# HKU-BAL/MegaPath-Nano

Hardware: AMD Instinct MI355X
Metric: Gbp/min ONT reads aligned+species-assigned vs RefSeq, 1/2/4/8 MI355X (higher is better)
Workload: dtype int32

## Files before the change

### include/mpn_map.h

```cpp
#ifndef MPN_MAP_H
#define MPN_MAP_H
#include <stdint.h>

#ifdef __cplusplus
extern "C" {
#endif

typedef struct mpn_index mpn_index;

typedef struct {
    int32_t k, w;
    float mid_occ_frac;
    int32_t mid_occ;
    int32_t max_gap, bw, max_chain_skip, max_chain_iter, min_cnt, min_chain_score;
    float mask_level, pri_ratio;
    int32_t best_n;
    int32_t max_join_long, max_join_short, min_join_flank_sc;
    float min_join_flank_ratio;
    int32_t a, b, q, e, q2, e2, sc_ambi, zdrop, zdrop_inv, end_bonus, min_dp_max, min_ksw_len;
    float max_clip_ratio;
    int64_t max_sw_mat;
    int32_t with_cigar;
    uint32_t seed;
    int32_t host_threads;
    int32_t out_sam;
    int32_t out_tags;
} mpn_map_opt;

enum {
    MPN_TAG_CS = 1,
    MPN_TAG_CS_LONG = 2,
    MPN_TAG_MD = 4,
    MPN_TAG_EQX = 8
};

void mpn_map_opt_init(mpn_map_opt *opt);

mpn_index *mpn_index_build(int32_t n_seq, const char *const *names, const char *const *seqs, const int32_t *lens,
                           int32_t k, int32_t w);
mpn_index *mpn_index_build_device(int32_t n_seq, const char *const *names, const void *d_seqs, const int64_t *seq_off,
                                  const int32_t *lens, int32_t k, int32_t w);
void mpn_index_destroy(mpn_index *idx);
int mpn_index_save(const mpn_index *idx, const char *path);
int64_t mpn_sam_header(const mpn_index *idx, const char *cmdline, char *buf, int64_t cap);
mpn_index *mpn_index_load(const char *path);
int mpn_index_save_append(const mpn_index *idx, const char *path);
mpn_index *mpn_index_load_at(const char *path, int64_t offset, int64_t *next_offset);
int32_t mpn_index_part_info(const char *path, int64_t offset, int64_t *bases, int64_t *next_offset);
int32_t mpn_index_n_seq(const mpn_index *idx);
int32_t mpn_index_seq_len(const mpn_index *idx, int32_t i);
int32_t mpn_index_seq_name(const mpn_index *idx, int32_t i, char *buf, int32_t cap);
int32_t mpn_index_k(const mpn_index *idx);
int32_t mpn_index_w(const mpn_index *idx);
int64_t mpn_index_n_minimizers(const mpn_index *idx);
int64_t mpn_index_n_keys(const mpn_index *idx);
int32_t mpn_index_mid_occ(const mpn_index *idx, float frac);
int64_t mpn_index_fetch_seq(const mpn_index *idx, int32_t i, int64_t start, int64_t len, char *out);
int mpn_index_export(const mpn_index *idx, uint64_t *keys, int64_t *key_off, uint64_t *pos);

int64_t mpn_sketch_batch(int32_t n, const char *seqs, const int64_t *seq_off, const int32_t *seq_len, int32_t k,
                         int32_t w, int64_t *mz_off, uint64_t *mz, int64_t cap);

int mpn_seed_chain_batch(const mpn_index *idx, const mpn_map_opt *opt, int32_t n, const char *seqs,
                         const int64_t *seq_off, const int32_t *seq_len, int64_t *n_anchor, int32_t *rep_len,
                         int64_t *chain_off, uint64_t *u, int64_t u_cap, int64_t *anchor_off, uint64_t *b,
                         int64_t b_cap);

int mpn_chain_batch(const mpn_map_opt *opt, int32_t n, const int64_t *anchor_off, const uint64_t *anchors, int32_t chain_item,
                    int32_t bt_par_min, int32_t grid_cap, int32_t *n_chain, int64_t *n_chained, uint64_t *u, int64_t *recs,
                    int64_t u_cap, uint64_t *b, int64_t b_cap);

int mpn_ext_dp_batch(const mpn_map_opt *opt, int32_t n, const uint8_t *qcodes, const int64_t *q_off, const int32_t *q_len,
                     const uint8_t *tcodes, const int64_t *t_off, const int32_t *t_len, const int32_t *w, const int32_t *zdrop,
                     const int32_t *end_bonus, const int32_t *flag, int32_t force_kernel, int32_t *out9, uint32_t *cigar_pool,
                     int64_t cigar_cap, int64_t *cig_off);

int mpn_aln_tags_batch(int32_t n, const uint8_t *qcodes, const int64_t *q_off, const int32_t *q_len,
                       const int32_t *qs, const int32_t *qe, const int32_t *rev,
                       const uint8_t *tcodes, const int64_t *t_off, const int32_t *t_len, const int32_t *ts,
                       const uint32_t *cigar, const int64_t *cig_off, const int32_t *n_cigar, int32_t out_tags,
                       char *cs, int64_t cs_cap, int64_t *cs_off, char *md, int64_t md_cap, int64_t *md_off,
                       uint32_t *eqx, int64_t eqx_cap, int64_t *eqx_off);

int mpn_aln_finish_batch(const mpn_map_opt *opt, int32_t n, const uint8_t *qcodes, const int64_t *q_off, const int32_t *q_len,
                         const int32_t *qs, const int32_t *qe, const int32_t *rev,
                         const uint8_t *tcodes, const int64_t *t_off, const int32_t *t_len, const int32_t *ts,
                         const uint32_t *cigar, const int64_t *cig_off, const int32_t *n_cigar, int32_t force_class,
                         int32_t *out8, uint32_t *cigar_out);

int mpn_hit_select_batch(const mpn_map_opt *opt, int32_t k, int32_t n, const int32_t *q_len, const char *const *names,
                         const int64_t *chain_off, const uint64_t *u, const uint64_t *fx, const uint64_t *fy, const uint64_t *lx,
                         const uint64_t *ly, const int32_t *mlen, const int32_t *blen, const int64_t *anchor_off, const uint64_t *anchors,
                         int32_t path, int32_t max_chains, int32_t grid_cap, int32_t *n_regs, int32_t *n_a, int64_t *hits,
                         uint64_t *sq_anchors);

int mpn_ext_plan_batch(const mpn_map_opt *opt, int32_t k, int32_t n_targets, const int32_t *t_len, int32_t n, const int32_t *q_len,
                       const int64_t *anchor_off, const uint64_t *anchors, const int64_t *hit_off, const int32_t *h_as,
                       const int32_t *h_cnt, const int32_t *h_mlen, const int32_t *h_split_inv, int32_t grid_cap,
                       int32_t *hits_out, int64_t win_cap, int64_t *n_win, int32_t *win_out, uint64_t *anchors_out);

int mpn_stitch_batch(int32_t n, const int64_t *anchor_off, const uint64_t *anchors, int32_t n_hits, const int32_t *hits, int64_t n_win,
                     const int32_t *wins, const int64_t *cig_pos, int64_t n_compact, const uint32_t *compact, int32_t min_cnt,
                     int32_t grid_cap, int64_t *out, int64_t pool_cap, uint32_t *pool_out, int64_t *pool_used, int64_t *splits_out,
                     int64_t *n_splits);

int64_t mpn_map_batch(const mpn_index *idx, const mpn_map_opt *opt, int32_t n, const char *const *names,
                      const char *seqs, const int64_t *seq_off, const int32_t *seq_len, char *paf, int64_t paf_cap);

typedef struct {
    int64_t cap, n_rows;
    int32_t *read_idx, *qs, *qe, *rev, *rid, *rs, *re, *mlen, *blen, *mapq, *nm, *as, *primary;
} mpn_aln_cols;

int64_t mpn_map_batch_ex(const mpn_index *idx, const mpn_map_opt *opt, int32_t n, const char *const *names,
                         const char *seqs, const int64_t *seq_off, const int32_t *seq_len, const void *d_seqs,
                         const int64_t *d_off, const int32_t *d_len, char *paf, int64_t paf_cap, mpn_aln_cols *cols);

int64_t mpn_map_batch_q(const mpn_index *idx, const mpn_map_opt *opt, int32_t n, const char *const *names, const char *seqs,
                        const char *quals, const int64_t *seq_off, const int32_t *seq_len, const void *d_seqs, const int64_t *d_off,
                        const int32_t *d_len, char *paf, int64_t paf_cap, mpn_aln_cols *cols);
int64_t mpn_map_fetch_sam(char *buf, int64_t cap);

typedef struct mpn_hits mpn_hits;
mpn_hits *mpn_hits_create(int32_t n_reads);
void mpn_hits_destroy(mpn_hits *h);
void mpn_hits_set_text(mpn_hits *h, int32_t want_text);
int mpn_map_batch_part(const mpn_index *part, const mpn_map_opt *opt, int32_t n, const char *const *names, const char *seqs,
                       const int64_t *seq_off, const int32_t *seq_len, const void *d_seqs, const int64_t *d_off,
                       const int32_t *d_len, mpn_hits *acc);
int mpn_map_batch_parts(const mpn_index *const *parts, int32_t n_parts, const mpn_map_opt *opt, int32_t n, const char *const *names,
                        const char *seqs, const int64_t *seq_off, const int32_t *seq_len, const void *r_seqs, const int64_t *r_off,
                        const int32_t *r_len, mpn_hits *acc);
int64_t mpn_hits_finish(mpn_hits *acc, const mpn_map_opt *opt, int32_t n, const char *const *names, const char *seqs,
                        const char *quals, const int64_t *seq_off, const int32_t *seq_len, char *paf, int64_t paf_cap,
                        mpn_aln_cols *cols);
int32_t mpn_hits_n_parts(const mpn_hits *h);
int32_t mpn_hits_n_seq(const mpn_hits *h);
int32_t mpn_hits_seq_len(const mpn_hits *h, int32_t i);
int32_t mpn_hits_seq_name(const mpn_hits *h, int32_t i, char *buf, int32_t cap);
int64_t mpn_hits_sam_header(const mpn_hits *h, const char *cmdline, char *buf, int64_t cap);

int64_t mpn_hits_export(const mpn_hits *h, int32_t lo, int32_t hi, void *buf, int64_t cap);
int mpn_hits_import(mpn_hits *h, const void *buf, int64_t len, int32_t n_parts, int32_t n_seq, const char *const *names,
                    const int32_t *lens);

int64_t mpn_map_fetch_cols(mpn_aln_cols *cols);
int64_t mpn_map_fetch_text(char *buf, int64_t cap);

void mpn_map_last_stats(int64_t stats[32]);
int32_t mpn_map_last_stats_ex(int64_t *stats, int32_t n);

#ifdef __cplusplus
}
#endif
#endif
```

### megapath_nano_amd/csrc/align.hip

```cpp
#include "map_types.h"
#include "ext_kernels.h"
#include "fin_kernels.h"
#include "tag_kernels.h"
#include "stitch_kernels.h"
#include "plan_kernels.h"
#include "hit_kernels.h"
#include "mapper_internal.h"
#include "../../include/mpn_map.h"
#include "../../include/mpn_ssw.h"

#include <algorithm>
#include <condition_variable>
#include <deque>
#include <math.h>
#include <stdio.h>
#include <string.h>
#include <thread>
#include <pthread.h>
#include <time.h>
#include <atomic>
#include <functional>
#include <mutex>
#include <stdlib.h>
#include <string>
// ... 1818 lines not shown
        std::vector<uint32_t> nh((size_t)n, 0u);
        if (names) for (int i = 0; i < n; ++i) nh[(size_t)i] = names[i] ? x31_hash(names[i]) : 0u;
        if (d_name_hash.upload(nh.data(), (size_t)n, st0)) return -1;
        MPN_HIP_CHECK(hipStreamSynchronize(st0));
    }
    MPN_HIP_CHECK(hipStreamSynchronize(st0));
    wt.stop_into(g_stats[16]);
    int n_threads = default_host_threads(opt);
    *n_threads_out = n_threads;
    g_pool.ensure(n_threads);
    int n_workers = 12;
    if (const char *e = getenv("MPN_PIPE_WORKERS")) n_workers = std::max(1, std::min(16, atoi(e)));
    static double obs_bytes_per_bp = 0.0;
    static int64_t obs_sub_bp = 0;
    const bool env_target = getenv("MPN_SUB_BATCH_BP") != nullptr;
    const int W_all = n_workers;
    std::vector<int> cut;
    auto make_cuts = [&](int64_t target) {
        cut.assign(1, 0);
        std::vector<int64_t> sizes;
        int64_t n_cut = std::max<int64_t>(1, (bases + target - 1) / target);
        if (n_cut > W_all) n_cut = (n_cut + W_all - 1) / W_all * W_all;
        for (int64_t i = 0; i < n_cut; ++i) sizes.push_back(std::max<int64_t>(1, (bases + n_cut - 1) / n_cut));
        size_t si = 0;
        int64_t acc = 0;
        for (int i = 0; i < n; ++i) {
            acc += seq_len[i];
            if (si + 1 < sizes.size() && acc >= sizes[si] && i + 1 < n) { cut.push_back(i + 1); acc = 0; ++si; }
        }
        cut.push_back(n);
    };
    int64_t target = 32000000;
    if (env_target) target = std::max<int64_t>(1000, atoll(getenv("MPN_SUB_BATCH_BP")));
    make_cuts(target);
    int n_sub = (int)cut.size() - 1;
    int64_t largest = n_sub > 0 ? (bases + n_sub - 1) / n_sub : bases;
    {
        size_t free_b = 0, total_b = 0, held = 0;
        if (hipMemGetInfo(&free_b, &total_b) == hipSuccess) {
            for (const Slot &S : g_slots) held += S.device_bytes();
            const double avail = 0.9 * (double)(free_b + held);
            const double bytes_per_bp = obs_bytes_per_bp > 0 ? std::max(400.0, 1.15 * obs_bytes_per_bp) : 900.0;
            auto per_worker = [&](int64_t sub_bp) { return bytes_per_bp * (double)std::max<int64_t>(sub_bp, 1) + 2e9; };
            int fit = (int)std::max(1.0, avail / per_worker(largest));
            if (fit < std::min(W_all, n_sub) && !env_target && largest > 11000000) {
                const double room = avail / W_all - 2e9;
                const int64_t t2 = std::max<int64_t>(11000000, (int64_t)(room / bytes_per_bp));
                if (t2 < largest) {
                    make_cuts(t2);
                    n_sub = (int)cut.size() - 1;
                    largest = n_sub > 0 ? (bases + n_sub - 1) / n_sub : bases;
                    fit = (int)std::max(1.0, avail / per_worker(largest));
                }
            }
            if (obs_sub_bp > 0 && largest < obs_sub_bp * 3 / 4) {
                MPN_HIP_CHECK(hipDeviceSynchronize());
                for (Slot &S : g_slots) S.release_device();
            }
            n_workers = std::min(n_workers, fit);
        }
    }
    const int n_items = n_sub;
    n_workers = std::max(1, std::min(n_workers, n_items));
    for (int wdx = n_workers; wdx < 16; ++wdx)
        if (g_slots[wdx].device_bytes()) { MPN_HIP_CHECK(hipDeviceSynchronize()); g_slots[wdx].release_device(); }
    int dev = 0;
    MPN_HIP_CHECK(hipGetDevice(&dev));
    QueueStreams *qs = queue_streams(dev);
    if (!qs) { set_error("creating the submission streams failed"); return -1; }
    rs.assign((size_t)n_parts, std::vector<ReadState>());
    rep_len.assign((size_t)n_parts, std::vector<int32_t>());
    for (int p = 0; p < n_parts; ++p) { rs[(size_t)p].assign((size_t)n, ReadState()); rep_len[(size_t)p].assign((size_t)n, 0); }
    std::atomic<int> next(0), failed(0);
    std::mutex mu;
    std::deque<int> retry;
    int live_workers = n_workers, live_workers_busy = 0, n_shed = 0;
    int64_t tot_stats[MPN_NSTATS] = {0};
    std::string err;
    const bool dbg_workers = getenv("MPN_DEBUG_WORKERS") != nullptr;
    g_phase_log.on = getenv("MPN_DEBUG_PHASES") != nullptr;
    g_cpu_on = getenv("MPN_DEBUG_CPU") != nullptr;
    if (g_cpu_on) { for (auto &c : g_cpu_ns) c = 0; for (auto &c : g_worker_cpu_ns) c = 0; }
    g_worker_cpu_on = g_cpu_on;
    if (g_phase_log.on) { g_phase_log.recs.clear(); g_phase_log.origin = std::chrono::steady_clock::now(); }
    const auto t_call = std::chrono::steady_clock::now();
    auto since = [&]() { return std::chrono::duration<double, std::milli>(std::chrono::steady_clock::now() - t_call).count(); };
    auto worker = [&](int wid) {
        pthread_setname_np(pthread_self(), "mpn-work");
        if (hipSetDevice(dev) != hipSuccess) { failed = 1; return; }
        Slot &S = g_slots[wid];
        StreamLease lease(qs);
        tl_slot = &S;
        tl_arena = &S.arena;
        tl_worker_id = wid;
        memset(g_stats, 0, sizeof(g_stats));
        for (;;) {
            int sb = -1;
            { std::lock_guard<std::mutex> g(mu); if (!retry.empty()) { sb = retry.front(); retry.pop_front(); } }
            if (sb < 0) sb = next.fetch_add(1);
            if (sb >= n_items || failed) {
                std::unique_lock<std::mutex> lk(mu);
                if (failed || (retry.empty() && live_workers_busy == 0)) break;
                lk.unlock();
                timespec ts{0, 200000};
                nanosleep(&ts, nullptr);
                continue;
            }
            { std::lock_guard<std::mutex> g(mu); ++live_workers_busy; }
            struct Busy { std::mutex &m; int &c; ~Busy() { std::lock_guard<std::mutex> g(m); --c; } } busy_{mu, live_workers_busy};
            S.arena.reset();
            tl_oom = false;
            int64_t stats_before[MPN_NSTATS];
            memcpy(stats_before, g_stats, sizeof(stats_before));
            const double t_in = since();
            struct Out { bool on; int wid, sb; double t_in; decltype(since) &f; ~Out() { if (on) fprintf(stderr, "[worker %d] sub-batch %d: %.1f -> %.1f ms\n", wid, sb, t_in, f()); } } out_{dbg_workers, wid, sb, t_in, since};
            int rc_item = 0;
            {
                ReadSketch sk;
                const int sbi = sb, nr = cut[sbi + 1] - cut[sbi];
                if (n_parts > 1 && nr > 0) {
                    WallTimer wts;
                    rc_item = sketch_reads(parts[0]->k, parts[0]->w, nr, dv.p, dv.po + cut[sbi], dv.pl + cut[sbi], seq_len + cut[sbi], sk, lease);
                    wts.stop_into(g_stats[17]);
                }
                const Arena::Mark after_sketch = S.arena.mark();
                for (int prt = 0; prt < n_parts && !rc_item; ++prt) {
                    S.arena.rewind(after_sketch);
                    rc_item = map_range(parts[prt], opt, names, seqs, seq_off, seq_len, dv.p, dv.po, dv.pl, d_name_hash.p, cut[sbi], cut[sbi + 1], n_threads, lease,
                                        rs[(size_t)prt], rep_len[(size_t)prt], sk.valid ? &sk : nullptr);
                }
                if (!rc_item && stream_sync(lease) != hipSuccess) { set_error("stream wait failed"); rc_item = -1; }
            }
            if (rc_item) {
                std::lock_guard<std::mutex> g(mu);
                if (tl_oom && live_workers > 1) {
                    --live_workers;
                    ++n_shed;
                    memcpy(g_stats, stats_before, sizeof(stats_before));
                    (void)hipGetLastError();
                    (void)stream_sync(lease);
                    S.release_device();
                    retry.push_back(sb);
                    if (dbg_workers) fprintf(stderr, "[worker %d] out of device memory at sub-batch %d: leaving, %d workers go on\n", wid, sb, live_workers);
                    break;
                }
                err = get_error();
                failed = 1;
                (void)stream_sync(lease);
                break;
            }
        }
        tl_arena = nullptr;
        std::lock_guard<std::mutex> g(mu);
        for (int k = 0; k < MPN_NSTATS; ++k) tot_stats[k] += g_stats[k];
    };
    {
        std::vector<std::thread> th;
        for (int wdx = 0; wdx < n_workers; ++wdx) th.emplace_back(worker, wdx);
        for (auto &t : th) t.join();
    }
    if (dbg_workers) {
        fprintf(stderr, "[call] workers joined at %.1f ms\n", since());
        for (int wdx = 0; wdx < n_workers; ++wdx) {
            const Slot &S = g_slots[wdx];
            size_t arena = 0;
            for (const auto &c : S.arena.chunks) arena += c.cap;
            const size_t pools = S.pool_jobs.cap + S.pool_P.cap + S.pool_P2.cap + S.pool_OFF.cap + S.pool_order.cap + S.pool_state.cap + S.pool_CIG.cap +
                                 S.pool_res.cap + S.pool_redo.cap + S.pool_compact.cap + S.pool_used.cap;
            const size_t pinned = S.pin_order.cap + S.pin_res.cap + S.pin_chain_u.cap + S.pin_chain_b.cap + S.pin_segs.cap + S.pin_pregs.cap + S.pin_fin_cig.cap + S.pin_fin_out.cap + S.pin_tags.cap + S.pin_tag_bytes.cap;
            fprintf(stderr, "[slot %d] arena %.2f GB, pools %.2f GB (P %.2f, CIG %.2f, compact %.2f), pinned host %.2f GB\n", wdx, arena / 1e9,
                    pools / 1e9, S.pool_P.cap / 1e9, S.pool_CIG.cap / 1e9, S.pool_compact.cap / 1e9, pinned / 1e9);
        }
    }
    if (g_phase_log.on) {
        for (const auto &r : g_phase_log.recs) fprintf(stderr, "[phase] %d %d %lld %lld\n", r.worker, r.slot, (long long)r.t0, (long long)r.t1);
        fprintf(stderr, "[phase-end]\n");
    }
    if (g_cpu_on) {
        static const char *const nm[] = {"other", "hits", "plan", "plan-copy", "stitch", "final", "dp-group-A", "strip-sort", "job-copy", "finish-copy", "accumulate", "merge"};
        fprintf(stderr, "[cpu] thread CPU ms in parallel regions:");
        for (int k = 0; k < 12; ++k) fprintf(stderr, " %s %.0f", nm[k], g_cpu_ns[k].load() / 1e6);
        fprintf(stderr, "\n[cpu] sections: stitch-append %.0f", g_cpu_ns[16].load() / 1e6);
        for (int k = 3; k < 16; ++k) if (g_cpu_ns[16 + k].load() > 500000) fprintf(stderr, " s%d %.0f", k, g_cpu_ns[16 + k].load() / 1e6);
        fprintf(stderr, "\n[cpu] worker-thread CPU ms by phase slot:");
        for (int k = 0; k < 64; ++k) if (g_worker_cpu_ns[k].load() > 500000) fprintf(stderr, " [%d] %.0f", k, g_worker_cpu_ns[k].load() / 1e6);
        fprintf(stderr, "\n");
    }
    if (failed) { set_error("%s", err.empty() ? "worker failed" : err.c_str()); return -1; }
    {
        const int64_t h2d = g_stats[16];
        memcpy(g_stats, tot_stats, sizeof(tot_stats));
        g_stats[16] = h2d;
        g_stats[0] = bases;
        g_stats[60] = n_shed; g_stats[61] = n_workers;
        {
            size_t held_max = 0;
            for (const Slot &S : g_slots) held_max = std::max(held_max, S.device_bytes());
            if (largest > 0 && held_max > 0) {
                const double r = (double)held_max / (double)largest;
                obs_bytes_per_bp = obs_sub_bp == largest ? std::max(obs_bytes_per_bp, r) : r;
                obs_sub_bp = largest;
            }
        }
    }
    return 0;
}

static struct Kept { std::vector<int32_t> cols; int64_t n_rows = -1; std::string text, sam; bool has_text = false, has_sam = false; } g_kept;

static int64_t emit_batch(const Targets tg, const mpn_map_opt *opt, int32_t n, const char *const *names, const char *seqs, const char *quals,
                          const int64_t *seq_off, const int32_t *seq_len, std::vector<std::vector<Reg>*> &regs, const std::vector<int32_t> &rep_len,
                          int n_threads, char *text, int64_t text_cap, mpn_aln_cols *cols) {
    const bool want_paf = text && opt->out_sam != 1, want_sam = opt->out_sam == 2 || (text && opt->out_sam == 1);
    std::vector<std::string> paf_lines(want_paf ? n : 0), sam_lines(want_sam ? n : 0);
    int64_t n_aln = 0;
    for (int i = 0; i < n; ++i) n_aln += (int64_t)regs[i]->size();
    if (want_paf || want_sam)
        parallel_for(n, n_threads, [&](int i, int) {
            const char *nm = names && names[i] ? names[i] : "*";
            if (want_paf && !regs[i]->empty()) write_paf(tg, opt, nm, seq_len[i], *regs[i], rep_len[i], paf_lines[i]);
            if (want_sam) write_sam(tg, opt, nm, seq_len[i], seqs + seq_off[i], quals ? quals + seq_off[i] : nullptr, *regs[i], rep_len[i], sam_lines[i]);
        }, 0, 16);
    bool short_cols = false, short_text = false;
    g_kept.cols.clear(); g_kept.text.clear(); g_kept.sam.clear(); g_kept.n_rows = -1; g_kept.has_text = g_kept.has_sam = false;
    if (cols) {
        cols->n_rows = n_aln;
        short_cols = n_aln > cols->cap;
        int32_t *dst[13] = {cols->read_idx, cols->qs, cols->qe, cols->rev, cols->rid, cols->rs, cols->re, cols->mlen, cols->blen, cols->mapq,
                            cols->nm, cols->as, cols->primary};
        if (short_cols) {
            g_kept.cols.resize((size_t)n_aln * 13);
            g_kept.n_rows = n_aln;
            for (int c = 0; c < 13; ++c) dst[c] = g_kept.cols.data() + (size_t)c * (size_t)n_aln;
        }
        int64_t k = 0;
        for (int i = 0; i < n; ++i)
            for (const Reg &r : *regs[i]) {
                dst[0][k] = i; dst[1][k] = r.qs; dst[2][k] = r.qe; dst[3][k] = (int32_t)r.rev; dst[4][k] = r.rid;
                dst[5][k] = r.rs; dst[6][k] = r.re; dst[7][k] = r.mlen; dst[8][k] = r.blen; dst[9][k] = (int32_t)r.mapq;
                dst[10][k] = r.has_p ? r.blen - r.mlen + r.n_ambi : -1;
                dst[11][k] = r.has_p ? r.dp_score : -1;
                dst[12][k] = r.id == r.parent;
                ++k;
            }
    }
    int64_t w = 0;
    if (text) {
        std::vector<std::string> &lines = opt->out_sam == 1 ? sam_lines : paf_lines;
        int64_t tot = 0;
        for (auto &l : lines) tot += (int64_t)l.size();
        short_text = tot + 1 > text_cap;
        if (short_text) {
            g_kept.text.reserve((size_t)tot);
            for (auto &l : lines) g_kept.text += l;
            g_kept.has_text = true;
        } else {
            for (auto &l : lines) { memcpy(text + w, l.data(), l.size()); w += (int64_t)l.size(); }
            text[w] = 0;
        }
    }
    if (opt->out_sam == 2) {
        size_t tot = 0;
        for (auto &l : sam_lines) tot += l.size();
        g_kept.sam.reserve(tot);
        for (auto &l : sam_lines) g_kept.sam += l;
        g_kept.has_sam = true;
    }
    parallel_chunks(n, n_threads, [&](int64_t lo, int64_t hi, int) {
        for (int64_t i = lo; i < hi; ++i) { if (want_paf) std::string().swap(paf_lines[i]); if (want_sam) std::string().swap(sam_lines[i]); }
    });
    g_stats[6] = n_aln;
    return (short_cols || short_text) ? -3 : w;
}

static std::mutex g_call_mu;

extern "C" int64_t mpn_map_batch_q(const mpn_index *idx, const mpn_map_opt *opt, int32_t n, const char *const *names,
                                   const char *seqs, const char *quals, const int64_t *seq_off, const int32_t *seq_len, const void *r_seqs,
                                   const int64_t *r_off, const int32_t *r_len, char *paf, int64_t paf_cap, mpn_aln_cols *cols) {
    std::lock_guard<std::mutex> call_guard(g_call_mu);
    memset(g_stats, 0, sizeof(g_stats));
    if (cols) cols->n_rows = 0;
    if (n <= 0) { if (paf && paf_cap > 0) paf[0] = 0; g_kept = Kept(); if (opt->out_sam == 2) g_kept.has_sam = true; return 0; }
    WallTimer whole;
    std::vector<std::vector<ReadState>> rs_p;
    std::vector<std::vector<int32_t>> rep_p;
    int n_threads = 1;
    g_need_cigar = paf != nullptr || opt->out_sam != 0;
    if (map_batch_core(&idx, 1, opt, n, names, seqs, seq_off, seq_len, r_seqs, r_off, r_len, rs_p, rep_p, &n_threads)) return -1;
    std::vector<ReadState> &rs = rs_p[0];
    std::vector<int32_t> &rep_len = rep_p[0];
    std::vector<std::vector<Reg>*> regs((size_t)n);
    for (int i = 0; i < n; ++i) regs[(size_t)i] = &rs[(size_t)i].regs;
    const int64_t w = emit_batch(Targets{&idx->names, &idx->lens}, opt, n, names, seqs, quals, seq_off, seq_len, regs, rep_len, n_threads, paf, paf_cap, cols);
    parallel_chunks(n, n_threads, [&](int64_t lo, int64_t hi, int) { for (int64_t i = lo; i < hi; ++i) rs[(size_t)i] = ReadState(); });
    whole.stop_into(g_stats[24]);
    return w;
}

extern "C" int64_t mpn_map_batch_ex(const mpn_index *idx, const mpn_map_opt *opt, int32_t n, const char *const *names,
                                    const char *seqs, const int64_t *seq_off, const int32_t *seq_len, const void *r_seqs,
                                    const int64_t *r_off, const int32_t *r_len, char *paf, int64_t paf_cap, mpn_aln_cols *cols) {
    return mpn_map_batch_q(idx, opt, n, names, seqs, nullptr, seq_off, seq_len, r_seqs, r_off, r_len, paf, paf_cap, cols);
}

extern "C" mpn_hits *mpn_hits_create(int32_t n_reads) {
    if (n_reads < 0) { set_error("mpn_hits_create: negative read count"); return nullptr; }
// ... 885 lines not shown
```

### megapath_nano_amd/csrc/map_kernels.h

```cpp
#pragma once
#include "mpn_common.h"
#include "map_types.h"

#include <type_traits>

namespace mpn {

__device__ __forceinline__ uint64_t hash64m(uint64_t key, uint64_t mask) {
    key = (~key + (key << 21)) & mask;
    key = key ^ key >> 24;
    key = ((key + (key << 3)) + (key << 8)) & mask;
    key = key ^ key >> 14;
    key = ((key + (key << 2)) + (key << 4)) & mask;
    key = key ^ key >> 28;
    key = (key + (key << 31)) & mask;
    return key;
}

constexpr int SKETCH_FAST_MAX_W = 32;

template <bool HASH64>
__device__ __forceinline__ uint64_t sketch_hash(uint64_t key, uint64_t mask) {
    if (HASH64) return hash64m(key, mask);
    uint32_t h = (uint32_t)key;
// ... 1272 lines not shown
                const unsigned long long over = __ballot(skipev && skips > cp.max_skip);
                const int brk = over ? __builtin_ctzll(over) : 64;
                if (!over) n_skip = __builtin_amdgcn_readlane(skips, 63);
                const bool elig = !cont && lane < brk;
                const int best = brk > 0 ? __builtin_amdgcn_readlane(incl, brk - 1) : NEG_INF;
                if (best > max_f) {
                    const unsigned long long who = __ballot(elig && sc == best);
                    const int wl = __builtin_ctzll(who);
                    max_f = best;
                    max_j = j0 - wl;
                }
                if (!tile_in_ring && elig && pj >= 0) {
                    if (pj >= win_lo) wt[pj & M] = i;
                    else { t[pj] = i; gmark = true; }
                }
                if (brk < 64) done = true;
                if (__ballot(gmark)) __builtin_amdgcn_fence(__ATOMIC_RELEASE, "workgroup");
                MPN_LDS_FENCE();
            }
            int32_t vprev = 0;
            if (max_j >= 0) vprev = max_j >= win_lo ? wv[max_j & M] : v[max_j];
            const int32_t vi = (max_j >= 0 && vprev > max_f) ? vprev : max_f;
            if (lane == li) { rf = max_f; rp = max_j >= 0 ? max_j + rel : -1; rv = vi; }
            if (lane == 0) {
                const int sl = i & M;
                *reinterpret_cast<uint4 *>(&ring[sl]) = make_uint4(ri, (uint32_t)qi, (uint32_t)max_f, (uint32_t)max_j);
                wv[sl] = vi; wt[sl] = 0;
            }
            MPN_LDS_FENCE();
            if (li == 63 || i == n - 1) {
                const int32_t k = (i & ~63) + lane;
                if (k <= i) { f[k] = rf; p[k] = rp; v[k] = rv; }
                const uint32_t carry = (uint32_t)__builtin_amdgcn_readlane((int)cx, 63);
                cx = (uint32_t)wave_scan_add((int)nstep) + carry; cx64 = nx64; cyl = nyl; cyh = nyh;
            }
        }
        __builtin_amdgcn_fence(__ATOMIC_RELEASE, "workgroup");
        __syncthreads();
    }
}

__global__ __launch_bounds__(64) void chain_ends_kernel(const int64_t *__restrict__ anchor_off, int n_reads, ChainParams cp,
                                                        const int32_t *__restrict__ F, const int32_t *__restrict__ P,
                                                        int32_t *__restrict__ T, const int32_t *__restrict__ V,
                                                        uint64_t *__restrict__ U, int32_t *__restrict__ n_ends) {
    const int lane = threadIdx.x;
    for (int read = blockIdx.x; read < n_reads; read += gridDim.x) {
        const int64_t base = anchor_off[read];
        const int64_t n = anchor_off[read + 1] - base;
        const int32_t *f = F + base, *p = P + base, *v = V + base;
        int32_t *t = T + base;
        uint64_t *u = U + base;
        for (int64_t i = lane; i < n; i += 64) t[i] = 0;
        __builtin_amdgcn_fence(__ATOMIC_RELEASE, "workgroup");
        __syncthreads();
        for (int64_t i = lane; i < n; i += 64) if (p[i] >= 0) t[p[i]] = 1;
        __builtin_amdgcn_fence(__ATOMIC_RELEASE, "workgroup");
        __syncthreads();
        int cnt = 0;
        for (int64_t i0 = 0; i0 < n; i0 += 64) {
            const int64_t i = i0 + lane;
            bool is_end = i < n && t[i] == 0 && v[i] >= cp.min_sc;
            uint64_t val = 0;
            if (is_end) {
                int64_t j = i;
                while (j >= 0 && f[j] < v[j]) j = p[j];
                if (j < 0) j = i;
                val = (uint64_t)(uint32_t)f[j] << 32 | (uint64_t)j;
            }
            const unsigned long long m = __ballot(is_end);
            if (is_end) u[cnt + __popcll(m & ((1ULL << lane) - 1))] = val;
            cnt += __popcll(m);
        }
        if (lane == 0) n_ends[read] = cnt;
        __syncthreads();
    }
}

__global__ __launch_bounds__(256) void chain_sort_ends_kernel(uint64_t *__restrict__ U, uint64_t *__restrict__ Utmp,
                                                              const int64_t *__restrict__ anchor_off,
                                                              const int32_t *__restrict__ n_ends, int n_reads) {
    __shared__ uint32_t hist[256];
    __shared__ uint32_t bins[256];
    __shared__ uint32_t wcnt[4][256];
    __shared__ int s_skip;
    const int tid = threadIdx.x, lane = tid & 63, wv = tid >> 6;
    for (int read = blockIdx.x; read < n_reads; read += gridDim.x) {
        const int64_t base = anchor_off[read];
        const int n = n_ends[read];
        if (n < 2) continue;
        uint64_t *src = U + base, *dst = Utmp + base;
        for (int pass = 0; pass < 8; ++pass) {
            hist[tid] = 0;
            __syncthreads();
            for (int i = tid; i < n; i += 256) atomicAdd(&hist[(uint32_t)(~src[i] >> (8 * pass)) & 0xff], 1u);
            __syncthreads();
            if (tid == 0) s_skip = 0;
            __syncthreads();
            if (hist[tid] == (uint32_t)n) s_skip = 1;
            __syncthreads();
            if (s_skip) { __syncthreads(); continue; }
            {
                uint32_t v = hist[tid];
                bins[tid] = v;
                __syncthreads();
                for (int d = 1; d < 256; d <<= 1) {
                    uint32_t a = tid >= d ? bins[tid - d] : 0;
                    __syncthreads();
                    bins[tid] += a;
                    __syncthreads();
                }
                uint32_t excl = bins[tid] - v;
                __syncthreads();
                bins[tid] = excl;
                __syncthreads();
            }
            for (int t0 = 0; t0 < n; t0 += 256) {
                const int i = t0 + tid;
                const bool act = i < n;
                uint64_t r = 0;
                uint32_t dg = 0;
                if (act) { r = src[i]; dg = (uint32_t)(~r >> (8 * pass)) & 0xff; }
                wcnt[0][tid] = 0; wcnt[1][tid] = 0; wcnt[2][tid] = 0; wcnt[3][tid] = 0;
                __syncthreads();
                unsigned long long same = __ballot(act);
#pragma unroll
                for (int b = 0; b < 8; ++b) {
                    unsigned long long m = __ballot((dg >> b) & 1);
                    same &= ((dg >> b) & 1) ? m : ~m;
                }
                const uint32_t rank = __popcll(same & ((1ULL << lane) - 1));
                if (act && rank == 0) wcnt[wv][dg] = __popcll(same);
                __syncthreads();
                if (act) {
                    uint32_t o = bins[dg] + rank;
                    for (int w2 = 0; w2 < wv; ++w2) o += wcnt[w2][dg];
                    dst[o] = r;
                }
                __syncthreads();
                bins[tid] += wcnt[0][tid] + wcnt[1][tid] + wcnt[2][tid] + wcnt[3][tid];
                __syncthreads();
            }
            uint64_t *sw = src; src = dst; dst = sw;
            __threadfence_block();
            __syncthreads();
        }
        if (src != U + base) for (int i = tid; i < n; i += 256) U[base + i] = src[i];
        __syncthreads();
    }
}

constexpr int BT_PAR_MIN = 16;

__global__ __launch_bounds__(64) void chain_backtrack_kernel(const u128 *__restrict__ anchors, const int64_t *__restrict__ anchor_off,
                                                             int n_reads, ChainParams cp, const int32_t *__restrict__ F,
                                                             const int32_t *__restrict__ P, int32_t *__restrict__ T,
                                                             int32_t *__restrict__ V, uint64_t *__restrict__ U,
                                                             const int32_t *__restrict__ n_ends, u128 *__restrict__ B,
                                                             uint64_t *__restrict__ Uc, unsigned long long *__restrict__ used,
                                                             int64_t *__restrict__ u_pos, int64_t *__restrict__ b_pos,
                                                             int32_t *__restrict__ n_chain, int64_t *__restrict__ n_chained,
                                                             ChainRec *__restrict__ Rc, int par_min) {
    __shared__ int s_k;
    __shared__ unsigned long long s_up, s_bp;
    const int lane = threadIdx.x;
    for (int read = blockIdx.x; read < n_reads; read += gridDim.x) {
        const int64_t base = anchor_off[read];
        const int64_t n = anchor_off[read + 1] - base;
        const u128 *a = anchors + base;
        const int32_t *f = F + base, *p = P + base;
        int32_t *t = T + base, *v = V + base;
        uint64_t *u = U + base;
        const int n_u = n_ends[read];
        if (n_u >= par_min) {
            for (int64_t i = lane; i < n; i += 64) t[i] = 0x7fffffff;
            __builtin_amdgcn_fence(__ATOMIC_RELEASE, "agent");
            __syncthreads();
            for (int e0 = 0; e0 < n_u; e0 += 64) {
                const int e = e0 + lane;
                if (e < n_u) {
                    int32_t j = (int32_t)u[e];
                    while (j >= 0) { const int32_t nj = p[j]; if (atomicMin(&t[j], e) < e) break; j = nj; }
                }
            }
            __builtin_amdgcn_fence(__ATOMIC_ACQ_REL, "agent");
            __syncthreads();
            int k_run = 0, nv_run = 0;
            for (int e0 = 0; e0 < n_u; e0 += 64) {
                const int e = e0 + lane;
                int cnt = 0;
                if (e < n_u) {
                    const uint64_t ui = u[e];
                    int32_t j = p[(int32_t)ui];
                    cnt = 1;
                    while (j >= 0) { const int32_t tj = t[j], nj = p[j]; if (tj != e) break; ++cnt; j = nj; }
                    const bool keep = cnt >= cp.min_cnt && (j < 0 || (int32_t)(ui >> 32) - f[j] >= cp.min_sc);
                    if (!keep) cnt = 0;
                    v[e] = cnt;
                }
                k_run += __builtin_amdgcn_readlane(wave_scan_add(cnt > 0 ? 1 : 0), 63);
                nv_run += __builtin_amdgcn_readlane(wave_scan_add(cnt), 63);
            }
            if (lane == 0) {
                s_k = k_run;
                n_chain[read] = k_run;
                n_chained[read] = nv_run;
                s_up = k_run ? atomicAdd(&used[0], (unsigned long long)k_run) : 0ULL;
                s_bp = nv_run ? atomicAdd(&used[1], (unsigned long long)nv_run) : 0ULL;
                u_pos[read] = (int64_t)s_up;
                b_pos[read] = (int64_t)s_bp;
            }
            __builtin_amdgcn_fence(__ATOMIC_ACQ_REL, "agent");
            __syncthreads();
            u128 *b = B + s_bp;
            uint64_t *uc = Uc + s_up;
            ChainRec *rc = Rc + s_up;
            k_run = 0; nv_run = 0;
            for (int e0 = 0; e0 < n_u; e0 += 64) {
                const int e = e0 + lane;
                const int cnt = e < n_u ? v[e] : 0;
                const int incl = wave_scan_add(cnt), kin = wave_scan_add(cnt > 0 ? 1 : 0);
                if (cnt > 0) {
                    const int kidx = k_run + kin - 1, off = nv_run + incl - cnt;
                    const uint64_t ui = u[e];
                    int32_t j = (int32_t)ui;
                    u128 nxt = a[j];
                    const u128 last = nxt;
                    int ml = 0, bl = 0;
                    b[off + cnt - 1] = nxt;
                    for (int q = cnt - 2; q >= 0; --q) {
                        j = p[j];
                        const u128 cur = a[j];
                        b[off + q] = cur;
                        const int span = (int)(nxt.y >> 32 & 0xff);
                        const int tl = (int32_t)nxt.x - (int32_t)cur.x, ql = (int32_t)nxt.y - (int32_t)cur.y;
                        bl += tl > ql ? tl : ql;
                        ml += tl > span && ql > span ? span : tl < ql ? tl : ql;
                        nxt = cur;
                    }
                    const int span0 = (int)(nxt.y >> 32 & 0xff);
                    ml += span0; bl += span0;
                    j = p[j];
                    const uint64_t sc = j < 0 ? ui >> 32 : (ui >> 32) - (uint64_t)f[j];
                    uc[kidx] = sc << 32 | (uint32_t)cnt;
                    rc[kidx] = ChainRec{nxt.x, nxt.y, last.x, last.y, ml, bl};
                }
                k_run += __builtin_amdgcn_readlane(kin, 63);
                nv_run += __builtin_amdgcn_readlane(incl, 63);
            }
            __syncthreads();
            continue;
        }
        for (int64_t i = lane; i < n; i += 64) t[i] = 0;
        __builtin_amdgcn_fence(__ATOMIC_RELEASE, "workgroup");
        __syncthreads();
        if (lane == 0) {
            int n_v = 0, k = 0;
            for (int i = 0; i < n_u; ++i) {
                const int n_v0 = n_v, k0 = k;
                const uint64_t ui = u[i];
                int64_t j = (int32_t)ui;
                do { v[n_v++] = (int32_t)j; t[j] = 1; j = p[j]; } while (j >= 0 && t[j] == 0);
                if (j < 0) {
                    if (n_v - n_v0 >= cp.min_cnt) u[k++] = ui >> 32 << 32 | (uint32_t)(n_v - n_v0);
                } else if ((int32_t)(ui >> 32) - f[j] >= cp.min_sc) {
                    if (n_v - n_v0 >= cp.min_cnt) u[k++] = ((ui >> 32) - (uint64_t)f[j]) << 32 | (uint32_t)(n_v - n_v0);
                }
                if (k0 == k) n_v = n_v0;
            }
            s_k = k;
            n_chain[read] = k;
            n_chained[read] = n_v;
            s_up = k ? atomicAdd(&used[0], (unsigned long long)k) : 0ULL;
            s_bp = n_v ? atomicAdd(&used[1], (unsigned long long)n_v) : 0ULL;
            u_pos[read] = (int64_t)s_up;
            b_pos[read] = (int64_t)s_bp;
        }
        __builtin_amdgcn_fence(__ATOMIC_RELEASE, "workgroup");
        __syncthreads();
        const int k = s_k;
        u128 *b = B + s_bp;
        uint64_t *uc = Uc + s_up;
        ChainRec *rc = Rc + s_up;
        int off = 0;
        for (int c = 0; c < k; ++c) {
            const int ni = (int32_t)u[c];
            int ml = 0, bl = 0;
            for (int j = lane; j < ni; j += 64) {
                const u128 cur = a[v[off + (ni - j - 1)]];
                b[off + j] = cur;
                const int span = (int)(cur.y >> 32 & 0xff);
                if (j == 0) { ml += span; bl += span; }
                else {
                    const u128 prev = a[v[off + (ni - j)]];
                    const int tl = (int32_t)cur.x - (int32_t)prev.x, ql = (int32_t)cur.y - (int32_t)prev.y;
                    bl += tl > ql ? tl : ql;
                    ml += tl > span && ql > span ? span : tl < ql ? tl : ql;
                }
            }
            ml = __builtin_amdgcn_readlane(wave_scan_add(ml), 63);
            bl = __builtin_amdgcn_readlane(wave_scan_add(bl), 63);
            if (lane == 0) {
                const u128 first = a[v[off + ni - 1]], last = a[v[off]];
                rc[c] = ChainRec{first.x, first.y, last.x, last.y, ml, bl};
            }
            off += ni;
        }
        for (int c = lane; c < k; c += 64) uc[c] = u[c];
        __syncthreads();
    }
}

__global__ __launch_bounds__(256) void idx_bucket_hist_kernel(const u128 *__restrict__ mz, int64_t n, int shift, unsigned long long *__restrict__ hist) {
    for (int64_t i = (int64_t)blockIdx.x * blockDim.x + threadIdx.x; i < n; i += (int64_t)gridDim.x * blockDim.x)
        atomicAdd(&hist[(mz[i].x >> 8) >> shift], 1ULL);
}

__global__ __launch_bounds__(256) void idx_bucket_scatter_kernel(const u128 *__restrict__ mz, int64_t n, int shift,
                                                                 unsigned long long *__restrict__ cursor, u128 *__restrict__ out) {
    for (int64_t i = (int64_t)blockIdx.x * blockDim.x + threadIdx.x; i < n; i += (int64_t)gridDim.x * blockDim.x) {
        u128 r = mz[i];
        r.x >>= 8;
        const unsigned long long p = atomicAdd(&cursor[r.x >> shift], 1ULL);
        out[p] = r;
    }
}

__global__ __launch_bounds__(256) void idx_flag_count_kernel(const u128 *__restrict__ rec, int64_t n, int64_t *__restrict__ block_cnt) {
    __shared__ int s[256];
    const int64_t base = (int64_t)blockIdx.x * 2048;
    int c = 0;
    for (int k = 0; k < 8; ++k) {
        const int64_t i = base + k * 256 + threadIdx.x;
        if (i < n && (i == 0 || rec[i].x != rec[i - 1].x)) ++c;
    }
    s[threadIdx.x] = c;
    __syncthreads();
    for (int d = 128; d; d >>= 1) { if (threadIdx.x < d) s[threadIdx.x] += s[threadIdx.x + d]; __syncthreads(); }
    if (threadIdx.x == 0) block_cnt[blockIdx.x] = s[0];
}

__global__ __launch_bounds__(256) void idx_emit_kernel(const u128 *__restrict__ rec, int64_t n, const int64_t *__restrict__ block_off,
                                                       uint64_t *__restrict__ keys, int64_t *__restrict__ key_off,
                                                       uint64_t *__restrict__ pos) {
    __shared__ int s[256];
    const int64_t base = (int64_t)blockIdx.x * 2048;
    int flags = 0, c = 0;
    for (int k = 0; k < 8; ++k) {
        const int64_t i = base + (int64_t)threadIdx.x * 8 + k;
        if (i < n) {
            pos[i] = rec[i].y;
            if (i == 0 || rec[i].x != rec[i - 1].x) { flags |= 1 << k; ++c; }
        }
    }
    s[threadIdx.x] = c;
    __syncthreads();
    for (int d = 1; d < 256; d <<= 1) {
        const int v = threadIdx.x >= d ? s[threadIdx.x - d] : 0;
        __syncthreads();
        s[threadIdx.x] += v;
        __syncthreads();
    }
    int64_t o = block_off[blockIdx.x] + s[threadIdx.x] - c;
    for (int k = 0; k < 8; ++k)
        if (flags >> k & 1) {
            const int64_t i = base + (int64_t)threadIdx.x * 8 + k;
            keys[o] = rec[i].x;
            key_off[o] = i;
            ++o;
        }
}

__global__ __launch_bounds__(256) void idx_pack2_kernel(const uint8_t *__restrict__ seqs, int64_t total, uint32_t *__restrict__ words,
                                                        int64_t n_words, unsigned long long *__restrict__ counters,
                                                        int64_t *__restrict__ starts, int64_t *__restrict__ ends, int64_t cap) {
    const bool aligned = (reinterpret_cast<uintptr_t>(seqs) & 15) == 0;
    for (int64_t wi = (int64_t)blockIdx.x * blockDim.x + threadIdx.x; wi < n_words; wi += (int64_t)gridDim.x * blockDim.x) {
        const int64_t g0 = wi * 16;
        uint8_t b[16];
        if (aligned && g0 + 16 <= total) {
            const uint4 v = *reinterpret_cast<const uint4 *>(seqs + g0);
            const uint32_t q[4] = {v.x, v.y, v.z, v.w};
#pragma unroll
            for (int k = 0; k < 16; ++k) b[k] = (uint8_t)(q[k >> 2] >> (8 * (k & 3)));
        } else {
#pragma unroll
            for (int k = 0; k < 16; ++k) b[k] = g0 + k < total ? seqs[g0 + k] : (uint8_t)'A';
        }
        bool prev_n = g0 > 0 && g0 - 1 < total && nt4_code(seqs[g0 - 1]) > 3;
        uint32_t word = 0;
#pragma unroll
        for (int k = 0; k < 16; ++k) {
            const int64_t g = g0 + k;
            const int c = nt4_code(b[k]);
            const bool isn = g < total && c > 3;
            if (g < total && !isn) word |= (uint32_t)c << (2 * k);
            if (isn != prev_n && g <= total) {
                const unsigned long long p = atomicAdd(&counters[isn ? 0 : 1], 1ULL);
                if ((int64_t)p < cap) (isn ? starts : ends)[p] = g;
            }
            prev_n = isn;
        }
        words[wi] = word;
    }
}

__global__ __launch_bounds__(256) void idx_occ_hist_kernel(const u128 *__restrict__ kv, int64_t n_keys, int nbins,
                                                           unsigned long long *__restrict__ hist) {
    __shared__ unsigned int local[1024];
    for (int k = threadIdx.x; k < 1024; k += blockDim.x) local[k] = 0;
    __syncthreads();
    for (int64_t i = (int64_t)blockIdx.x * blockDim.x + threadIdx.x; i < n_keys; i += (int64_t)gridDim.x * blockDim.x) {
        const int64_t occ = (int64_t)(kv[i + 1].y - kv[i].y);
        if (occ < 1024) atomicAdd(&local[(int)occ], 1u);
        else atomicAdd(&hist[occ < nbins - 1 ? occ : nbins - 1], 1ULL);
    }
    __syncthreads();
    for (int k = threadIdx.x; k < 1024; k += blockDim.x) if (local[k]) atomicAdd(&hist[k], (unsigned long long)local[k]);
}

}
```

### megapath_nano_amd/csrc/mapper.hip

```cpp
#include "map_kernels.h"
#include "mapper_internal.h"
#include "../../include/mpn_map.h"

#include <algorithm>
#include <mutex>
#include <string.h>
#include <time.h>
#include <sys/stat.h>
#include <string>
#include <vector>

namespace mpn {

hipError_t stream_sync(hipStream_t st) {
    struct Ev {
        hipEvent_t e = nullptr;
        ~Ev() { if (e) (void)hipEventDestroy(e); }
    };
    static thread_local Ev ev;
    hipError_t rc;
    if (!ev.e && (rc = hipEventCreateWithFlags(&ev.e, hipEventDisableTiming)) != hipSuccess) return rc;
    if ((rc = hipEventRecord(ev.e, st)) != hipSuccess) return rc;
    unsigned int us = 20;
    for (;;) {
// ... 57 lines not shown
    *out = *s;
    return 0;
}

thread_local int64_t g_stats[MPN_NSTATS] = {0};
PhaseLog g_phase_log;
bool g_worker_cpu_on = false;
std::atomic<long long> g_worker_cpu_ns[64];
thread_local int tl_worker_id = -1;

void pack_2bit(const uint8_t *codes, int64_t n, std::vector<uint32_t> &words, std::vector<int64_t> &ns, std::vector<int64_t> &ne) {
    words.assign((size_t)(n + 15) / 16 + 1, 0u);
    ns.clear(); ne.clear();
    for (int64_t i = 0; i < n; ++i) {
        const uint8_t c = codes[i];
        if (c > 3) {
            if (!ne.empty() && ne.back() == i) ne.back() = i + 1;
            else { ns.push_back(i); ne.push_back(i + 1); }
        } else words[(size_t)(i >> 4)] |= (uint32_t)c << (2 * (int)(i & 15));
    }
}

static int grid_1d(int64_t n, int block, int cap = 256 * 16) {
    int64_t g = (n + block - 1) / block;
    return (int)std::max<int64_t>(1, std::min<int64_t>(g, cap));
}

int sketch_device(const uint8_t *d_seqs, const int64_t *d_off, const int32_t *d_len, const int32_t *h_len, int n, int k, int w,
                  uint32_t rid_base, DevBuf<int64_t> &mz_off, DevBuf<u128> &mz, int64_t *n_mz, hipStream_t st, EvTimer *ev = nullptr) {
    const int C = 256;
    std::vector<int64_t> chunk_off((size_t)n + 1, 0);
    for (int i = 0; i < n; ++i) chunk_off[i + 1] = chunk_off[i] + (h_len[i] + C - 1) / C;
    const int64_t n_chunks = chunk_off[n];
    DevBuf<int64_t> cnt, d_chunk_off, slow_list;
    DevBuf<int32_t> chunk_cnt, chunk_rel;
    DevBuf<unsigned long long> n_slow, emask;
    DevBuf<uint8_t> cfast;
    DevBuf<int32_t> chunk_read;
    DevBuf<u128> stage;
    int64_t stage_chunks = 0;
    if (cnt.alloc((size_t)n + 1) || mz_off.alloc((size_t)n + 1) || d_chunk_off.upload(chunk_off.data(), (size_t)n + 1, st) ||
        chunk_cnt.alloc((size_t)n_chunks) || chunk_rel.alloc((size_t)n_chunks) || slow_list.alloc((size_t)n_chunks) || n_slow.alloc(1) ||
        emask.alloc((size_t)n_chunks * 4 + 4) || cfast.alloc((size_t)n_chunks + 1) || chunk_read.alloc((size_t)n_chunks + 1))
        return -1;
    hipLaunchKernelGGL(sketch_chunk_read_kernel, dim3(std::max(1, std::min((n + 3) / 4, 4096))), dim3(256), 0, st, (const int64_t *)d_chunk_off.p, n, chunk_read.p);
    {
        std::vector<int64_t> slow;
        const bool none_fast = !(k & 1) || w > SKETCH_FAST_MAX_W;
        for (int i = 0; i < n; ++i) {
            const int64_t nc = chunk_off[i + 1] - chunk_off[i];
            for (int64_t c = 0; c < nc; ++c) {
                const int64_t p0 = c * C, p1 = std::min<int64_t>(h_len[i], p0 + C);
                if (none_fast || p0 - 2 * w - k < 0 || p1 + w + 1 > h_len[i]) slow.push_back(chunk_off[i] + c);
                else if (p1 + C + w + 1 <= h_len[i]) c = std::max<int64_t>(c, (h_len[i] - w - 1) / C - 2);
            }
        }
        const unsigned long long ns = slow.size();
        stage_chunks = (int64_t)std::min<unsigned long long>((unsigned long long)n_chunks, ns + 2048);
        if (stage_chunks * SKETCH_STAGE_CAP * sizeof(u128) > ((size_t)1 << 30)) stage_chunks = ((size_t)1 << 30) / (SKETCH_STAGE_CAP * sizeof(u128));
        if (stage.alloc((size_t)stage_chunks * SKETCH_STAGE_CAP + 1)) return -1;
        if (ns) MPN_HIP_CHECK(hipMemcpyAsync(slow_list.p, slow.data(), ns * 8, hipMemcpyHostToDevice, st));
        MPN_HIP_CHECK(hipMemcpyAsync(n_slow.p, &ns, 8, hipMemcpyHostToDevice, st));
        MPN_HIP_CHECK(stream_sync(st));
    }
    const size_t lds = (size_t)2 * w * 64 * sizeof(uint64_t);
    const unsigned fast_grid = (unsigned)std::max<int64_t>(1, std::min<int64_t>((n_chunks + 3) / 4, 256 * 64));
    const unsigned slow_grid = (unsigned)std::max<int64_t>(1, std::min<int64_t>((n_chunks + 63) / 64, 256 * 16));
    const bool hash64 = 2 * k > 32;
    auto pass = [&](bool fill, u128 *out) {
        if (n_chunks <= 0) return;
        const int64_t *moff = fill ? (const int64_t *)mz_off.p : nullptr;
        const int32_t *crel = fill ? (const int32_t *)chunk_rel.p : nullptr;
        int32_t *ccnt = fill ? nullptr : chunk_cnt.p;
        if (fill) {
            if (hash64) hipLaunchKernelGGL(sketch_fill_kernel<true>, dim3(fast_grid), dim3(256), 0, st, d_seqs, d_off, d_len, n, (const int64_t *)d_chunk_off.p, (const int32_t *)chunk_read.p, n_chunks, C,
                                           w, k, moff, crel, out, rid_base, (const unsigned long long *)emask.p, (const uint8_t *)cfast.p);
            else hipLaunchKernelGGL(sketch_fill_kernel<false>, dim3(fast_grid), dim3(256), 0, st, d_seqs, d_off, d_len, n, (const int64_t *)d_chunk_off.p, (const int32_t *)chunk_read.p, n_chunks, C,
                                    w, k, moff, crel, out, rid_base, (const unsigned long long *)emask.p, (const uint8_t *)cfast.p);
        } else {
#define MPN_SKETCH_FAST(H, WCT) hipLaunchKernelGGL((sketch_fast_kernel<H, WCT>), dim3(fast_grid), dim3(256), 0, st, d_seqs, d_off, d_len, n, \
                                                  (const int64_t *)d_chunk_off.p, (const int32_t *)chunk_read.p, n_chunks, C, w, k, ccnt, slow_list.p, n_slow.p, emask.p, cfast.p)
            if (hash64) MPN_SKETCH_FAST(true, 0); else if (w == 10) MPN_SKETCH_FAST(false, 10); else MPN_SKETCH_FAST(false, 0);
#undef MPN_SKETCH_FAST
        }
        if (fill) {
            hipLaunchKernelGGL(sketch_stage_copy_kernel, dim3(slow_grid), dim3(256), 0, st, (const int32_t *)chunk_read.p, (const int64_t *)slow_list.p,
                               (const unsigned long long *)n_slow.p, stage_chunks, moff, crel, (const int32_t *)chunk_cnt.p, (const u128 *)stage.p, out);
            if (stage_chunks < n_chunks)
                hipLaunchKernelGGL(sketch_chunk_kernel<true>, dim3(slow_grid), dim3(64), lds, st, d_seqs, d_off, d_len, n, (const int64_t *)d_chunk_off.p, (const int32_t *)chunk_read.p,
                                   (const int64_t *)slow_list.p, (const unsigned long long *)n_slow.p, C, w, k, moff, crel, ccnt, out, rid_base,
                                   (u128 *)nullptr, (int64_t)0, stage_chunks);
        } else hipLaunchKernelGGL(sketch_chunk_kernel<false>, dim3(slow_grid), dim3(64), lds, st, d_seqs, d_off, d_len, n, (const int64_t *)d_chunk_off.p, (const int32_t *)chunk_read.p,
                                  (const int64_t *)slow_list.p, (const unsigned long long *)n_slow.p, C, w, k, moff, crel, ccnt, out, rid_base,
                                  stage.p, stage_chunks, (int64_t)0);
    };
    if (ev) ev->skip();
    pass(false, nullptr);
    MPN_HIP_CHECK(hipGetLastError());
    if (ev) ev->mark(10, 33);
    hipLaunchKernelGGL(sketch_chunk_prefix_kernel, dim3((n + 255) / 256), dim3(256), 0, st, (const int64_t *)d_chunk_off.p, n,
                       (const int32_t *)chunk_cnt.p, chunk_rel.p, cnt.p);
    MPN_HIP_CHECK(hipGetLastError());
    hipLaunchKernelGGL(scan_i64_kernel, dim3(1), dim3(1024), 0, st, cnt.p, mz_off.p, n);
    MPN_HIP_CHECK(hipGetLastError());
    int64_t total = 0;
    if (read_i64(mz_off.p + n, &total, st)) return -1;
    if (mz.alloc((size_t)total)) return -1;
    if (ev) ev->mark(10);
    if (total > 0) {
        pass(true, mz.p);
        MPN_HIP_CHECK(hipGetLastError());
        if (ev) ev->mark(10, 34);
    }
    *n_mz = total;
    return 0;
}

int upload_seqs(int32_t n, const char *seqs, const int64_t *seq_off, const int32_t *seq_len, DevBuf<uint8_t> &d_seqs,
                DevBuf<int64_t> &d_off, DevBuf<int32_t> &d_len, int64_t *total_bases, hipStream_t st) {
    int64_t extent = 0, bases = 0;
    for (int i = 0; i < n; ++i) {
        if (seq_len[i] < 0 || seq_off[i] < 0) { set_error("negative sequence length/offset at %d", i); return -2; }
        extent = std::max<int64_t>(extent, seq_off[i] + seq_len[i]);
        bases += seq_len[i];
    }
    if (d_seqs.alloc((size_t)extent + 16)) return -1;
    if (extent) MPN_HIP_CHECK(hipMemcpyAsync(d_seqs.p, seqs, (size_t)extent, hipMemcpyHostToDevice, st));
    if (d_off.upload(seq_off, n, st) || d_len.upload(seq_len, n, st)) return -1;
    *total_bases = bases;
    return 0;
}

int sketch_reads(int k, int w, int n, const uint8_t *d_seqs, const int64_t *d_off, const int32_t *d_len, const int32_t *h_len, ReadSketch &sk,
                 StreamLease &st) {
    EvTimer ev(st);
    sk.valid = false;
    if (sketch_device(d_seqs, d_off, d_len, h_len, n, k, w, 0, sk.mz_off, sk.mz, &sk.n_mz, st, &ev)) return -1;
    MPN_HIP_CHECK(stream_sync(st));
    ev.resolve();
    sk.k = k; sk.w = w; sk.valid = true;
    return 0;
}

static int chain_gap_check(const mpn_map_opt *opt, const char *who) {
    if (opt->max_gap > CHAIN_MAX_GAP) {
        set_error("%s: max_gap %d is beyond %d, the largest the chain DP's 32-bit ring coordinate holds", who, opt->max_gap, CHAIN_MAX_GAP);
        return -1;
    }
    return 0;
}

static int alloc_chain_tables(SeedChainOut &o, int n) {
    const size_t N = (size_t)n, o1 = (N + 1) * 8, o2 = o1 + N * 8, o3 = o2 + N * 8, o4 = o3 + N * 8, o5 = o4 + N * 4, o6 = (o5 + N * 4 + 7) & ~(size_t)7;
    o.tables_bytes = o6 + (size_t)(2 + WORK_SLOTS) * 8;
    if (o.tables.alloc(o.tables_bytes)) return -1;
    auto view = [&](auto &buf, size_t off, size_t count) { buf.release(); buf.p = reinterpret_cast<decltype(buf.p)>(o.tables.p + off); buf.n = count; buf.owned = false; };
    view(o.n_anchor, 0, N + 1); view(o.n_chained, o1, N); view(o.u_pos, o2, N); view(o.b_pos, o3, N);
    view(o.n_chain, o4, N); view(o.rep_len, o5, N); view(o.used, o6, 2 + WORK_SLOTS);
    return 0;
}

struct ChainKnobs {
    int chain_item = 0;
    int bt_par_min = 0;
    int grid_cap = 0;
};
struct ChainScratch {
    DevBuf<int64_t> kept, piece_kept, piece_off;
    DevBuf<float> avg_qspan;
    DevBuf<int32_t> F, P, T, V;
    DevBuf<uint64_t> Utmp;
    DevBuf<ChainSeg> seg_big, seg_small;
};
static int chain_enqueue(const mpn_map_opt *opt, int n, int64_t n_a, SeedChainOut &o, u128 *tmp, unsigned long long *read_kept,
                         const unsigned long long *span_sum, unsigned int *seg_counters, const ChainKnobs &kn, ChainScratch &cs, StreamLease &st,
                         EvTimer &ev) {
    auto &[kept, piece_kept, piece_off, avg_qspan, F, P, T, V, Utmp, seg_big, seg_small] = cs;
    ChainParams cp;
    cp.max_dist_x = opt->max_gap; cp.max_dist_y = opt->max_gap; cp.bw = opt->bw; cp.max_skip = opt->max_chain_skip;
    cp.max_iter = opt->max_chain_iter; cp.min_cnt = opt->min_cnt; cp.min_sc = opt->min_chain_score;
    const auto capped = [&](int64_t grid) { return (int)(kn.grid_cap > 0 ? std::min<int64_t>(grid, kn.grid_cap) : grid); };
    const int g = capped(std::max(1, std::min(n, 256 * 32)));
    const int64_t n_pieces = (n_a + COMPACT_PIECE - 1) / COMPACT_PIECE;
    if (kept.alloc((size_t)n + 1) || o.c_off.alloc((size_t)n + 1) || avg_qspan.alloc(n) || piece_kept.alloc((size_t)n_pieces + 1) ||
        piece_off.alloc((size_t)n_pieces + 1))
        return -1;
    const int gp = capped(std::max<int64_t>(1, std::min<int64_t>(n_pieces, 256 * 64)));
    if (n_a > 0) {
        hipLaunchKernelGGL(anchor_compact_kernel<false>, dim3(gp), dim3(64), 0, st, (const u128 *)o.anchors.p, (const int64_t *)o.anchor_off.p, n, n_a,
                           cp.max_dist_x, cp.min_cnt, piece_kept.p, read_kept, (const int64_t *)nullptr, (u128 *)nullptr);
        MPN_HIP_CHECK(hipGetLastError());
    }
    hipLaunchKernelGGL(anchor_compact_finish_kernel, dim3((n + 255) / 256), dim3(256), 0, st, (const int64_t *)o.n_anchor.p, n,
                       (const unsigned long long *)read_kept, span_sum, kept.p, avg_qspan.p);
    hipLaunchKernelGGL(scan_i64x2_kernel, dim3(2), dim3(1024), 0, st, (const int64_t *)kept.p, o.c_off.p, n, (const int64_t *)piece_kept.p, piece_off.p, (int)n_pieces);
    MPN_HIP_CHECK(hipGetLastError());
    int64_t n_c = 0;
    if (read_i64(o.c_off.p + n, &n_c, st)) return -1;
    g_stats[45] += n_c;
    if (F.alloc(n_c) || P.alloc(n_c) || T.alloc(n_c) || V.alloc(n_c) || o.u.alloc(n_c) || Utmp.alloc(n_c) || o.chained.alloc(n_c) ||
        o.recs.alloc((size_t)(n_c / std::max(1, opt->min_cnt)) + 1))
        return -1;
    u128 *ca = tmp;
    if (n_a > 0) {
        hipLaunchKernelGGL(anchor_compact_kernel<true>, dim3(gp), dim3(64), 0, st, (const u128 *)o.anchors.p, (const int64_t *)o.anchor_off.p, n, n_a,
                           cp.max_dist_x, cp.min_cnt, (int64_t *)nullptr, (unsigned long long *)nullptr, (const int64_t *)piece_off.p, ca);
        MPN_HIP_CHECK(hipGetLastError());
    }
    ev.mark(46);
    static const int chain_item_env = []() { const char *e = getenv("MPN_CHAIN_ITEM"); return e ? std::min(CHAIN_BIG, std::max(16, atoi(e))) : CHAIN_ITEM; }();
    const int chain_item = kn.chain_item > 0 ? std::min(CHAIN_BIG, std::max(16, kn.chain_item)) : chain_item_env;
    if (seg_big.alloc((size_t)n_c / CHAIN_BIG + (size_t)n + 1) || seg_small.alloc((size_t)n_c / chain_item + (size_t)n + 1)) return -1;
    hipLaunchKernelGGL(chain_segments_kernel, dim3(g), dim3(64), 0, st, (const u128 *)ca, (const int64_t *)o.c_off.p, n, cp, avg_qspan.p, 1, seg_big.p,
                       seg_small.p, seg_counters, chain_item);
    MPN_HIP_CHECK(hipGetLastError());
    ev.mark(13);
    hipLaunchKernelGGL(chain_dp_kernel, dim3(capped(256 * 32)), dim3(64), 0, st, (const u128 *)ca, (const int64_t *)o.c_off.p, (const float *)avg_qspan.p,
                       (const ChainSeg *)seg_big.p, (const ChainSeg *)seg_small.p, seg_counters, cp, F.p, P.p, T.p, V.p);
    MPN_HIP_CHECK(hipGetLastError());
    ev.mark(13, 37);
    hipLaunchKernelGGL(chain_ends_kernel, dim3(g), dim3(64), 0, st, (const int64_t *)o.c_off.p, n, cp, F.p, P.p, T.p, V.p, o.u.p, o.n_ends.p);
    MPN_HIP_CHECK(hipGetLastError());
    hipLaunchKernelGGL(chain_sort_ends_kernel, dim3(capped(std::max(1, std::min(n, 256 * 8)))), dim3(256), 0, st, o.u.p, Utmp.p,
                       (const int64_t *)o.c_off.p, o.n_ends.p, n);
    MPN_HIP_CHECK(hipGetLastError());
    o.u_compact.p = Utmp.p; o.u_compact.n = Utmp.n; o.u_compact.owned = Utmp.owned; Utmp.p = nullptr; Utmp.n = 0;
    static const int bt_par_min_env = []() { const char *e = getenv("MPN_BT_PAR_MIN"); return e ? std::max(1, atoi(e)) : BT_PAR_MIN; }();
    const int bt_par_min = kn.bt_par_min > 0 ? kn.bt_par_min : bt_par_min_env;
    hipLaunchKernelGGL(chain_backtrack_kernel, dim3(g), dim3(64), 0, st, (const u128 *)ca, (const int64_t *)o.c_off.p, n, cp, F.p, P.p, T.p, V.p,
                       o.u.p, o.n_ends.p, o.chained.p, o.u_compact.p, o.used.p, o.u_pos.p, o.b_pos.p, o.n_chain.p, o.n_chained.p, o.recs.p, bt_par_min);
    MPN_HIP_CHECK(hipGetLastError());
    return 0;
}

int seed_chain_device(const mpn_index *idx, const mpn_map_opt *opt, int n, const uint8_t *d_seqs, const int64_t *d_off,
                      const int32_t *d_len, const int32_t *h_len, SeedChainOut &o, StreamLease &st, const ReadSketch *pre) {
    if (chain_gap_check(opt, "seed + chain stage")) return -1;
    int64_t n_mz = 0;
    DevBuf<int64_t> mz_off;
    DevBuf<u128> mz;
    EvTimer ev(st);
    if (pre && pre->valid && pre->k == idx->k && pre->w == idx->w) {
        mz_off.p = pre->mz_off.p; mz_off.n = pre->mz_off.n; mz_off.owned = false;
        mz.p = pre->mz.p; mz.n = pre->mz.n; mz.owned = false;
        n_mz = pre->n_mz;
    } else if (sketch_device(d_seqs, d_off, d_len, h_len, n, idx->k, idx->w, 0, mz_off, mz, &n_mz, st, &ev)) return -1;
    g_stats[1] += n_mz;
    int32_t mid_occ = opt->mid_occ > 0 ? opt->mid_occ : mpn_index_mid_occ(idx, opt->mid_occ_frac);
    if (mid_occ > (1 << 25)) {
        const int32_t top = mpn_index_mid_occ(idx, 1e-30f);
        if (top > 0) mid_occ = std::min(mid_occ, top);
    }
    DevBuf<int32_t> occ;
    DevBuf<int64_t> pos_start, rel_off, full_off, n_blk, blk_base;
    DevBuf<unsigned long long> span_sum;
    if (alloc_chain_tables(o, n)) return -1;
    if (occ.alloc(n_mz) || pos_start.alloc(n_mz) || rel_off.alloc(n_mz) || full_off.alloc((size_t)n + 1) ||
        n_blk.alloc((size_t)n + 1) || blk_base.alloc((size_t)n + 1) || span_sum.alloc(n) || o.anchor_off.alloc((size_t)n + 1))
        return -1;
    if (n_mz > 0) {
        hipLaunchKernelGGL(seed_lookup_kernel, dim3(grid_1d(n_mz, 256)), dim3(256), 0, st, (const u128 *)idx->kv.p,
                           idx->n_keys, (const int64_t *)idx->bucket_start.p, idx->bucket_shift, mz.p, n_mz, mid_occ, occ.p, pos_start.p);
        MPN_HIP_CHECK(hipGetLastError());
        ev.mark(11, 35);
    }
    hipLaunchKernelGGL(seed_prefix_kernel, dim3(std::max(1, std::min(n, 256 * 32))), dim3(64), 0, st, mz.p, mz_off.p, n, occ.p, rel_off.p,
                       o.n_anchor.p, o.rep_len.p, span_sum.p, n_blk.p);
    MPN_HIP_CHECK(hipGetLastError());
    hipLaunchKernelGGL(scan_i64x2_kernel, dim3(2), dim3(1024), 0, st, (const int64_t *)o.n_anchor.p, full_off.p, n, (const int64_t *)n_blk.p, blk_base.p, n);
    MPN_HIP_CHECK(hipGetLastError());
    int64_t n_full = 0;
    if (read_i64(full_off.p + n, &n_full, st)) return -1;
    g_stats[2] += n_full;
    const int64_t nb_cap = n_mz / 64 + n + 1;
    DevBuf<unsigned long long> keep;
    DevBuf<int64_t> blk_kept, blk_off;
    DevBuf<int32_t> blk_read, order;
    DevBuf<unsigned int> next_read;
    DevBuf<unsigned int> n_list, seg_counters;
    DevBuf<unsigned long long> read_kept;
    if (next_read.alloc(4) || order.alloc(n) || keep.alloc((size_t)(n_full / 64 + nb_cap + 8)) || blk_kept.alloc((size_t)nb_cap + 1) || blk_off.alloc((size_t)nb_cap + 2) ||
        blk_read.alloc((size_t)nb_cap + 1) || n_list.alloc(4) || seg_counters.alloc(4) || read_kept.alloc(n))
        return -1;
    {
        ZeroList z{};
        zero_list_push(z, next_read.p, 4 * sizeof(unsigned int));
        zero_list_push(z, blk_kept.p, ((size_t)nb_cap + 1) * 8);
        zero_list_push(z, o.used.p, o.used.n * sizeof(unsigned long long));
        zero_list_push(z, n_list.p, 4 * sizeof(unsigned int));
        zero_list_push(z, seg_counters.p, 4 * sizeof(unsigned int));
        zero_list_push(z, read_kept.p, (size_t)n * 8);
        MPN_HIP_CHECK(zero_regions(z, st));
    }
    if (nb_cap > 0x7fffffff) { set_error("sub-batch too large for the seed filter"); return -1; }
    if (mid_occ > (1 << 25)) { set_error("occurrence cut-off %d too large (a block of 64 minimizers must hold fewer than 2^32 hits)", mid_occ); return -1; }
    if (n_full > 0) {
        FilterParams fp;
        {
            const int T = std::max(1, std::min(opt->min_cnt, 3));
            const int64_t need = 2 * (int64_t)(T - 1) * std::max(opt->max_gap, 1);
            int sh = 1;
            while (sh < 32 && ((int64_t)1 << sh) < need) ++sh;
            fp.shift = sh; fp.half = (uint32_t)((uint64_t)1 << (sh - 1)); fp.level = T - 1;
            static const int64_t round2 = []() { const char *e = getenv("MPN_FLT_ROUND2"); return e ? atoll(e) : INT64_MAX; }();
            fp.second_round = round2;
        }
        MPN_HIP_CHECK(hipFuncSetAttribute((const void *)seed_filter_kernel, hipFuncAttributeMaxDynamicSharedMemorySize, (int)FLT_LDS_BYTES));
        hipLaunchKernelGGL(seed_order_kernel, dim3(1), dim3(1024), 0, st, (const int64_t *)o.n_anchor.p, n, order.p);
        static const int flt_wgs = []() { const char *e = getenv("MPN_FLT_WGS"); return e ? std::max(1, atoi(e)) : 256; }();
        hipLaunchKernelGGL(seed_filter_kernel, dim3(std::max(1, std::min(n, flt_wgs))), dim3(FLT_THREADS), FLT_LDS_BYTES, st, mz.p, mz_off.p, n, occ.p,
                           pos_start.p, rel_off.p, idx->pos.p, (const int64_t *)full_off.p, (const int64_t *)blk_base.p, (const int32_t *)order.p,
                           fp, keep.p, blk_kept.p, blk_read.p, next_read.p);
        MPN_HIP_CHECK(hipGetLastError());
        ev.mark(11, 50);
    }
    hipLaunchKernelGGL(scan_i64_kernel, dim3(1), dim3(1024), 0, st, blk_kept.p, blk_off.p, (int)nb_cap);
    hipLaunchKernelGGL(seed_read_off_kernel, dim3((n + 256) / 256), dim3(256), 0, st, (const int64_t *)blk_off.p, (const int64_t *)blk_base.p, n,
                       o.anchor_off.p);
    MPN_HIP_CHECK(hipGetLastError());
    int64_t n_a = 0;
    if (read_i64(o.anchor_off.p + n, &n_a, st)) return -1;
    o.n_anchors = n_a;
    g_stats[51] += n_a;
    DevBuf<u128> tmp;
    if (o.anchors.alloc(n_a) || tmp.alloc(n_a) || o.n_ends.alloc(n)) return -1;
    ev.mark(11);
    if (n_a > 0) {
        hipLaunchKernelGGL(seed_emit_kernel, dim3(grid_1d(nb_cap, 4, 256 * 64)), dim3(256), 0, st, mz.p, mz_off.p, occ.p, pos_start.p, rel_off.p,
                           idx->pos.p, (const int64_t *)full_off.p, (const int64_t *)blk_base.p, n, (const unsigned long long *)keep.p,
                           (const int64_t *)blk_kept.p, (const int64_t *)blk_off.p, (const int32_t *)blk_read.p, d_len, tmp.p);
        MPN_HIP_CHECK(hipGetLastError());
        ev.mark(11, 36);
        BinParams bp;
        {
            int32_t max_len = 1;
            for (int32_t l : idx->lens) max_len = std::max(max_len, l);
            int rid_bits = 0, pos_bits = 1;
            while (((int64_t)1 << rid_bits) < (int64_t)idx->n_seq) ++rid_bits;
            while (((int64_t)1 << pos_bits) < (int64_t)max_len) ++pos_bits;
            bp.pos_bits = pos_bits;
            bp.shift = std::max(0, rid_bits + pos_bits - (MSD_BITS - 1));
        }
        SortLists lists;
        DevBuf<SortSeg> list_mem;
        {
            const int64_t c0 = n_a / (SMALL_BUCKET + 1) + (int64_t)n + 16, c1 = n_a / (BITONIC_SMALL + 1) + 16, c2 = n_a / (BITONIC_MID + 1) + 16;
            if (c0 > 0x7fffffff) { set_error("sub-batch too large for the anchor sort"); return -1; }
            if (list_mem.alloc((size_t)(c0 + c1 + c2))) return -1;
            lists.seg[0] = list_mem.p; lists.seg[1] = list_mem.p + c0; lists.seg[2] = list_mem.p + c0 + c1;
            lists.cap[0] = (unsigned int)c0; lists.cap[1] = (unsigned int)c1; lists.cap[2] = (unsigned int)c2;
            lists.count = n_list.p;
        }
        const size_t msd_lds = (size_t)(MSD_NB + 32) * sizeof(uint32_t);
        MPN_HIP_CHECK(hipFuncSetAttribute((const void *)anchor_msd_kernel, hipFuncAttributeMaxDynamicSharedMemorySize, (int)msd_lds));
        const int gr = std::max(1, std::min(n, 256 * 4));
        hipLaunchKernelGGL(anchor_msd_kernel, dim3(gr), dim3(MSD_THREADS), msd_lds, st, (const u128 *)tmp.p, o.anchors.p, (const int64_t *)o.anchor_off.p, n, bp,
                           lists, o.used.p + 2);
        MPN_HIP_CHECK(hipGetLastError());
        ev.mark(12, 47);
        const int64_t n_win = (n_a + SORT_WIN - 1) / SORT_WIN;
        hipLaunchKernelGGL(anchor_window_sort_kernel, dim3((unsigned)std::min<int64_t>(n_win, 256 * 64)), dim3(256), 0, st, o.anchors.p,
                           (const int64_t *)o.anchor_off.p, n, n_a, bp, o.used.p + 2);
        MPN_HIP_CHECK(hipGetLastError());
        ev.mark(12, 48);
        hipLaunchKernelGGL(anchor_bitonic_list_kernel<BITONIC_SMALL>, dim3(256 * 16), dim3(256), 0, st, o.anchors.p, (const SortSeg *)lists.seg[0],
                           (const unsigned int *)n_list.p, lists.cap[0], o.used.p + 2);
        hipLaunchKernelGGL(anchor_bitonic_list_kernel<BITONIC_MID>, dim3(256 * 4), dim3(256), 0, st, o.anchors.p, (const SortSeg *)lists.seg[1],
                           (const unsigned int *)n_list.p + 1, lists.cap[1], o.used.p + 2);
        hipLaunchKernelGGL(seg_sort_list_kernel<4>, dim3(256 * 4), dim3(256), 0, st, o.anchors.p, tmp.p, (const SortSeg *)lists.seg[2],
                           (const unsigned int *)n_list.p + 2, lists.cap[2], o.used.p + 2);
        MPN_HIP_CHECK(hipGetLastError());
        ev.mark(12, 49);
    }
    ChainScratch cs;
    if (chain_enqueue(opt, n, n_a, o, tmp.p, read_kept.p, span_sum.p, seg_counters.p, ChainKnobs{}, cs, st, ev)) return -1;
    ev.mark(14);
    MPN_HIP_CHECK(stream_sync(st));
    ev.resolve();
    return 0;
}

int download_chains(int n, SeedChainOut &o, HostChains &h, PoolBuf &pin_u, PoolBuf &pin_b, StreamLease &st, int mode) {
    const bool with_anchors = mode == 2;
    h.n_anchor.resize((size_t)n);
    h.n_chain.resize(n); h.n_chained.resize(n); h.rep_len.resize(n); h.u_pos.resize(n); h.b_pos.resize(n);
    unsigned long long used[2 + WORK_SLOTS] = {0};
    {
        const size_t N = (size_t)n;
        const size_t o1 = (N + 1) * 8, o2 = o1 + N * 8, o3 = o2 + N * 8, o4 = o3 + N * 8, o5 = o4 + N * 4, o6 = (o5 + N * 4 + 7) & ~(size_t)7;
        char *pn = (char *)tl_pin.get(o.tables_bytes + 64);
        if (!pn) { set_error("pinned scratch allocation failed"); return -1; }
        MPN_HIP_CHECK(hipMemcpyAsync(pn, o.tables.p, o.tables_bytes, hipMemcpyDeviceToHost, st));
        MPN_HIP_CHECK(stream_sync(st));
        memcpy(h.n_anchor.data(), pn, N * 8); memcpy(h.n_chained.data(), pn + o1, N * 8);
        memcpy(h.u_pos.data(), pn + o2, N * 8); memcpy(h.b_pos.data(), pn + o3, N * 8);
        memcpy(h.n_chain.data(), pn + o4, N * 4); memcpy(h.rep_len.data(), pn + o5, N * 4);
        memcpy(used, pn + o6, sizeof(used));
    }
    for (int k = 0; k < WORK_SLOTS; ++k) g_stats[44] += (int64_t)used[2 + k];
    ++g_stats[32];
    h.n_pool_chains = (int64_t)used[0];
    if (mode == 0) { h.u_all = nullptr; h.rec_all = nullptr; h.b_all = nullptr; }
    else if (with_anchors) {
        if (pin_u.ensure((size_t)used[0] * 8 + 16) || pin_b.ensure((size_t)used[1] * 16 + 16)) return -1;
        if (o.u_compact.download(pin_u.as<uint64_t>(), (size_t)used[0], st) || o.chained.download(pin_b.as<u128>(), (size_t)used[1], st)) return -1;
        h.u_all = pin_u.as<uint64_t>(); h.b_all = pin_b.as<u128>();
    } else {
        const size_t rec_bytes = ((size_t)used[0] * sizeof(ChainRec) + 15) & ~(size_t)15;
        if (pin_u.ensure(rec_bytes + (size_t)used[0] * 8 + 16)) return -1;
        h.rec_all = pin_u.as<ChainRec>();
        h.u_all = reinterpret_cast<const uint64_t *>(reinterpret_cast<const char *>(pin_u.p) + rec_bytes);
        h.b_all = nullptr;
        if (o.recs.download(const_cast<ChainRec *>(h.rec_all), (size_t)used[0], st) || o.u_compact.download(const_cast<uint64_t *>(h.u_all), (size_t)used[0], st)) return -1;
    }
    h.chain_off.assign((size_t)n + 1, 0);
    h.b_off.assign((size_t)n + 1, 0);
    for (int i = 0; i < n; ++i) { h.chain_off[i + 1] = h.chain_off[i] + h.n_chain[i]; h.b_off[i + 1] = h.b_off[i] + h.n_chained[i]; }
    MPN_HIP_CHECK(stream_sync(st));
    return 0;
}

void HostChains::read_chains(int i, uint64_t *uo, u128 *bo) const {
    const int nc = n_chain[i];
    if (nc == 0) return;
    const uint64_t *u = u_all + u_pos[i];
    const u128 *b = b_all + b_pos[i];
    std::vector<std::pair<std::pair<uint64_t, uint64_t>, int>> w(nc);
    int64_t k = 0;
    for (int c = 0; c < nc; ++c) { w[c] = {{b[k].x, (uint64_t)k << 32 | (uint32_t)c}, c}; k += (int32_t)u[c]; }
    std::sort(w.begin(), w.end());
    int64_t kk = 0;
    for (int c = 0; c < nc; ++c) {
        const int j = w[c].second;
        const int64_t start = (int64_t)(w[c].first.second >> 32);
        const int32_t cnt = (int32_t)u[j];
        uo[c] = u[j];
        memcpy(bo + kk, b + start, (size_t)cnt * sizeof(u128));
        kk += cnt;
    }
}

int download_chain_records(SeedChainOut &o, HostChains &h, PoolBuf &pin_u, StreamLease &st) {
    const size_t nc = (size_t)h.n_pool_chains;
    const size_t rec_bytes = (nc * sizeof(ChainRec) + 15) & ~(size_t)15;
    if (pin_u.ensure(rec_bytes + nc * 8 + 16)) return -1;
    h.rec_all = pin_u.as<ChainRec>();
    h.u_all = reinterpret_cast<const uint64_t *>(reinterpret_cast<const char *>(pin_u.p) + rec_bytes);
    if (o.recs.download(const_cast<ChainRec *>(h.rec_all), nc, st) || o.u_compact.download(const_cast<uint64_t *>(h.u_all), nc, st)) return -1;
    MPN_HIP_CHECK(stream_sync(st));
    return 0;
}

void HostChains::chain_order(int i, int32_t *order, int64_t *src) const {
    const int nc = n_chain[i];
    if (nc == 0) return;
    const uint64_t *u = u_all + u_pos[i];
    const ChainRec *r = rec_all + u_pos[i];
    static thread_local std::vector<std::pair<std::pair<uint64_t, uint64_t>, int>> w;
    w.resize((size_t)nc);
    int64_t k = 0;
    for (int c = 0; c < nc; ++c) { w[c] = {{r[c].fx, (uint64_t)k << 32 | (uint32_t)c}, c}; k += (int32_t)u[c]; }
    std::sort(w.begin(), w.end());
    for (int c = 0; c < nc; ++c) { order[c] = w[c].second; src[c] = (int64_t)(w[c].first.second >> 32); }
}

}

using namespace mpn;

extern "C" {

void mpn_map_opt_init(mpn_map_opt *o) {
    memset(o, 0, sizeof(*o));
    o->k = 15; o->w = 10;
    o->mid_occ_frac = 2e-4f;
    o->min_cnt = 3; o->min_chain_score = 40; o->bw = 500; o->max_gap = 5000;
    o->max_chain_skip = 25; o->max_chain_iter = 5000;
    o->mask_level = 0.5f; o->pri_ratio = 0.8f; o->best_n = 5;
    o->max_join_long = 20000; o->max_join_short = 2000; o->min_join_flank_sc = 1000; o->min_join_flank_ratio = 0.5f;
    o->a = 2; o->b = 4; o->q = 4; o->e = 2; o->q2 = 24; o->e2 = 1;
    o->sc_ambi = 1; o->zdrop = 400; o->zdrop_inv = 200; o->end_bonus = -1;
    o->min_dp_max = o->min_chain_score * o->a;
    o->min_ksw_len = 200;
    o->max_clip_ratio = 1.0f;
    o->max_sw_mat = 100000000;
    o->with_cigar = 1;
    o->seed = 11;
    o->host_threads = 0;
}

static int build_bucket_table(mpn_index *idx, hipStream_t st);

static int pack_targets_device(mpn_index *idx, const uint8_t *d_seqs, int64_t total, hipStream_t st) {
    const int64_t n_words = (total + 15) / 16 + 1;
    DevBuf<unsigned long long> cnt;
    DevBuf<int64_t> starts, ends;
    if (idx->d_seq2.alloc((size_t)n_words) || cnt.alloc(2)) return -1;
    std::vector<int64_t> ns, ne;
    for (int64_t cap = 1 << 16;;) {
        if (cnt.zero(st) || starts.alloc((size_t)cap) || ends.alloc((size_t)cap)) return -1;
        hipLaunchKernelGGL(idx_pack2_kernel, dim3(grid_1d(n_words, 256, 256 * 64)), dim3(256), 0, st, d_seqs, total, idx->d_seq2.p, n_words,
                           cnt.p, starts.p, ends.p, cap);
        MPN_HIP_CHECK(hipGetLastError());
        unsigned long long h_cnt[2] = {0, 0};
        if (cnt.download(h_cnt, 2, st)) return -1;
        MPN_HIP_CHECK(stream_sync(st));
        if (h_cnt[0] != h_cnt[1]) { set_error("index build: unbalanced ambiguous-base runs"); return -1; }
        if ((int64_t)h_cnt[0] > cap) { cap = (int64_t)h_cnt[0] + 16; continue; }
        ns.resize((size_t)h_cnt[0]); ne.resize((size_t)h_cnt[0]);
        if (starts.download(ns.data(), ns.size(), st) || ends.download(ne.data(), ne.size(), st)) return -1;
        MPN_HIP_CHECK(stream_sync(st));
        break;
    }
    std::sort(ns.begin(), ns.end());
    std::sort(ne.begin(), ne.end());
    idx->n_nruns = (int32_t)ns.size();
    if (idx->d_nrun_s.upload(ns.data(), ns.size(), st) || idx->d_nrun_e.upload(ne.data(), ne.size(), st)) return -1;
    MPN_HIP_CHECK(stream_sync(st));
    idx->h_nrun_s.swap(ns); idx->h_nrun_e.swap(ne);
    return 0;
}

static int build_index_device(mpn_index *idx, const uint8_t *d_seqs, const std::vector<int64_t> &off, const int32_t *lens, hipStream_t st) {
    const int n_seq = idx->n_seq, k = idx->k, w = idx->w;
    const int64_t total = off[(size_t)n_seq];
    if (pack_targets_device(idx, d_seqs, total, st)) return -1;
    DevBuf<int64_t> d_off;
    DevBuf<int32_t> d_len;
    if (d_off.upload(off.data(), (size_t)n_seq, st) || d_len.upload(lens, (size_t)n_seq, st)) return -1;
    DevBuf<u128> rec;
    int64_t n_mz = 0;
    const int hbits = 2 * k;
    int bbits = 8, shift = 0, nb = 0;
    DevBuf<int64_t> bucket_off;
    std::vector<int64_t> h_bucket_off;
    {
        DevBuf<int64_t> mz_off;
        DevBuf<u128> mz;
        if (sketch_device(d_seqs, d_off.p, d_len.p, lens, n_seq, k, w, 0, mz_off, mz, &n_mz, st)) return -1;
        idx->n_mz = n_mz;
        while (bbits < 16 && ((int64_t)1 << (bbits + 16)) < n_mz) ++bbits;
        bbits = std::min(bbits, hbits);
        shift = hbits - bbits; nb = 1 << bbits;
        DevBuf<unsigned long long> hist, cursor;
        if (hist.alloc((size_t)nb) || hist.zero(st) || cursor.alloc((size_t)nb + 1) || bucket_off.alloc((size_t)nb + 1) || rec.alloc((size_t)n_mz))
            return -1;
        const int g = grid_1d(n_mz, 256);
        if (n_mz > 0) hipLaunchKernelGGL(idx_bucket_hist_kernel, dim3(g), dim3(256), 0, st, mz.p, n_mz, shift, hist.p);
        hipLaunchKernelGGL(scan_i64_kernel, dim3(1), dim3(1024), 0, st, (const int64_t *)hist.p, bucket_off.p, nb);
        MPN_HIP_CHECK(hipMemcpyAsync(cursor.p, bucket_off.p, ((size_t)nb + 1) * 8, hipMemcpyDeviceToDevice, st));
        if (n_mz > 0) hipLaunchKernelGGL(idx_bucket_scatter_kernel, dim3(g), dim3(256), 0, st, mz.p, n_mz, shift, cursor.p, rec.p);
        MPN_HIP_CHECK(hipGetLastError());
        h_bucket_off.resize((size_t)nb + 1);
// ... 246 lines not shown
    for (int64_t i = 0; i < idx->n_keys; ++i) {
        if (h_key_off[(size_t)i + 1] <= h_key_off[(size_t)i]) return fail("corrupt key offsets");
        if (keys[(size_t)i] > hmask || (i > 0 && keys[(size_t)i] <= keys[(size_t)i - 1])) return fail("keys are not sorted");
    }
    for (int64_t i = 0; i < idx->n_mz; ++i) {
        const uint64_t rid = pos[(size_t)i] >> 32, p = (uint32_t)pos[(size_t)i] >> 1;
        if (rid >= (uint64_t)idx->n_seq || p >= (uint64_t)idx->lens[(size_t)rid]) return fail("position outside its target");
    }
    {
        const int64_t end = (int64_t)ftello(f);
        if (next_offset && end >= 0 && end < file_size) *next_offset = end;
    }
    fclose(f);
    f = nullptr;
    hipStream_t st = 0;
    if (idx->keys.upload(keys.data(), keys.size(), st) || idx->key_off.upload(h_key_off.data(), h_key_off.size(), st) ||
        idx->pos.upload(pos.data(), pos.size(), st) || idx->d_seq_off.upload(idx->seq_off.data(), idx->seq_off.size(), st) ||
        idx->d_lens.upload(idx->lens.data(), idx->lens.size(), st) ||
        idx->d_seq2.upload(idx->h_seq2.data(), idx->h_seq2.size(), st) || idx->d_nrun_s.upload(ns.data(), ns.size(), st) ||
        idx->d_nrun_e.upload(ne.data(), ne.size(), st) || build_bucket_table(idx, st) || stream_sync(st) != hipSuccess) {
        delete idx;
        return nullptr;
    }
    idx->h_nrun_s.swap(ns); idx->h_nrun_e.swap(ne);
    std::vector<uint32_t>().swap(idx->h_seq2);
    return idx;
}

void mpn_index_destroy(mpn_index *idx) { delete idx; }
int64_t mpn_index_n_minimizers(const mpn_index *idx) { return idx->n_mz; }
int64_t mpn_index_n_keys(const mpn_index *idx) { return idx->n_keys; }
int32_t mpn_index_n_seq(const mpn_index *idx) { return idx->n_seq; }
int32_t mpn_index_k(const mpn_index *idx) { return idx->k; }
int32_t mpn_index_w(const mpn_index *idx) { return idx->w; }
int32_t mpn_index_seq_len(const mpn_index *idx, int32_t i) { return i >= 0 && i < idx->n_seq ? idx->lens[(size_t)i] : -1; }
int32_t mpn_index_seq_name(const mpn_index *idx, int32_t i, char *buf, int32_t cap) {
    if (i < 0 || i >= idx->n_seq || !buf || cap <= 0) return -1;
    const std::string &nm = idx->names[(size_t)i];
    const int32_t l = (int32_t)std::min<size_t>(nm.size(), (size_t)cap - 1);
    memcpy(buf, nm.data(), (size_t)l);
    buf[l] = 0;
    return (int32_t)nm.size();
}

int32_t mpn_index_mid_occ(const mpn_index *idx, float f) {
    if (f <= 0.f) return INT32_MAX;
    const int64_t n = idx->n_keys;
    if (n == 0) return 1;
    std::lock_guard<std::mutex> g(idx->mu);
    for (auto &kv : idx->mid_occ_cache) if (kv.first == f) return kv.second;
    int64_t kk = (int64_t)(uint32_t)((1. - (double)f) * (double)n);
    if (kk >= n) kk = n - 1;
    hipStream_t st = 0;
    const int nbins = 1 << 16;
    if (idx->occ_hist.empty()) {
        DevBuf<unsigned long long> hist;
        idx->occ_hist.assign((size_t)nbins, 0);
        if (hist.alloc((size_t)nbins) || hist.zero(st)) return -1;
        hipLaunchKernelGGL(idx_occ_hist_kernel, dim3(grid_1d(n, 256)), dim3(256), 0, st, (const u128 *)idx->kv.p, n, nbins, hist.p);
        if (hist.download((unsigned long long *)idx->occ_hist.data(), (size_t)nbins, st) || stream_sync(st) != hipSuccess) {
            idx->occ_hist.clear();
            set_error("mpn_index_mid_occ: histogram failed");
            return -1;
        }
    }
    int64_t cum = 0, v = -1;
    for (int b = 0; b < nbins; ++b) { cum += (int64_t)idx->occ_hist[(size_t)b]; if (cum > kk) { v = b; break; } }
    if (v < 0 || v == nbins - 1) {
        std::vector<int64_t> h_key_off((size_t)n + 1);
        if (fetch_keys(idx, nullptr, h_key_off.data(), st)) return -1;
        std::vector<uint32_t> a((size_t)n);
        for (int64_t i = 0; i < n; ++i) a[(size_t)i] = (uint32_t)(h_key_off[(size_t)i + 1] - h_key_off[(size_t)i]);
        std::nth_element(a.begin(), a.begin() + kk, a.end());
        v = a[(size_t)kk];
    }
    idx->mid_occ_cache.push_back({f, (int32_t)(v + 1)});
    return (int32_t)(v + 1);
}

__global__ void idx_decode_kernel(RefView rv, int64_t g0, int64_t len, char *out) {
    const int64_t i = (int64_t)blockIdx.x * blockDim.x + threadIdx.x;
    if (i < len) out[i] = "ACGTN"[ref_code(rv, g0 + i)];
}

int64_t mpn_index_fetch_seq(const mpn_index *idx, int32_t i, int64_t start, int64_t len, char *out) {
    if (!idx || !out || i < 0 || i >= idx->n_seq || start < 0 || len < 0 || start + len > idx->lens[(size_t)i]) {
        set_error("mpn_index_fetch_seq: range outside the target");
        return -2;
    }
    if (len == 0) return 0;
    hipStream_t st = 0;
    DevBuf<char> d;
    if (d.alloc((size_t)len)) return -1;
    const RefView rv{idx->d_seq2.p, idx->d_seq_off.p, idx->d_nrun_s.p, idx->d_nrun_e.p, idx->n_nruns};
    hipLaunchKernelGGL(idx_decode_kernel, dim3((unsigned)((len + 255) / 256)), dim3(256), 0, st, rv, idx->seq_off[(size_t)i] + start, len, d.p);
    MPN_HIP_CHECK(hipGetLastError());
    if (d.download(out, (size_t)len, st)) return -1;
    MPN_HIP_CHECK(stream_sync(st));
    return len;
}

int mpn_index_export(const mpn_index *idx, uint64_t *keys, int64_t *key_off, uint64_t *pos) {
    hipStream_t st = 0;
    if (fetch_keys(idx, keys, key_off, st) || idx->pos.download(pos, (size_t)idx->n_mz, st)) return -1;
    MPN_HIP_CHECK(stream_sync(st));
    return 0;
}

int64_t mpn_sketch_batch(int32_t n, const char *seqs, const int64_t *seq_off, const int32_t *seq_len, int32_t k, int32_t w,
                         int64_t *mz_off, uint64_t *mz, int64_t cap) {
    hipStream_t st = 0;
    DevBuf<uint8_t> d_seqs;
    DevBuf<int64_t> d_off, d_mz_off;
    DevBuf<int32_t> d_len;
    DevBuf<u128> d_mz;
    int64_t bases = 0, n_mz = 0;
    if (upload_seqs(n, seqs, seq_off, seq_len, d_seqs, d_off, d_len, &bases, st)) return -1;
    if (sketch_device(d_seqs.p, d_off.p, d_len.p, seq_len, n, k, w, 0, d_mz_off, d_mz, &n_mz, st)) return -1;
    if (d_mz_off.download(mz_off, (size_t)n + 1, st)) return -1;
    if (n_mz <= cap && d_mz.download((u128 *)mz, (size_t)n_mz, st)) return -1;
    MPN_HIP_CHECK(stream_sync(st));
    return n_mz <= cap ? n_mz : -3;
}

int mpn_seed_chain_batch(const mpn_index *idx, const mpn_map_opt *opt, int32_t n, const char *seqs, const int64_t *seq_off,
                         const int32_t *seq_len, int64_t *n_anchor, int32_t *rep_len, int64_t *chain_off, uint64_t *u,
                         int64_t u_cap, int64_t *anchor_off, uint64_t *b, int64_t b_cap) {
    hipStream_t st = 0;
    memset(g_stats, 0, sizeof(g_stats));
    DevBuf<uint8_t> d_seqs;
    DevBuf<int64_t> d_off;
    DevBuf<int32_t> d_len;
    int64_t bases = 0;
    if (upload_seqs(n, seqs, seq_off, seq_len, d_seqs, d_off, d_len, &bases, st)) return -1;
    g_stats[0] = bases;
    SeedChainOut o;
    StreamLease sl(st);
    if (seed_chain_device(idx, opt, n, d_seqs.p, d_off.p, d_len.p, seq_len, o, sl, nullptr)) return -1;
    HostChains h;
    PoolBuf pin_u{nullptr, 0, true}, pin_b{nullptr, 0, true};
    struct Free { PoolBuf &a, &b; ~Free() { a.release(); b.release(); } } free_pins{pin_u, pin_b};
    if (download_chains(n, o, h, pin_u, pin_b, sl, 2)) return -1;
    for (int i = 0; i < n; ++i) { n_anchor[i] = h.n_anchor[i]; rep_len[i] = h.rep_len[i]; }
    memcpy(chain_off, h.chain_off.data(), ((size_t)n + 1) * 8);
    memcpy(anchor_off, h.b_off.data(), ((size_t)n + 1) * 8);
    if (h.chain_off[n] > u_cap || h.b_off[n] > b_cap) return -3;
    for (int i = 0; i < n; ++i) h.read_chains(i, u + h.chain_off[i], (u128 *)b + h.b_off[i]);
    return 0;
}

int mpn_chain_batch(const mpn_map_opt *opt, int32_t n, const int64_t *anchor_off, const uint64_t *anchors, int32_t chain_item,
                    int32_t bt_par_min, int32_t grid_cap, int32_t *n_chain, int64_t *n_chained, uint64_t *u, int64_t *recs, int64_t u_cap,
                    uint64_t *b, int64_t b_cap) {
    if (!opt || n < 0) { set_error("mpn_chain_batch: options missing or a negative count"); return -1; }
    if (opt->max_gap < 0 || opt->bw < 0 || opt->max_chain_skip < 0 || opt->max_chain_iter < 0 || opt->min_cnt < 0 || opt->min_chain_score < 0) {
        set_error("mpn_chain_batch: a negative option"); return -1;
    }
    if (opt->max_chain_iter < 1) { set_error("mpn_chain_batch: max_chain_iter below 1"); return -1; }
    if (chain_gap_check(opt, "mpn_chain_batch")) return -1;
    if (chain_item < 0 || bt_par_min < 0 || grid_cap < 0 || u_cap < 0 || b_cap < 0) { set_error("mpn_chain_batch: chain_item, bt_par_min, grid_cap or a capacity negative"); return -1; }
    if (n == 0) return 0;
    if (!anchor_off || !n_chain || !n_chained) { set_error("mpn_chain_batch: an array missing"); return -1; }
    if (anchor_off[0] != 0) { set_error("mpn_chain_batch: offsets do not start at 0"); return -1; }
    for (int i = 0; i < n; ++i)
        if (anchor_off[i + 1] < anchor_off[i] || anchor_off[i + 1] - anchor_off[i] > 0x3fffffff) { set_error("mpn_chain_batch: read %d: offsets out of order", i); return -1; }
    const int64_t n_a = anchor_off[n];
    if (n_a > 0 && !anchors) { set_error("mpn_chain_batch: an array missing"); return -1; }
    std::vector<int64_t> cnt((size_t)n + 1, 0);
    std::vector<unsigned long long> sums((size_t)n, 0);
    for (int i = 0; i < n; ++i) {
        unsigned long long s = 0;
        for (int64_t k = anchor_off[i]; k < anchor_off[i + 1]; ++k) {
            const uint64_t x = anchors[2 * k], y = anchors[2 * k + 1];
            if (k > anchor_off[i] && x < anchors[2 * (k - 1)]) { set_error("mpn_chain_batch: read %d: anchor %lld: x decreases", i, (long long)(k - anchor_off[i])); return -1; }
            if (y & 0x80000000ull) { set_error("mpn_chain_batch: read %d: anchor %lld: query position outside 0 .. 2^31 - 1", i, (long long)(k - anchor_off[i])); return -1; }
            s += y >> 32 & 0xff;
        }
        cnt[(size_t)i] = anchor_off[i + 1] - anchor_off[i];
        sums[(size_t)i] = s;
    }
    hipStream_t st = 0;
    memset(g_stats, 0, sizeof(g_stats));
    SeedChainOut o;
    StreamLease sl(st);
    EvTimer ev(sl);
    DevBuf<u128> tmp;
    DevBuf<unsigned long long> span_sum, read_kept;
    DevBuf<unsigned int> seg_counters;
    if (alloc_chain_tables(o, n) || o.anchor_off.upload(anchor_off, (size_t)n + 1, st) || o.anchors.upload(reinterpret_cast<const u128 *>(anchors), (size_t)n_a, st) ||
        tmp.alloc((size_t)n_a) || o.n_ends.alloc((size_t)n) || span_sum.upload(sums.data(), (size_t)n, st) || read_kept.alloc((size_t)n) || seg_counters.alloc(4))
        return -1;
    MPN_HIP_CHECK(hipMemcpyAsync(o.n_anchor.p, cnt.data(), ((size_t)n + 1) * 8, hipMemcpyHostToDevice, st));
    {
        ZeroList z{};
        zero_list_push(z, o.used.p, o.used.n * sizeof(unsigned long long));
        zero_list_push(z, seg_counters.p, 4 * sizeof(unsigned int));
        zero_list_push(z, read_kept.p, (size_t)n * 8);
        zero_list_push(z, o.rep_len.p, (size_t)n * 4);
        MPN_HIP_CHECK(zero_regions(z, st));
    }
    o.n_anchors = n_a;
    ChainKnobs kn;
    kn.chain_item = chain_item; kn.bt_par_min = bt_par_min; kn.grid_cap = grid_cap;
    ChainScratch cs;
    if (chain_enqueue(opt, n, n_a, o, tmp.p, read_kept.p, span_sum.p, seg_counters.p, kn, cs, sl, ev)) return -1;
    ev.mark(14);
    MPN_HIP_CHECK(stream_sync(sl));
    ev.resolve();
    HostChains h;
    PoolBuf pin_u{nullptr, 0, true}, pin_b{nullptr, 0, true};
    struct Free { PoolBuf &a, &b; ~Free() { a.release(); b.release(); } } free_pins{pin_u, pin_b};
    if (download_chains(n, o, h, pin_u, pin_b, sl, 2)) return -1;
    if (h.n_pool_chains < 0 || (size_t)h.n_pool_chains > o.recs.n || (size_t)h.b_off[(size_t)n] > o.chained.n || h.chain_off[(size_t)n] != h.n_pool_chains) {
        set_error("mpn_chain_batch: the kernels counted %lld chains and %lld chained anchors, %zu and %zu at most expected", (long long)h.n_pool_chains,
                  (long long)h.b_off[(size_t)n], o.recs.n, o.chained.n);
        return -1;
    }
    std::vector<ChainRec> rv((size_t)h.n_pool_chains + 1);
    if (o.recs.download(rv.data(), (size_t)h.n_pool_chains, st)) return -1;
    MPN_HIP_CHECK(stream_sync(st));
    h.rec_all = rv.data();
    for (int i = 0; i < n; ++i) { n_chain[i] = h.n_chain[(size_t)i]; n_chained[i] = h.n_chained[(size_t)i]; }
    if (h.chain_off[(size_t)n] > u_cap || h.b_off[(size_t)n] > b_cap) return -3;
    if ((h.chain_off[(size_t)n] > 0 && (!u || !recs)) || (h.b_off[(size_t)n] > 0 && !b)) { set_error("mpn_chain_batch: an array missing"); return -1; }
    std::vector<int32_t> order;
    std::vector<int64_t> src;
    for (int i = 0; i < n; ++i) {
        const int nc = h.n_chain[(size_t)i];
        h.read_chains(i, u + h.chain_off[(size_t)i], (u128 *)b + h.b_off[(size_t)i]);
        order.resize((size_t)nc + 1); src.resize((size_t)nc + 1);
        h.chain_order(i, order.data(), src.data());
        for (int c = 0; c < nc; ++c) {
            const ChainRec &r = h.rec_all[h.u_pos[(size_t)i] + order[(size_t)c]];
            int64_t *q = recs + (size_t)(h.chain_off[(size_t)i] + c) * 6;
            q[0] = (int64_t)r.fx; q[1] = (int64_t)r.fy; q[2] = (int64_t)r.lx; q[3] = (int64_t)r.ly; q[4] = r.mlen; q[5] = r.blen;
        }
    }
    return 0;
}

void mpn_map_last_stats(int64_t stats[32]) { memcpy(stats, g_stats, 32 * sizeof(int64_t)); }
int32_t mpn_map_last_stats_ex(int64_t *stats, int32_t n) {
    const int32_t m = n < MPN_NSTATS ? n : MPN_NSTATS;
    if (stats && m > 0) memcpy(stats, g_stats, (size_t)m * sizeof(int64_t));
    return MPN_NSTATS;
}

}
```

### megapath_nano_amd/csrc/mapper_internal.h

```cpp
#pragma once
#include "mpn_common.h"
#include "map_types.h"
#include "queue_lease.h"

#include <atomic>
#include <chrono>
#include <time.h>
#include <mutex>
#include <stdint.h>
#include <stdlib.h>
#include <string.h>
#include <string>
#include <vector>

struct mpn_map_opt_s;


struct mpn_index {
    int k = 15, w = 10;
    int32_t n_seq = 0;
    std::vector<std::string> names;
    std::vector<int32_t> lens;
    std::vector<int64_t> seq_off;
    std::vector<uint32_t> h_seq2;
    std::vector<int64_t> h_nrun_s, h_nrun_e;
    int64_t n_keys = 0, n_mz = 0;
    mpn::DevBuf<uint64_t> keys, pos;
    mpn::DevBuf<int64_t> key_off;
    mpn::DevBuf<int64_t> bucket_start;
    mpn::DevBuf<mpn::u128> kv;
    int bucket_shift = 0;
    mpn::DevBuf<uint32_t> d_seq2;
    mpn::DevBuf<int64_t> d_seq_off, d_nrun_s, d_nrun_e;
    mpn::DevBuf<int32_t> d_lens;
    int32_t n_nruns = 0;
    mutable std::mutex mu;
    mutable std::vector<std::pair<float, int32_t>> mid_occ_cache;
    mutable std::vector<uint64_t> occ_hist;
};

namespace mpn {

struct SeedChainOut {
    int64_t n_anchors = 0;
    DevBuf<unsigned char> tables;
    size_t tables_bytes = 0;
    DevBuf<int64_t> n_anchor;
    DevBuf<int64_t> anchor_off, c_off, n_chained, u_pos, b_pos;
    DevBuf<int32_t> rep_len, n_ends, n_chain;
    DevBuf<u128> anchors, chained;
    DevBuf<uint64_t> u, u_compact;
    DevBuf<ChainRec> recs;
    DevBuf<unsigned long long> used;
};

struct ReadSketch {
    DevBuf<int64_t> mz_off;
    DevBuf<u128> mz;
    int64_t n_mz = 0;
    int k = 0, w = 0;
    bool valid = false;
};

struct HostChains {
    std::vector<int64_t> n_anchor, chain_off, b_off;
    std::vector<int64_t> n_chained, u_pos, b_pos;
    std::vector<int32_t> n_chain, rep_len;
    const uint64_t *u_all = nullptr;
    const u128 *b_all = nullptr;
    const ChainRec *rec_all = nullptr;
    int64_t n_pool_chains = 0;
    void read_chains(int i, uint64_t *u_out, u128 *b_out) const;
    void chain_order(int i, int32_t *order, int64_t *src) const;
};

constexpr int MPN_NSTATS = 77;
constexpr int STAT_LEASE_WAIT = 65;
constexpr int STAT_SIDE_LEASED = 66, STAT_SIDE_OWN = 67;
constexpr int STAT_TILE_CLASS = 68, STAT_TILE_GIVEUPS = 72;
constexpr int STAT_WALK_WAVE = 73, STAT_EV_WALK_LONG = 74, STAT_WALK_WAVE_FAILED = 75;
constexpr int STAT_K_TAGS = 76;
extern thread_local int64_t g_stats[MPN_NSTATS];

void pack_2bit(const uint8_t *codes, int64_t n, std::vector<uint32_t> &words, std::vector<int64_t> &ns, std::vector<int64_t> &ne);

hipError_t stream_sync(hipStream_t st);

struct QueueStreams {
    LeasePool pool;
    std::vector<hipStream_t> st;
    explicit QueueStreams(int q) : pool(q), st((size_t)q, nullptr) {}
};
QueueStreams *queue_streams(int dev);

class StreamLease {
  public:
    explicit StreamLease(QueueStreams *qs) : qs_(qs) {}
    explicit StreamLease(hipStream_t fixed) : fixed_(fixed) {}
    StreamLease(const StreamLease &) = delete;
    StreamLease &operator=(const StreamLease &) = delete;
    ~StreamLease() { release(); }
    hipStream_t get() {
        if (!qs_) return fixed_;
        if (n_ == 0) n_ = qs_->pool.acquire(1, id_, &g_stats[STAT_LEASE_WAIT]);
        return qs_->st[(size_t)id_[0]];
    }
    operator hipStream_t() { return get(); }
    int try_extra(int k, hipStream_t *out) {
        if (!qs_ || n_ == 0) return 0;
        const int got = qs_->pool.try_acquire(std::min(k, 3 - n_), id_ + n_);
        for (int i = 0; i < got; ++i) out[i] = qs_->st[(size_t)id_[n_ + i]];
        n_ += got;
        return got;
    }
    hipError_t sync_release() {
        hipError_t rc = hipSuccess;
        if (!qs_) return stream_sync(fixed_);
        for (int i = 0; i < n_; ++i) { const hipError_t r = stream_sync(qs_->st[(size_t)id_[i]]); if (rc == hipSuccess) rc = r; }
        release();
        return rc;
    }

  private:
    void release() { if (qs_ && n_) { qs_->pool.release(id_, n_); n_ = 0; } }
    QueueStreams *qs_ = nullptr;
    hipStream_t fixed_ = nullptr;
    int id_[3] = {0, 0, 0};
    int n_ = 0;
};
static inline hipError_t stream_sync(StreamLease &st) { return st.sync_release(); }

struct EvTimer {
    hipStream_t st = nullptr;
    StreamLease *lease = nullptr;
    std::vector<hipEvent_t> ev;
    std::vector<int> slot, slot2;
    static bool enabled() { static const bool on = []() { const char *e = getenv("MPN_KERNEL_EVENTS"); return !e || atoi(e) != 0; }(); return on; }
    explicit EvTimer(hipStream_t s) : st(s) { push(); }
    explicit EvTimer(StreamLease &l) : lease(&l) { push(); }
    void push() {
        if (!enabled()) return;
        hipEvent_t e = nullptr;
        (void)hipEventCreate(&e);
        (void)hipEventRecord(e, lease ? lease->get() : st);
        ev.push_back(e);
        slot.push_back(-1); slot2.push_back(-1);
    }
    void mark(int stat_index, int single = -1) { if (!enabled()) return; slot.back() = stat_index; slot2.back() = single; push(); }
    void skip() { push(); }
    void resolve() {
        if (!enabled()) return;
        for (size_t i = 0; i + 1 < ev.size(); ++i) {
            if (slot[i] < 0 && slot2[i] < 0) continue;
            float ms = 0;
            if (hipEventElapsedTime(&ms, ev[i], ev[i + 1]) != hipSuccess) continue;
            if (slot[i] >= 0) g_stats[slot[i]] += (int64_t)(ms * 1e6);
            if (slot2[i] >= 0) g_stats[slot2[i]] += (int64_t)(ms * 1e6);
        }
        for (size_t i = 0; i + 1 < ev.size(); ++i) (void)hipEventDestroy(ev[i]);
        hipEvent_t last = ev.back();
        ev.assign(1, last); slot.assign(1, -1); slot2.assign(1, -1);
    }
    ~EvTimer() { for (hipEvent_t e : ev) (void)hipEventDestroy(e); }
};

struct PoolBuf {
    void *p = nullptr;
    size_t cap = 0;
    bool pinned_host = false;
    int ensure(size_t bytes) {
        if (bytes <= cap) return 0;
        if (p) { if (pinned_host) (void)hipHostFree(p); else (void)hipFree(p); p = nullptr; cap = 0; }
        size_t want = bytes + bytes / 8 + 4096;
        const hipError_t e_ = pinned_host ? hipHostMalloc(&p, want, hipHostMallocDefault) : guarded_malloc(&p, want);
        if (e_ != hipSuccess) {
            if (e_ == hipErrorOutOfMemory && !pinned_host) tl_oom = true;
            p = nullptr;
            set_error("%s of %zu bytes failed: %s", pinned_host ? "hipHostMalloc" : "hipMalloc", want, hipGetErrorString(e_));
            (void)hipGetLastError();
            return -1;
        }
        cap = want;
        return 0;
    }
    void release() { if (p) { if (pinned_host) (void)hipHostFree(p); else (void)hipFree(p); } p = nullptr; cap = 0; }
    template <typename T> T *as() const { return (T *)p; }
};

struct PhaseLog {
    struct Rec { int worker, slot; int64_t t0, t1; };
    std::mutex mu;
    std::vector<Rec> recs;
    bool on = false;
    std::chrono::steady_clock::time_point origin;
    void add(int worker, int slot, std::chrono::steady_clock::time_point a, std::chrono::steady_clock::time_point b) {
        std::lock_guard<std::mutex> g(mu);
        recs.push_back({worker, slot, std::chrono::duration_cast<std::chrono::nanoseconds>(a - origin).count(),
                        std::chrono::duration_cast<std::chrono::nanoseconds>(b - origin).count()});
    }
};
extern PhaseLog g_phase_log;
extern thread_local int tl_worker_id;

extern bool g_worker_cpu_on;
extern std::atomic<long long> g_worker_cpu_ns[64];
static inline long long thread_cpu_ns() {
    timespec t;
    clock_gettime(CLOCK_THREAD_CPUTIME_ID, &t);
    return t.tv_sec * 1000000000LL + t.tv_nsec;
}

struct WallTimer {
    std::chrono::steady_clock::time_point t0 = std::chrono::steady_clock::now();
    long long c0 = g_worker_cpu_on ? thread_cpu_ns() : 0;
    void stop_into(int64_t &acc) {
        auto t1 = std::chrono::steady_clock::now();
        acc += std::chrono::duration_cast<std::chrono::nanoseconds>(t1 - t0).count();
        if (g_phase_log.on) g_phase_log.add(tl_worker_id, (int)(&acc - g_stats), t0, t1);
        if (g_worker_cpu_on) { const long long c1 = thread_cpu_ns(); g_worker_cpu_ns[(&acc - g_stats) & 63] += c1 - c0; c0 = c1; }
        t0 = t1;
    }
};

}
```

### megapath_nano_amd/mapper.py

```python
import ctypes as ct
import os

import numpy as np

from . import _ffi


class MapOpt(ct.Structure):
    _fields_ = [('k', ct.c_int32), ('w', ct.c_int32), ('mid_occ_frac', ct.c_float), ('mid_occ', ct.c_int32),
                ('max_gap', ct.c_int32), ('bw', ct.c_int32), ('max_chain_skip', ct.c_int32), ('max_chain_iter', ct.c_int32),
                ('min_cnt', ct.c_int32), ('min_chain_score', ct.c_int32), ('mask_level', ct.c_float),
                ('pri_ratio', ct.c_float), ('best_n', ct.c_int32), ('max_join_long', ct.c_int32),
                ('max_join_short', ct.c_int32), ('min_join_flank_sc', ct.c_int32), ('min_join_flank_ratio', ct.c_float),
                ('a', ct.c_int32), ('b', ct.c_int32), ('q', ct.c_int32), ('e', ct.c_int32), ('q2', ct.c_int32),
                ('e2', ct.c_int32), ('sc_ambi', ct.c_int32), ('zdrop', ct.c_int32), ('zdrop_inv', ct.c_int32),
                ('end_bonus', ct.c_int32), ('min_dp_max', ct.c_int32), ('min_ksw_len', ct.c_int32),
                ('max_clip_ratio', ct.c_float), ('max_sw_mat', ct.c_int64), ('with_cigar', ct.c_int32),
                ('seed', ct.c_uint32), ('host_threads', ct.c_int32), ('out_sam', ct.c_int32), ('out_tags', ct.c_int32)]


TAG_CS, TAG_CS_LONG, TAG_MD, TAG_EQX = 1, 2, 4, 8


COL_NAMES = ('read_idx', 'qs', 'qe', 'rev', 'rid', 'rs', 're', 'mlen', 'blen', 'mapq', 'nm', 'as_', 'primary')


class AlnCols(ct.Structure):
    _fields_ = [('cap', ct.c_int64), ('n_rows', ct.c_int64)] + [(n, ct.c_void_p) for n in COL_NAMES]


_bound = False


def _bind():
    global _bound
    lib = _ffi.lib()
    if not _bound:
        P = ct.c_void_p
        lib.mpn_map_opt_init.argtypes = [ct.POINTER(MapOpt)]
        lib.mpn_map_opt_init.restype = None
        lib.mpn_index_build.argtypes = [ct.c_int32, ct.POINTER(ct.c_char_p), ct.POINTER(ct.c_char_p), P, ct.c_int32, ct.c_int32]
        lib.mpn_index_build.restype = P
        lib.mpn_index_build_device.argtypes = [ct.c_int32, ct.POINTER(ct.c_char_p), P, P, P, ct.c_int32, ct.c_int32]
        lib.mpn_index_build_device.restype = P
        lib.mpn_index_destroy.argtypes = [P]
        lib.mpn_index_destroy.restype = None
        lib.mpn_index_n_minimizers.argtypes = [P]
        lib.mpn_index_n_minimizers.restype = ct.c_int64
        lib.mpn_index_n_keys.argtypes = [P]
        lib.mpn_index_n_keys.restype = ct.c_int64
        lib.mpn_index_mid_occ.argtypes = [P, ct.c_float]
        lib.mpn_index_mid_occ.restype = ct.c_int32
        lib.mpn_index_fetch_seq.argtypes = [P, ct.c_int32, ct.c_int64, ct.c_int64, ct.c_char_p]
        lib.mpn_index_fetch_seq.restype = ct.c_int64
        lib.mpn_index_export.argtypes = [P, P, P, P]
        lib.mpn_index_export.restype = ct.c_int
        lib.mpn_sam_header.argtypes = [P, ct.c_char_p, ct.c_char_p, ct.c_int64]
        lib.mpn_sam_header.restype = ct.c_int64
        lib.mpn_index_save.argtypes = [P, ct.c_char_p]
        lib.mpn_index_save.restype = ct.c_int
        lib.mpn_index_load.argtypes = [ct.c_char_p]
        lib.mpn_index_load.restype = P
        lib.mpn_index_save_append.argtypes = [P, ct.c_char_p]
        lib.mpn_index_save_append.restype = ct.c_int
        lib.mpn_index_load_at.argtypes = [ct.c_char_p, ct.c_int64, ct.POINTER(ct.c_int64)]
        lib.mpn_index_load_at.restype = P
        for fn in ('mpn_index_n_seq', 'mpn_index_k', 'mpn_index_w'):
            getattr(lib, fn).argtypes = [P]
            getattr(lib, fn).restype = ct.c_int32
        lib.mpn_index_seq_len.argtypes = [P, ct.c_int32]
        lib.mpn_index_seq_len.restype = ct.c_int32
        lib.mpn_index_seq_name.argtypes = [P, ct.c_int32, ct.c_char_p, ct.c_int32]
        lib.mpn_index_seq_name.restype = ct.c_int32
        lib.mpn_sketch_batch.argtypes = [ct.c_int32, P, P, P, ct.c_int32, ct.c_int32, P, P, ct.c_int64]
        lib.mpn_sketch_batch.restype = ct.c_int64
        lib.mpn_seed_chain_batch.argtypes = [P, ct.POINTER(MapOpt), ct.c_int32, P, P, P, P, P, P, P, ct.c_int64, P, P, ct.c_int64]
        lib.mpn_seed_chain_batch.restype = ct.c_int
        if True:
            lib.mpn_map_batch.argtypes = [P, ct.POINTER(MapOpt), ct.c_int32, ct.POINTER(ct.c_char_p), P, P, P, P, ct.c_int64]
            lib.mpn_map_batch.restype = ct.c_int64
        lib.mpn_map_batch_ex.argtypes = [P, ct.POINTER(MapOpt), ct.c_int32, ct.POINTER(ct.c_char_p), P, P, P, P, P, P, P,
                                         ct.c_int64, ct.POINTER(AlnCols)]
        lib.mpn_map_batch_ex.restype = ct.c_int64
        lib.mpn_map_batch_q.argtypes = [P, ct.POINTER(MapOpt), ct.c_int32, ct.POINTER(ct.c_char_p), P, P, P, P, P, P, P, P,
                                        ct.c_int64, ct.POINTER(AlnCols)]
        lib.mpn_map_batch_q.restype = ct.c_int64
        lib.mpn_hits_create.argtypes = [ct.c_int32]
        lib.mpn_hits_create.restype = P
        lib.mpn_hits_destroy.argtypes = [P]
        lib.mpn_hits_destroy.restype = None
        for fn in ('mpn_hits_n_seq', 'mpn_hits_n_parts'):
            getattr(lib, fn).argtypes = [P]
            getattr(lib, fn).restype = ct.c_int32
        lib.mpn_hits_seq_len.argtypes = [P, ct.c_int32]
        lib.mpn_hits_seq_len.restype = ct.c_int32
        lib.mpn_hits_seq_name.argtypes = [P, ct.c_int32, ct.c_char_p, ct.c_int32]
        lib.mpn_hits_seq_name.restype = ct.c_int32
        lib.mpn_hits_sam_header.argtypes = [P, ct.c_char_p, ct.c_char_p, ct.c_int64]
        lib.mpn_hits_sam_header.restype = ct.c_int64
        lib.mpn_map_batch_part.argtypes = [P, ct.POINTER(MapOpt), ct.c_int32, ct.POINTER(ct.c_char_p), P, P, P, P, P, P, P]
        lib.mpn_map_batch_part.restype = ct.c_int
        lib.mpn_map_batch_parts.argtypes = [ct.POINTER(ct.c_void_p), ct.c_int32, ct.POINTER(MapOpt), ct.c_int32, ct.POINTER(ct.c_char_p), P, P, P, P, P, P, P]
        lib.mpn_map_batch_parts.restype = ct.c_int
        lib.mpn_hits_set_text.argtypes = [P, ct.c_int32]
        lib.mpn_hits_set_text.restype = None
        lib.mpn_hits_export.argtypes = [P, ct.c_int32, ct.c_int32, P, ct.c_int64]
        lib.mpn_hits_export.restype = ct.c_int64
        lib.mpn_hits_import.argtypes = [P, P, ct.c_int64, ct.c_int32, ct.c_int32, ct.POINTER(ct.c_char_p), P]
        lib.mpn_hits_import.restype = ct.c_int
        lib.mpn_index_part_info.argtypes = [ct.c_char_p, ct.c_int64, ct.POINTER(ct.c_int64), ct.POINTER(ct.c_int64)]
        lib.mpn_index_part_info.restype = ct.c_int32
        lib.mpn_hits_finish.argtypes = [P, ct.POINTER(MapOpt), ct.c_int32, ct.POINTER(ct.c_char_p), P, P, P, P, P, ct.c_int64,
                                        ct.POINTER(AlnCols)]
        lib.mpn_hits_finish.restype = ct.c_int64
        lib.mpn_map_fetch_sam.argtypes = [ct.c_char_p, ct.c_int64]
        lib.mpn_map_fetch_sam.restype = ct.c_int64
        lib.mpn_map_fetch_cols.argtypes = [ct.POINTER(AlnCols)]
        lib.mpn_map_fetch_cols.restype = ct.c_int64
        lib.mpn_map_fetch_text.argtypes = [ct.c_char_p, ct.c_int64]
        lib.mpn_map_fetch_text.restype = ct.c_int64
        lib.mpn_ext_dp_batch.argtypes = [ct.POINTER(MapOpt), ct.c_int32, P, P, P, P, P, P, P, P, P, P, ct.c_int32, P, P, ct.c_int64, P]
        lib.mpn_ext_dp_batch.restype = ct.c_int
        lib.mpn_aln_tags_batch.argtypes = [ct.c_int32, P, P, P, P, P, P, P, P, P, P, P, P, P, ct.c_int32, P, ct.c_int64, P, P, ct.c_int64, P,
                                           P, ct.c_int64, P]
        lib.mpn_aln_tags_batch.restype = ct.c_int
        lib.mpn_aln_finish_batch.argtypes = [ct.POINTER(MapOpt), ct.c_int32, P, P, P, P, P, P, P, P, P, P, P, P, P, ct.c_int32, P, P]
        lib.mpn_aln_finish_batch.restype = ct.c_int
        lib.mpn_hit_select_batch.argtypes = [ct.POINTER(MapOpt), ct.c_int32, ct.c_int32, P, ct.POINTER(ct.c_char_p), P, P, P, P, P, P, P, P, P, P,
                                             ct.c_int32, ct.c_int32, ct.c_int32, P, P, P, P]
        lib.mpn_hit_select_batch.restype = ct.c_int
        lib.mpn_ext_plan_batch.argtypes = [ct.POINTER(MapOpt), ct.c_int32, ct.c_int32, P, ct.c_int32, P, P, P, P, P, P, P, P, ct.c_int32, P, ct.c_int64,
                                           P, P, P]
        lib.mpn_ext_plan_batch.restype = ct.c_int
        lib.mpn_stitch_batch.argtypes = [ct.c_int32, P, P, ct.c_int32, P, ct.c_int64, P, P, ct.c_int64, P, ct.c_int32, ct.c_int32, P, ct.c_int64, P, P,
                                         P, P]
        lib.mpn_stitch_batch.restype = ct.c_int
        lib.mpn_chain_batch.argtypes = [ct.POINTER(MapOpt), ct.c_int32, P, P, ct.c_int32, ct.c_int32, ct.c_int32, P, P, P, P, ct.c_int64, P, ct.c_int64]
        lib.mpn_chain_batch.restype = ct.c_int
        lib.mpn_map_last_stats.argtypes = [P]
        lib.mpn_map_last_stats.restype = None
        lib.mpn_reads_split_plan.argtypes = [ct.c_int32, P, ct.c_int64, P, P, ct.c_int32, ct.c_int64, P, P, P, P, P, P]
        lib.mpn_reads_split_plan.restype = ct.c_int
        lib.mpn_reads_split_gather.argtypes = [ct.c_int32, P, P, ct.c_int64, P, P, ct.c_int32, ct.c_int64, P, P, ct.c_int64, P, P, ct.c_int64, P, P]
        lib.mpn_reads_split_gather.restype = ct.c_int
        lib.mpn_reads_split_last_ns.argtypes = [ct.c_int32]
        lib.mpn_reads_split_last_ns.restype = ct.c_int64
        lib.mpn_map_last_stats_ex.argtypes = [P, ct.c_int32]
        lib.mpn_map_last_stats_ex.restype = ct.c_int32
        _bound = True
    return lib


def default_opt(**kw):
    o = MapOpt()
    _bind().mpn_map_opt_init(ct.byref(o))
    for k, v in kw.items():
        setattr(o, k, v)
    return o


def pack_seqs(seqs):
    lens = np.array([len(s) for s in seqs], dtype=np.int32)
    off = np.zeros(len(seqs), dtype=np.int64)
    if len(seqs) > 1:
        off[1:] = np.cumsum(lens[:-1].astype(np.int64))
    total = int(lens.astype(np.int64).sum())
    buf = np.zeros(total + 16, dtype=np.uint8)
    for s, o in zip(seqs, off):
        a = np.frombuffer(s, dtype=np.uint8) if isinstance(s, (bytes, bytearray)) else np.asarray(s, dtype=np.uint8)
        buf[o:o + len(a)] = a
    return buf, off, lens


class Index:

    MAGIC = b'MPNIDX01'

    def __init__(self, genomes, k=15, w=10):
        lib = _bind()
        n = len(genomes)
        self.names = [g[0] for g in genomes]
        seqs_b = [bytes(g[1]) if not isinstance(g[1], bytes) else g[1] for g in genomes]
        self.lens = np.array([len(s) for s in seqs_b], dtype=np.int32)
        names = (ct.c_char_p * n)(*[x.encode() for x in self.names])
        seqs = (ct.c_char_p * n)(*seqs_b)
        self.k, self.w = k, w
        self.h = lib.mpn_index_build(n, names, seqs, self.lens.ctypes.data, k, w)
        if not self.h:
            raise _ffi.MpnError('mpn_index_build failed: ' + _ffi.hint(_ffi.last_error()))

    @classmethod
    def from_device(cls, names, d_seqs_ptr, lens, k=15, w=10):
        lib = _bind()
        self = cls.__new__(cls)
        n = len(names)
        self.names = list(names)
        self.lens = np.ascontiguousarray(lens, dtype=np.int32)
        off = np.zeros(n + 1, dtype=np.int64)
        off[1:] = np.cumsum(self.lens.astype(np.int64))
        cn = (ct.c_char_p * n)(*[x.encode() for x in self.names])
        self.k, self.w = k, w
        self.h = lib.mpn_index_build_device(n, cn, d_seqs_ptr, off.ctypes.data, self.lens.ctypes.data, k, w)
        if not self.h:
            raise _ffi.MpnError('mpn_index_build_device failed: ' + _ffi.hint(_ffi.last_error()))
        return self

    def sam_header(self, cmdline=None):
        cap = 64 * len(self.names) + sum(len(n) for n in self.names) + 4096 + (len(cmdline) if cmdline else 0)
        buf = ct.create_string_buffer(cap)
        r = _bind().mpn_sam_header(self.h, cmdline.encode() if cmdline else None, buf, cap)
        if r < 0:
            raise _ffi.MpnError(f'mpn_sam_header rc={r}')
        return buf.raw[:r].decode()

    def save(self, path, append=False):
        lib = _bind()
        _ffi.check((lib.mpn_index_save_append if append else lib.mpn_index_save)(self.h, os.fsencode(path)), 'mpn_index_save')

    @classmethod
    def load(cls, path):
        idx, _ = cls.load_at(path, 0)
        return idx

    @classmethod
    def iter_parts(cls, path):
        off = 0
        while off >= 0:
            idx, off = cls.load_at(path, off)
            yield idx

    @classmethod
    def load_at(cls, path, offset):
        lib = _bind()
        nxt = ct.c_int64(-1)
        h = lib.mpn_index_load_at(os.fsencode(path), int(offset), ct.byref(nxt))
        if not h:
            raise _ffi.MpnError('mpn_index_load failed: ' + _ffi.last_error())
        self = cls._from_handle(h)
        return self, int(nxt.value)

    @classmethod
    def part_info(cls, path):
        lib = _bind()
        out, off = [], 0
        while off >= 0:
            bases, nxt = ct.c_int64(0), ct.c_int64(-1)
            n = lib.mpn_index_part_info(os.fsencode(path), int(off), ct.byref(bases), ct.byref(nxt))
            if n < 0:
                raise _ffi.MpnError('mpn_index_part_info failed: ' + _ffi.last_error())
            out.append((off, int(n), int(bases.value)))
            off = int(nxt.value)
        return out

    @classmethod
    def _from_handle(cls, h):
        lib = _bind()
        self = cls.__new__(cls)
        self.h = h
        n = lib.mpn_index_n_seq(h)
        buf = ct.create_string_buffer(1 << 16)
        self.names, lens = [], []
        for i in range(n):
            lib.mpn_index_seq_name(h, i, buf, len(buf))
            self.names.append(buf.value.decode())
            lens.append(lib.mpn_index_seq_len(h, i))
        self.lens = np.array(lens, dtype=np.int32)
        self.k, self.w = lib.mpn_index_k(h), lib.mpn_index_w(h)
        return self

    @classmethod
    def is_index_file(cls, path):
        try:
            with open(path, 'rb') as f:
                return f.read(8) == cls.MAGIC
        except OSError:
            return False

    @property
    def n_minimizers(self):
        return _bind().mpn_index_n_minimizers(self.h)

    @property
    def n_keys(self):
        return _bind().mpn_index_n_keys(self.h)

    def mid_occ(self, f=2e-4):
        return _bind().mpn_index_mid_occ(self.h, f)

    def fetch_seq(self, i, start, length):
        buf = ct.create_string_buffer(int(length) + 1)
        r = _bind().mpn_index_fetch_seq(self.h, int(i), int(start), int(length), buf)
        if r < 0:
            raise _ffi.MpnError(f'mpn_index_fetch_seq rc={r}: {_ffi.last_error()}')
        return buf.raw[:r]

    def export(self):
        keys = np.zeros(self.n_keys, dtype=np.uint64)
        key_off = np.zeros(self.n_keys + 1, dtype=np.int64)
        pos = np.zeros(self.n_minimizers, dtype=np.uint64)
        _ffi.check(_bind().mpn_index_export(self.h, keys.ctypes.data, key_off.ctypes.data, pos.ctypes.data), 'mpn_index_export')
        return keys, key_off, pos

    def close(self):
        if self.h:
            _bind().mpn_index_destroy(self.h)
            self.h = None

    def __del__(self):
        try:
            self.close()
        except Exception:
            pass


def sketch_batch(seqs, k=15, w=10):
    lib = _bind()
    buf, off, lens = pack_seqs(seqs)
    n = len(seqs)
    mz_off = np.zeros(n + 1, dtype=np.int64)
    cap = int(lens.astype(np.int64).sum()) + 16
    mz = np.zeros((cap, 2), dtype=np.uint64)
    r = lib.mpn_sketch_batch(n, buf.ctypes.data, off.ctypes.data, lens.ctypes.data, k, w, mz_off.ctypes.data, mz.ctypes.data, cap)
    if r < 0:
        raise _ffi.MpnError(f'mpn_sketch_batch rc={r}: {_ffi.last_error()}')
    return [mz[mz_off[i]:mz_off[i + 1]].copy() for i in range(n)]


def seed_chain_batch(idx, opt, seqs):
    lib = _bind()
    buf, off, lens = pack_seqs(seqs)
    n = len(seqs)
    n_anchor = np.zeros(n, dtype=np.int64)
    rep_len = np.zeros(n, dtype=np.int32)
    chain_off = np.zeros(n + 1, dtype=np.int64)
    anchor_off = np.zeros(n + 1, dtype=np.int64)
    u_cap, b_cap = 1 << 16, 1 << 20
    while True:
        u = np.zeros(u_cap, dtype=np.uint64)
        b = np.zeros((b_cap, 2), dtype=np.uint64)
        rc = lib.mpn_seed_chain_batch(idx.h, ct.byref(opt), n, buf.ctypes.data, off.ctypes.data, lens.ctypes.data,
                                      n_anchor.ctypes.data, rep_len.ctypes.data, chain_off.ctypes.data, u.ctypes.data, u_cap,
                                      anchor_off.ctypes.data, b.ctypes.data, b_cap)
        if rc == -3:
            u_cap, b_cap = max(u_cap, int(chain_off[n]) + 1), max(b_cap, int(anchor_off[n]) + 1)
            continue
        _ffi.check(rc, 'mpn_seed_chain_batch')
        break
    return [dict(n_anchor=int(n_anchor[i]), rep_len=int(rep_len[i]), u=u[chain_off[i]:chain_off[i + 1]].copy(),
                 b=b[anchor_off[i]:anchor_off[i + 1]].copy()) for i in range(n)]


CHAIN_REC_KEYS = ('fx', 'fy', 'lx', 'ly', 'mlen', 'blen')


def chain_batch(opt, anchor_off, anchors, chain_item=0, bt_par_min=0, grid_cap=0):
    lib = _bind()
    anchor_off = np.ascontiguousarray(anchor_off, dtype=np.int64)
    anchors = np.ascontiguousarray(anchors, dtype=np.uint64).reshape(-1, 2)
    n = len(anchor_off) - 1
    assert n >= 0 and (n == 0 or len(anchors) >= int(anchor_off[-1]))
    n_chain = np.zeros(n + 1, dtype=np.int32)
    n_chained = np.zeros(n + 1, dtype=np.int64)
    u_cap, b_cap = len(anchors) // 4 + 16, len(anchors) + 16
    while True:
        u = np.zeros(u_cap, dtype=np.uint64)
        recs = np.zeros((u_cap, 6), dtype=np.int64)
        b = np.zeros((b_cap, 2), dtype=np.uint64)
        rc = lib.mpn_chain_batch(ct.byref(opt), n, anchor_off.ctypes.data, anchors.ctypes.data, int(chain_item), int(bt_par_min), int(grid_cap),
                                 n_chain.ctypes.data, n_chained.ctypes.data, u.ctypes.data, recs.ctypes.data, u_cap, b.ctypes.data, b_cap)
        if rc == -3:
            u_cap, b_cap = max(u_cap, int(n_chain.sum()) + 1), max(b_cap, int(n_chained.sum()) + 1)
            continue
        _ffi.check(rc, 'mpn_chain_batch')
        break
    c_off = np.concatenate([[0], np.cumsum(n_chain[:n].astype(np.int64))])
    b_off = np.concatenate([[0], np.cumsum(n_chained[:n])])
    return [dict(n_chain=int(n_chain[i]), n_chained=int(n_chained[i]), u=u[c_off[i]:c_off[i + 1]].copy(), b=b[b_off[i]:b_off[i + 1]].copy(),
                 recs=recs[c_off[i]:c_off[i + 1]].copy()) for i in range(n)]


def map_batch(idx, opt, names, seqs):
    packed = PackedReads(names, seqs)
    return map_batch_ex(idx, opt, packed, want_paf=True, want_cols=False)[0]


class PackedReads:

    def __init__(self, names, seqs, device=None, quals=None):
        self.n = len(seqs)
        self.names = list(names)
        self.buf, self.off, self.lens = pack_seqs(seqs)
        self.qbuf = None
        if quals is not None and any(q is not None for q in quals):
            self.qbuf = pack_seqs([q if q is not None else b'!' * int(l) for q, l in zip(quals, self.lens)])[0]
        self._finish(device)

    @classmethod
    def from_arrays(cls, names, buf, off, lens, dev=None, qbuf=None):
        self = cls.__new__(cls)
        self.n = len(lens)
        self.names = list(names)
        self.buf = np.ascontiguousarray(buf, dtype=np.uint8)
        self.off = np.ascontiguousarray(off, dtype=np.int64)
        self.lens = np.ascontiguousarray(lens, dtype=np.int32)
        self.qbuf = None if qbuf is None else np.ascontiguousarray(qbuf, dtype=np.uint8)
        self._finish(None)
        self.dev = dev
        return self

    def _finish(self, device):
        self.cnames = (ct.c_char_p * self.n)(*[x.encode() for x in self.names])
        self.bases = int(self.lens.astype(np.int64).sum())
        self.dev = None
        if device is not None:
            import torch
            self.dev = (torch.from_numpy(self.buf).to(device), torch.from_numpy(self.off).to(device),
                        torch.from_numpy(self.lens).to(device))
            torch.cuda.synchronize(device)

    def seq(self, i):
        return self.buf[self.off[i]:self.off[i] + self.lens[i]]

    def sub(self, lo, hi):
        lo, hi = int(lo), int(hi)
        assert 0 <= lo <= hi <= self.n, (lo, hi, self.n)
        a = int(self.off[lo]) if hi > lo else 0
        b = int(self.off[hi - 1] + self.lens[hi - 1]) if hi > lo else 0
        out = self.__class__.__new__(self.__class__)
        out.n = hi - lo
        out.names = self.names[lo:hi]
        out.buf = np.zeros(b - a + 16, dtype=np.uint8)
        out.buf[:b - a] = self.buf[a:b]
        out.off = (self.off[lo:hi] - a).astype(np.int64)
        out.lens = self.lens[lo:hi].copy()
        out.qbuf = None
        if getattr(self, 'qbuf', None) is not None:
            out.qbuf = np.zeros(b - a + 16, dtype=np.uint8)
            out.qbuf[:b - a] = self.qbuf[a:b]
        out._finish(self.dev[0].device if self.dev is not None else None)
        return out


SPLIT_ALIGN = 16
PLAN_KEYS = ('n_out', 'out_read', 'group_first', 'out_off', 'group_byte', 'out_bytes')


def _split_args(lens, mem_read, mem_group):
    c = lambda v, t: np.ascontiguousarray(v, dtype=t)
    lens, mem_read, mem_group = c(lens, np.int32), c(mem_read, np.int32), c(mem_group, np.int32)
    if mem_read.shape != mem_group.shape or mem_read.ndim != 1:
        raise ValueError('mem_read and mem_group: two 1-d arrays of one length')
    return lens, mem_read, mem_group


def host_split_plan(lens, mem_read, mem_group, n_groups):
    lens, mem_read, mem_group = _split_args(lens, mem_read, mem_group)
    n, n_groups = len(lens), int(n_groups)
    if (lens < 0).any() or ((mem_read < 0) | (mem_read >= n)).any() or ((mem_group < 0) | (mem_group >= n_groups)).any():
        raise ValueError('split: a negative length, or a pair outside [0, n) x [0, n_groups)')
    key = np.unique(mem_group.astype(np.int64) << 32 | mem_read.astype(np.int64))
    out_group, out_read = (key >> 32).astype(np.int64), (key & 0xffffffff).astype(np.int32)
    group_first = np.searchsorted(out_group, np.arange(n_groups + 1)).astype(np.int64)
    out_len = lens[out_read].astype(np.int64)
    g_bytes = np.bincount(out_group, weights=None if not len(key) else out_len, minlength=n_groups).astype(np.int64) if n_groups else np.zeros(0, np.int64)
    group_byte = np.zeros(n_groups + 1, dtype=np.int64)
    group_byte[1:] = np.cumsum((g_bytes + SPLIT_ALIGN - 1) // SPLIT_ALIGN * SPLIT_ALIGN)
    before = np.cumsum(out_len) - out_len
    out_off = group_byte[out_group] + before - (before[group_first[out_group]] if len(key) else 0)
    return dict(n_out=len(key), out_read=out_read, group_first=group_first, out_off=out_off.astype(np.int64), group_byte=group_byte,
                out_bytes=int(group_byte[n_groups]) + SPLIT_ALIGN)


def host_split_gather(plan, buf, off, lens, qbuf=None):
    outs = []
    for src in (buf, qbuf):
        if src is None:
            outs.append(None)
            continue
        o = np.zeros(plan['out_bytes'], dtype=np.uint8)
        for r, d in zip(plan['out_read'], plan['out_off']):
            o[d:d + lens[r]] = src[off[r]:off[r] + lens[r]]
        outs.append(o)
    return outs[0], outs[1]


def host_split_reads(buf, off, lens, mem_read, mem_group, n_groups, qbuf=None):
    plan = host_split_plan(lens, mem_read, mem_group, n_groups)
    plan['seqs'], plan['quals'] = host_split_gather(plan, buf, off, lens, qbuf)
    return plan


def device_split_plan(lens, mem_read, mem_group, n_groups, out_cap=None):
    lib = _bind()
    lens, mem_read, mem_group = _split_args(lens, mem_read, mem_group)
    n, m, n_groups = len(lens), len(mem_read), int(n_groups)
    cap = m if out_cap is None else int(out_cap)
    out_read, out_off = np.zeros(max(cap, 1), dtype=np.int32), np.zeros(max(cap, 1), dtype=np.int64)
    group_first, group_byte = np.zeros(max(n_groups, 0) + 1, dtype=np.int64), np.zeros(max(n_groups, 0) + 1, dtype=np.int64)
    n_out, out_bytes = ct.c_int64(0), ct.c_int64(0)
    _ffi.check(lib.mpn_reads_split_plan(n, lens.ctypes.data, m, mem_read.ctypes.data, mem_group.ctypes.data, n_groups, cap, ct.addressof(n_out),
                                        out_read.ctypes.data, group_first.ctypes.data, out_off.ctypes.data, group_byte.ctypes.data,
                                        ct.addressof(out_bytes)), 'mpn_reads_split_plan')
    k = int(n_out.value)
    return dict(n_out=k, out_read=out_read[:k], group_first=group_first, out_off=out_off[:k], group_byte=group_byte, out_bytes=int(out_bytes.value))


def device_split_gather(plan, buf, off, lens, d_out, qbuf=None, d_qout=None, dev_src=None, want_host=True):
    lib = _bind()
    off, lens = np.ascontiguousarray(off, dtype=np.int64), np.ascontiguousarray(lens, dtype=np.int32)
    src_bytes = int((off + lens).max()) if len(lens) else 0
    if dev_src is not None:
        if int(dev_src[0].numel()) < src_bytes or (qbuf is not None and int(dev_src[1].numel()) < src_bytes):
            raise ValueError(f'split: the reads end at byte {src_bytes}, beyond their device buffer')
        s_ptr, q_ptr = dev_src[0].data_ptr(), (dev_src[1].data_ptr() if qbuf is not None else None)
    else:
        buf = np.ascontiguousarray(buf, dtype=np.uint8)
        qbuf = None if qbuf is None else np.ascontiguousarray(qbuf, dtype=np.uint8)
        if len(buf) < src_bytes or (qbuf is not None and len(qbuf) < src_bytes):
            raise ValueError(f'split: the reads end at byte {src_bytes}, beyond their buffer')
        s_ptr, q_ptr = buf.ctypes.data, (qbuf.ctypes.data if qbuf is not None else None)
    with_q = qbuf is not None
    out_bytes = int(plan['out_bytes'])
# ... 263 lines not shown
    for c, o in zip(cigars, coff):
        cig[o:o + len(c)] = np.asarray(c, dtype=np.uint32)
    cols = sum(int(x) >> 4 for c in cigars for x in c)
    ops = int(ncig.astype(np.int64).sum())
    want_cs, want_md, want_eqx = bool(out_tags & (TAG_CS | TAG_CS_LONG)), bool(out_tags & TAG_MD), bool(out_tags & TAG_EQX)
    cs_cap, md_cap, eqx_cap = caps if caps is not None else (3 * cols + 2 * ops + 16, 2 * cols + 2 * ops + 16 * n + 16, cols + ops + 16)
    cs = np.zeros(cs_cap if want_cs else 1, dtype=np.uint8)
    md = np.zeros(md_cap if want_md else 1, dtype=np.uint8)
    eqx = np.zeros(eqx_cap if want_eqx else 1, dtype=np.uint32)
    cs_off, md_off, eqx_off = (np.zeros(n + 1, dtype=np.int64) for _ in range(3))
    rc = lib.mpn_aln_tags_batch(n, qbuf.ctypes.data, qoff.ctypes.data, qlen.ctypes.data, qs.ctypes.data, qe.ctypes.data, rev.ctypes.data,
                                tbuf.ctypes.data, toff.ctypes.data, tlen.ctypes.data, ts.ctypes.data, cig.ctypes.data, coff.ctypes.data,
                                ncig.ctypes.data, int(out_tags), cs.ctypes.data, cs_cap if want_cs else 0, cs_off.ctypes.data,
                                md.ctypes.data, md_cap if want_md else 0, md_off.ctypes.data, eqx.ctypes.data, eqx_cap if want_eqx else 0,
                                eqx_off.ctypes.data)
    _ffi.check(rc, 'mpn_aln_tags_batch')
    res = []
    for i in range(n):
        res.append(dict(cs=cs[cs_off[i]:cs_off[i + 1]].tobytes().decode() if want_cs else None,
                        md=md[md_off[i]:md_off[i + 1]].tobytes().decode() if want_md else None,
                        eqx=[int(x) for x in eqx[eqx_off[i]:eqx_off[i + 1]]] if want_eqx else None))
    return res



def aln_finish_batch(opt, queries, q_ivals, revs, targets, t_starts, cigars, force_class=0):
    lib = _bind()
    n = len(queries)
    qbuf, qoff, qlen = pack_seqs([np.asarray(q, dtype=np.uint8) for q in queries])
    tbuf, toff, tlen = pack_seqs([np.asarray(t, dtype=np.uint8) for t in targets])
    qs = np.ascontiguousarray([iv[0] for iv in q_ivals], dtype=np.int32)
    qe = np.ascontiguousarray([iv[1] for iv in q_ivals], dtype=np.int32)
    rev = np.ascontiguousarray(np.broadcast_to(np.asarray(revs, dtype=np.int32), (n,)))
    ts = np.ascontiguousarray(np.broadcast_to(np.asarray(t_starts, dtype=np.int32), (n,)))
    ncig = np.array([len(c) for c in cigars], dtype=np.int32)
    coff = np.zeros(n, dtype=np.int64)
    if n > 1:
        coff[1:] = np.cumsum(ncig[:-1].astype(np.int64))
    cig = np.zeros(int(ncig.astype(np.int64).sum()) + 1, dtype=np.uint32)
    for c, o in zip(cigars, coff):
        cig[o:o + len(c)] = np.asarray(c, dtype=np.uint32)
    out = np.zeros((n, 8), dtype=np.int32)
    fixed = np.zeros_like(cig)
    rc = lib.mpn_aln_finish_batch(ct.byref(opt), n, qbuf.ctypes.data, qoff.ctypes.data, qlen.ctypes.data, qs.ctypes.data, qe.ctypes.data,
                                  rev.ctypes.data, tbuf.ctypes.data, toff.ctypes.data, tlen.ctypes.data, ts.ctypes.data, cig.ctypes.data,
                                  coff.ctypes.data, ncig.ctypes.data, int(force_class), out.ctypes.data, fixed.ctypes.data)
    _ffi.check(rc, 'mpn_aln_finish_batch')
    keys = ('n_cigar', 'qshift', 'tshift', 'blen', 'mlen', 'n_ambi', 'dp_max')
    res = []
    for i in range(n):
        d = {k: int(out[i, j]) for j, k in enumerate(keys)}
        d['cigar'] = fixed[coff[i]:coff[i] + d['n_cigar']].tolist()
        res.append(d)
    return res


HIT_KEYS = ('fx', 'fy', 'lx', 'ly', 'score', 'score0', 'cnt', 'as', 'parent', 'subsc', 'n_sub', 'mlen', 'blen', 'hash', 'sam_pri')


def hit_select_batch(opt, k, q_len, names, chain_off, u, recs, anchor_off, anchors, path=0, max_chains=0, grid_cap=0):
    lib = _bind()
    n = len(q_len)
    c = lambda v, t: np.ascontiguousarray(v, dtype=t)
    q_len, chain_off, anchor_off, u = c(q_len, np.int32), c(chain_off, np.int64), c(anchor_off, np.int64), c(u, np.uint64)
    fx, fy, lx, ly = (c(r, np.uint64) for r in recs[:4])
    mlen, blen = c(recs[4], np.int32), c(recs[5], np.int32)
    anchors = c(anchors, np.uint64).reshape(-1, 2)
    assert len(chain_off) == n + 1 and len(anchor_off) == n + 1 and len(names) == n
    n_chains, n_anch = int(chain_off[-1]) if n else 0, int(anchor_off[-1]) if n else 0
    assert all(len(x) == n_chains for x in (u, fx, fy, lx, ly, mlen, blen)) and len(anchors) == n_anch
    cnames = (ct.c_char_p * max(1, n))(*[(nm.encode() if isinstance(nm, str) else nm) for nm in names])
    n_regs, n_a = np.zeros(n, dtype=np.int32), np.zeros(n, dtype=np.int32)
    hits = np.zeros((n_chains + 1, 15), dtype=np.int64)
    sq = np.zeros((n_anch + 1, 2), dtype=np.uint64)
    rc = lib.mpn_hit_select_batch(ct.byref(opt), int(k), n, q_len.ctypes.data, cnames, chain_off.ctypes.data, u.ctypes.data, fx.ctypes.data,
                                  fy.ctypes.data, lx.ctypes.data, ly.ctypes.data, mlen.ctypes.data, blen.ctypes.data, anchor_off.ctypes.data,
                                  anchors.ctypes.data, int(path), int(max_chains), int(grid_cap), n_regs.ctypes.data, n_a.ctypes.data,
                                  hits.ctypes.data, sq.ctypes.data)
    _ffi.check(rc, 'mpn_hit_select_batch')
    return n_regs, n_a, hits[:int(n_regs.sum())], (sq[:int(n_a.sum())] if opt.with_cigar else None)


PLAN_HIT_KEYS = ('n_jobs', 'as1', 'cnt1', 'qs', 'rs', 'qe', 're', 'qs0', 'qe0', 'rid', 'rev')
PLAN_WIN_KEYS = ('read', 'rid', 'rev', 'qs', 'qlen', 'ts', 'tlen', 'reversed', 'w', 'zdrop', 'end_bonus', 'flag', 'anchor')


def ext_plan_batch(opt, k, t_len, q_len, anchor_off, anchors, hit_off, h_as, h_cnt, h_mlen, h_split_inv, grid_cap=0):
    lib = _bind()
    n = len(q_len)
    c = lambda v, t: np.ascontiguousarray(v, dtype=t)
    t_len, q_len, anchor_off, hit_off = c(t_len, np.int32), c(q_len, np.int32), c(anchor_off, np.int64), c(hit_off, np.int64)
    h_as, h_cnt, h_mlen, h_split_inv = (c(v, np.int32) for v in (h_as, h_cnt, h_mlen, h_split_inv))
    anchors = c(anchors, np.uint64).reshape(-1, 2)
    assert len(anchor_off) == n + 1 and len(hit_off) == n + 1
    n_anch, n_hits = (int(anchor_off[-1]), int(hit_off[-1])) if n else (0, 0)
    assert len(anchors) == n_anch and all(len(v) == n_hits for v in (h_as, h_cnt, h_mlen, h_split_inv))
    win_cap = int(np.maximum(h_cnt.astype(np.int64), 0).sum()) + n_hits
    hits = np.zeros((n_hits + 1, 11), dtype=np.int32)
    wins = np.zeros((win_cap + 1, 13), dtype=np.int32)
    left = np.zeros((n_anch + 1, 2), dtype=np.uint64)
    n_win = ct.c_int64(0)
    rc = lib.mpn_ext_plan_batch(ct.byref(opt), int(k), len(t_len), t_len.ctypes.data, n, q_len.ctypes.data, anchor_off.ctypes.data,
                                anchors.ctypes.data, hit_off.ctypes.data, h_as.ctypes.data, h_cnt.ctypes.data, h_mlen.ctypes.data,
                                h_split_inv.ctypes.data, int(grid_cap), hits.ctypes.data, win_cap, ct.addressof(n_win), wins.ctypes.data,
                                left.ctypes.data)
    _ffi.check(rc, 'mpn_ext_plan_batch')
    return hits[:n_hits], wins[:n_win.value], left[:n_anch]


STITCH_HIT_KEYS = ('read', 'rid', 'rev', 'as', 'cnt', 'as1', 'cnt1', 'qs', 'rs', 'qe', 're', 'qs0', 'qe0', 'first_win', 'n_win')
STITCH_WIN_KEYS = ('flag', 'reversed', 'qs', 'ts', 'anchor', 'max', 'zdropped', 'max_q', 'max_t', 'mqe_t', 'score', 'reach_end', 'n_cigar')
STITCH_OUT_KEYS = ('cig_off', 'n_ops', 'dp_score', 'rs1', 're1', 'qs1', 'qe1', 'has_p', 'dropped', 'drop_fill', 'drop_max_t', 'drop_max_q',
                   'split_n', 'split_inv', 'split_rec')
STITCH_FIN_KEYS = ('cig_off', 'code_off', 'n_cigar', 'read', 'rid', 'rev', 'qs1', 'rs1', 'qspan', 'tspan')
STITCH_SPLIT_KEYS = ('fx', 'fy', 'lx_left', 'ly_left', 'mlen_l', 'blen_l', 'mlen_r', 'blen_r')


def stitch_batch(anchor_off, anchors, hits, wins, cig_pos, compact, min_cnt, grid_cap=0):
    lib = _bind()
    c = lambda v, t: np.ascontiguousarray(v, dtype=t)
    anchor_off, cig_pos, compact = c(anchor_off, np.int64), c(cig_pos, np.int64), c(compact, np.uint32)
    anchors, hits, wins = c(anchors, np.uint64).reshape(-1, 2), c(hits, np.int32).reshape(-1, 15), c(wins, np.int32).reshape(-1, 13)
    n = len(anchor_off) - 1
    assert n >= 0 and len(anchors) == (int(anchor_off[-1]) if n else 0) and len(cig_pos) == len(wins)
    n_hits = len(hits)
    pool_cap = int(np.maximum(wins[:, 12].astype(np.int64), 0).sum())
    out = np.zeros((n_hits + 1, 25), dtype=np.int64)
    pool = np.zeros(pool_cap + 1, dtype=np.uint32)
    splits = np.zeros((n_hits + 1, 8), dtype=np.int64)
    used, n_splits = ct.c_int64(0), ct.c_int64(0)
    rc = lib.mpn_stitch_batch(n, anchor_off.ctypes.data, anchors.ctypes.data, n_hits, hits.ctypes.data, len(wins), wins.ctypes.data,
                              cig_pos.ctypes.data, len(compact), compact.ctypes.data, int(min_cnt), int(grid_cap), out.ctypes.data, pool_cap,
                              pool.ctypes.data, ct.addressof(used), splits.ctypes.data, ct.addressof(n_splits))
    _ffi.check(rc, 'mpn_stitch_batch')
    return out[:n_hits], pool[:used.value], splits[:n_splits.value]


STAT_NAMES = {0: 'bases', 1: 'minimizers', 2: 'anchors', 3: 'chains', 4: 'dp_jobs', 5: 'dp_cells', 6: 'alignments',
              7: 'dp_rounds', 8: 'second_pass_jobs', 10: 'ev_sketch_ns', 11: 'ev_seed_ns', 12: 'ev_sort_ns',
              13: 'ev_chain_dp_ns', 14: 'ev_chain_bt_ns', 15: 'ev_ext_dp_ns', 25: 'ev_ext_bt_ns', 26: 'ev_ext_ztest_ns',
              16: 'wall_h2d_ns', 17: 'wall_seed_chain_ns', 18: 'wall_d2h_chains_ns', 19: 'wall_host_hits_ns',
              20: 'wall_host_plan_ns', 21: 'wall_ext_stage_ns', 22: 'wall_host_stitch_ns', 23: 'wall_host_final_ns',
              24: 'wall_total_ns', 27: 'wall_ext_host_prep_ns', 28: 'wall_ext_enqueue_ns', 29: 'wall_ext_gpu_wait_ns',
              30: 'wall_ext_finish_ns', 9: 'ev_ext_strip_ns', 31: 'strip_cells', 32: 'sub_batches',
              33: 'k_sketch_count_ns', 34: 'k_sketch_fill_ns', 35: 'k_seed_lookup_ns', 36: 'k_seed_fill_ns',
              37: 'k_chain_dp_ns', 38: 'k_strip16_ns', 39: 'k_strip32_ns', 40: 'k_strip64_ns', 41: 'strip16_cells',
              42: 'strip32_cells', 43: 'strip64_cells', 44: 'sort_records_moved', 45: 'anchors_kept', 46: 'k_compact_ns', 47: 'k_sort_msd_ns', 48: 'k_sort_chunk_ns', 49: 'k_sort_radix_ns',
              50: 'k_seed_filter_ns', 51: 'anchors_emitted', 52: 'k_finish_ns', 53: 'cigar_ops', 54: 'k_stitch_ns', 55: 'k_plan_ns', 56: 'k_layout_ns', 57: 'k_xstrip_ns', 58: 'xstrip_cells', 59: 'anchors_squeezed', 60: 'workers_shed', 61: 'workers', 62: 'k_hit_select_ns', 63: 'reads_hits_on_host',
              64: 'tile_windows', 65: 'wall_lease_wait_ns', 66: 'ext_groups_side_leased', 67: 'ext_groups_side_own',
              68: 'tile_windows_1w_s16', 69: 'tile_windows_s4_nw8', 70: 'tile_windows_s8_nw4', 71: 'tile_windows_s4_nw16',
              72: 'tile_wait_giveups',
              73: 'walk_wave_windows', 74: 'ev_ext_walk_long_ns',
              75: 'walk_wave_failed',
              76: 'k_tags_ns'}


def last_stats():
    n = max(STAT_NAMES) + 1
    s = np.zeros(n, dtype=np.int64)
    _bind().mpn_map_last_stats_ex(s.ctypes.data, n)
    return {name: int(s[i]) for i, name in STAT_NAMES.items()}
```

Baseline: 14.91.

## Stage chain backtrack predecessor steps in LDS with size-classed work queues

Adds an LDS-backed chain backtrack kernel that packs each read's predecessor steps and owner tags into 32-bit shared-memory words. The backtrack walk and ownership atomics then hit LDS instead of global memory. A classify kernel splits reads into small and big classes so the small class can run at higher per-CU occupancy, and blocks pull reads dynamically through atomic queues. Reads that are too large or have step overflows fall back to the old global path. This adds an extra kernel launch, dynamic-LDS limits and new stats counters.

Result: faster. 15.42 (median of 6 runs) (+3.5%).

```diff
diff --git a/include/mpn_map.h b/include/mpn_map.h
--- a/include/mpn_map.h
+++ b/include/mpn_map.h
@@ -69,6 +69,9 @@
 int mpn_chain_batch(const mpn_map_opt *opt, int32_t n, const int64_t *anchor_off, const uint64_t *anchors, int32_t chain_item,
                     int32_t bt_par_min, int32_t grid_cap, int32_t *n_chain, int64_t *n_chained, uint64_t *u, int64_t *recs,
                     int64_t u_cap, uint64_t *b, int64_t b_cap);
+int mpn_chain_batch_ex(const mpn_map_opt *opt, int32_t n, const int64_t *anchor_off, const uint64_t *anchors, int32_t chain_item,
+                       int32_t bt_par_min, int32_t grid_cap, int32_t *n_chain, int64_t *n_chained, uint64_t *u, int64_t *recs,
+                       int64_t u_cap, uint64_t *b, int64_t b_cap, int32_t bt_lds);
 
 int mpn_ext_dp_batch(const mpn_map_opt *opt, int32_t n, const uint8_t *qcodes, const int64_t *q_off, const int32_t *q_len,
                      const uint8_t *tcodes, const int64_t *t_off, const int32_t *t_len, const int32_t *w, const int32_t *zdrop,
diff --git a/megapath_nano_amd/csrc/align.hip b/megapath_nano_amd/csrc/align.hip
--- a/megapath_nano_amd/csrc/align.hip
+++ b/megapath_nano_amd/csrc/align.hip
@@ -1994,7 +1994,7 @@
         }
         tl_arena = nullptr;
         std::lock_guard<std::mutex> g(mu);
-        for (int k = 0; k < MPN_NSTATS; ++k) tot_stats[k] += g_stats[k];
+        for (int k = 0; k < MPN_NSTATS; ++k) tot_stats[k] = k == STAT_BT_MAX ? std::max(tot_stats[k], g_stats[k]) : tot_stats[k] + g_stats[k];
     };
     {
         std::vector<std::thread> th;
diff --git a/megapath_nano_amd/csrc/map_kernels.h b/megapath_nano_amd/csrc/map_kernels.h
--- a/megapath_nano_amd/csrc/map_kernels.h
+++ b/megapath_nano_amd/csrc/map_kernels.h
@@ -1448,19 +1448,44 @@
 
 constexpr int BT_PAR_MIN = 16;
 
-__global__ __launch_bounds__(64) void chain_backtrack_kernel(const u128 *__restrict__ anchors, const int64_t *__restrict__ anchor_off,
-                                                             int n_reads, ChainParams cp, const int32_t *__restrict__ F,
-                                                             const int32_t *__restrict__ P, int32_t *__restrict__ T,
-                                                             int32_t *__restrict__ V, uint64_t *__restrict__ U,
-                                                             const int32_t *__restrict__ n_ends, u128 *__restrict__ B,
-                                                             uint64_t *__restrict__ Uc, unsigned long long *__restrict__ used,
-                                                             int64_t *__restrict__ u_pos, int64_t *__restrict__ b_pos,
-                                                             int32_t *__restrict__ n_chain, int64_t *__restrict__ n_chained,
-                                                             ChainRec *__restrict__ Rc, int par_min) {
-    __shared__ int s_k;
-    __shared__ unsigned long long s_up, s_bp;
-    const int lane = threadIdx.x;
-    for (int read = blockIdx.x; read < n_reads; read += gridDim.x) {
+__device__ __forceinline__ void bt_seq_place(int lane, const u128 *a, const int32_t *v, const uint64_t *u, int k, u128 *b, uint64_t *uc,
+                                             ChainRec *rc) {
+    int off = 0;
+    for (int c = 0; c < k; ++c) {
+        const int ni = (int32_t)u[c];
+        int ml = 0, bl = 0;
+        for (int j = lane; j < ni; j += 64) {
+            const u128 cur = a[v[off + (ni - j - 1)]];
+            b[off + j] = cur;
+            const int span = (int)(cur.y >> 32 & 0xff);
+            if (j == 0) { ml += span; bl += span; }
+            else {
+                const u128 prev = a[v[off + (ni - j)]];
+                const int tl = (int32_t)cur.x - (int32_t)prev.x, ql = (int32_t)cur.y - (int32_t)prev.y;
+                bl += tl > ql ? tl : ql;
+                ml += tl > span && ql > span ? span : tl < ql ? tl : ql;
+            }
+        }
+        ml = __builtin_amdgcn_readlane(wave_scan_add(ml), 63);
+        bl = __builtin_amdgcn_readlane(wave_scan_add(bl), 63);
+        if (lane == 0) {
+            const u128 first = a[v[off + ni - 1]], last = a[v[off]];
+            rc[c] = ChainRec{first.x, first.y, last.x, last.y, ml, bl};
+        }
+        off += ni;
+    }
+    for (int c = lane; c < k; c += 64) uc[c] = u[c];
+}
+
+__device__ __forceinline__ void bt_read_global(int read, int lane, const u128 *__restrict__ anchors, const int64_t *__restrict__ anchor_off,
+                                               const ChainParams &cp, const int32_t *__restrict__ F, const int32_t *__restrict__ P,
+                                               int32_t *__restrict__ T, int32_t *__restrict__ V, uint64_t *__restrict__ U,
+                                               const int32_t *__restrict__ n_ends, u128 *__restrict__ B, uint64_t *__restrict__ Uc,
+                                               unsigned long long *__restrict__ used, int64_t *__restrict__ u_pos,
+                                               int64_t *__restrict__ b_pos, int32_t *__restrict__ n_chain,
+                                               int64_t *__restrict__ n_chained, ChainRec *__restrict__ Rc, int par_min, int &s_k,
+                                               unsigned long long &s_up, unsigned long long &s_bp) {
+    {
         const int64_t base = anchor_off[read];
         const int64_t n = anchor_off[read + 1] - base;
         const u128 *a = anchors + base;
@@ -1545,7 +1570,7 @@
                 nv_run += __builtin_amdgcn_readlane(incl, 63);
             }
             __syncthreads();
-            continue;
+            return;
         }
         for (int64_t i = lane; i < n; i += 64) t[i] = 0;
         __builtin_amdgcn_fence(__ATOMIC_RELEASE, "workgroup");
@@ -1574,35 +1599,262 @@
         }
         __builtin_amdgcn_fence(__ATOMIC_RELEASE, "workgroup");
         __syncthreads();
-        const int k = s_k;
-        u128 *b = B + s_bp;
-        uint64_t *uc = Uc + s_up;
-        ChainRec *rc = Rc + s_up;
-        int off = 0;
-        for (int c = 0; c < k; ++c) {
-            const int ni = (int32_t)u[c];
-            int ml = 0, bl = 0;
-            for (int j = lane; j < ni; j += 64) {
-                const u128 cur = a[v[off + (ni - j - 1)]];
-                b[off + j] = cur;
-                const int span = (int)(cur.y >> 32 & 0xff);
-                if (j == 0) { ml += span; bl += span; }
-                else {
-                    const u128 prev = a[v[off + (ni - j)]];
-                    const int tl = (int32_t)cur.x - (int32_t)prev.x, ql = (int32_t)cur.y - (int32_t)prev.y;
-                    bl += tl > ql ? tl : ql;
-                    ml += tl > span && ql > span ? span : tl < ql ? tl : ql;
-                }
-            }
-            ml = __builtin_amdgcn_readlane(wave_scan_add(ml), 63);
-            bl = __builtin_amdgcn_readlane(wave_scan_add(bl), 63);
+        bt_seq_place(lane, a, v, u, s_k, B + s_bp, Uc + s_up, Rc + s_up);
+        __syncthreads();
+    }
+}
+
+__global__ __launch_bounds__(64) void chain_backtrack_kernel(const u128 *__restrict__ anchors, const int64_t *__restrict__ anchor_off,
+                                                             int n_reads, ChainParams cp, const int32_t *__restrict__ F,
+                                                             const int32_t *__restrict__ P, int32_t *__restrict__ T,
+                                                             int32_t *__restrict__ V, uint64_t *__restrict__ U,
+                                                             const int32_t *__restrict__ n_ends, u128 *__restrict__ B,
+                                                             uint64_t *__restrict__ Uc, unsigned long long *__restrict__ used,
+                                                             int64_t *__restrict__ u_pos, int64_t *__restrict__ b_pos,
+                                                             int32_t *__restrict__ n_chain, int64_t *__restrict__ n_chained,
+                                                             ChainRec *__restrict__ Rc, int par_min) {
+    __shared__ int s_k;
+    __shared__ unsigned long long s_up, s_bp;
+    const int lane = threadIdx.x;
+    for (int read = blockIdx.x; read < n_reads; read += gridDim.x)
+        bt_read_global(read, lane, anchors, anchor_off, cp, F, P, T, V, U, n_ends, B, Uc, used, u_pos, b_pos, n_chain, n_chained, Rc, par_min, s_k, s_up,
+                       s_bp);
+}
+
+constexpr int BT_LDS_BIG = 40000;
+constexpr int BT_LDS_SMALL = 8000;
+#ifndef MPN_BT_PF
+#define MPN_BT_PF 16
+#endif
+constexpr int BT_PF = MPN_BT_PF;
+constexpr int BT_STAGE = 8;
+constexpr uint32_t BT_NONE = 0xffffu;
+constexpr int BT_SLOTS = 6;
+enum { BT_N_SMALL = 0, BT_N_BIG = 1, BT_PULL_SMALL = 2, BT_PULL_BIG = 3, BT_N_GLOBAL = 4, BT_MAX_ANCHORS = 5 };
+
+__global__ __launch_bounds__(256) void chain_bt_classify_kernel(const int64_t *__restrict__ anchor_off, int n_reads, int cap_small,
+                                                                int32_t *__restrict__ list_small, int32_t *__restrict__ list_big,
+                                                                unsigned long long *__restrict__ bt) {
+    const int read = blockIdx.x * 256 + threadIdx.x;
+    const int lane = threadIdx.x & 63;
+    int n = 0;
+    if (read < n_reads) n = (int)(anchor_off[read + 1] - anchor_off[read]);
+    for (int big = 0; big < 2; ++big) {
+        const bool mine = read < n_reads && (n > cap_small) == (big != 0);
+        const unsigned long long m = __ballot(mine);
+        if (m == 0) continue;
+        unsigned long long first = 0;
+        if (lane == __ffsll((long long)m) - 1) first = atomicAdd(&bt[big ? BT_N_BIG : BT_N_SMALL], (unsigned long long)__popcll(m));
+        first = __shfl(first, __ffsll((long long)m) - 1);
+        if (mine) (big ? list_big : list_small)[first + __popcll(m & ((1ULL << lane) - 1))] = read;
+    }
+    for (int d = 32; d; d >>= 1) { const int o = __shfl_xor(n, d); n = o > n ? o : n; }
+    if ((threadIdx.x & 63) == 0 && n > 0) atomicMax(&bt[BT_MAX_ANCHORS], (unsigned long long)n);
+}
+
+__global__ __launch_bounds__(64) void chain_backtrack_lds_kernel(const u128 *__restrict__ anchors, const int64_t *__restrict__ anchor_off,
+                                                                 ChainParams cp, const int32_t *__restrict__ F,
+                                                                 const int32_t *__restrict__ P, int32_t *__restrict__ T,
+                                                                 int32_t *__restrict__ V, uint64_t *__restrict__ U,
+                                                                 const int32_t *__restrict__ n_ends, u128 *__restrict__ B,
+                                                                 uint64_t *__restrict__ Uc, unsigned long long *__restrict__ used,
+                                                                 int64_t *__restrict__ u_pos, int64_t *__restrict__ b_pos,
+                                                                 int32_t *__restrict__ n_chain, int64_t *__restrict__ n_chained,
+                                                                 ChainRec *__restrict__ Rc, int par_min, const int32_t *__restrict__ list,
+                                                                 const unsigned long long *__restrict__ n_list_p,
+                                                                 unsigned long long *__restrict__ pull,
+                                                                 unsigned long long *__restrict__ n_global, int cap) {
+    extern __shared__ uint32_t bt_w[];
+    __shared__ int s_k;
+    __shared__ unsigned long long s_up, s_bp;
+    const int lane = threadIdx.x;
+    const unsigned int n_list = (unsigned int)*n_list_p;
+    for (;;) {
+        unsigned int item = 0;
+        if (lane == 0) item = (unsigned int)atomicAdd(pull, 1ULL);
+        item = (unsigned int)__builtin_amdgcn_readfirstlane((int)item);
+        if (item >= n_list) break;
+        const int read = list[item];
+        const int64_t base = anchor_off[read];
+        const int32_t n = (int32_t)(anchor_off[read + 1] - base);
+        const u128 *a = anchors + base;
+        const int32_t *f = F + base, *p = P + base;
+        int32_t *v = V + base;
+        uint64_t *u = U + base;
+        const int n_u = n_ends[read];
+        bool fits = n <= cap && n_u < (int)BT_NONE;
+        if (fits) {
+            bool bad = false;
+            const auto stage = [&](int32_t i, int32_t pi) {
+                const int32_t step = pi < 0 ? 0 : i - pi;
+                bad |= pi >= 0 && (step <= 0 || step > 0xffff);
+                bt_w[i] = BT_NONE << 16 | ((uint32_t)step & 0xffffu);
+            };
+            const int32_t to_16 = (int32_t)((4 - ((uintptr_t)p >> 2 & 3)) & 3);
+            const int32_t head = to_16 < n ? to_16 : n, n_vec = head + ((n - head) & ~3);
+            if (lane < head) stage(lane, p[lane]);
+            if (lane < n - n_vec) stage(n_vec + lane, p[n_vec + lane]);
+            for (int32_t i0 = head; i0 < n_vec; i0 += 256 * BT_STAGE) {
+                int4 q[BT_STAGE];
+#pragma unroll
+                for (int s = 0; s < BT_STAGE; ++s) {
+                    const int32_t i = i0 + (s * 64 + lane) * 4;
+                    q[s] = i < n_vec ? *reinterpret_cast<const int4 *>(p + i) : make_int4(-1, -1, -1, -1);
+                }
+#pragma unroll
+                for (int s = 0; s < BT_STAGE; ++s) {
+                    const int32_t i = i0 + (s * 64 + lane) * 4;
+                    if (i < n_vec) { stage(i, q[s].x); stage(i + 1, q[s].y); stage(i + 2, q[s].z); stage(i + 3, q[s].w); }
+                }
+            }
+            fits = !__any(bad);
+        }
+        __syncthreads();
+        if (!fits) {
+            if (lane == 0) atomicAdd(n_global, 1ULL);
+            bt_read_global(read, lane, anchors, anchor_off, cp, F, P, T, V, U, n_ends, B, Uc, used, u_pos, b_pos, n_chain, n_chained, Rc, par_min, s_k,
+                           s_up, s_bp);
+            continue;
+        }
+        if (n_u >= par_min) {
+            for (int e0 = 0; e0 < n_u; e0 += 64) {
+                const int e = e0 + lane;
+                if (e < n_u) {
+                    int32_t j = (int32_t)u[e];
+                    uint32_t w = bt_w[j];
+                    for (int32_t it = 0; it < n; ++it) {
+                        const uint32_t step = w & 0xffffu;
+                        const int32_t nj = step ? j - (int32_t)step : -1;
+                        const uint32_t wn = nj >= 0 ? bt_w[nj] : 0u;
+                        if (atomicMin(&bt_w[j], (uint32_t)e << 16 | step) >> 16 < (uint32_t)e) break;
+                        if (nj < 0) break;
+                        j = nj; w = wn;
+                    }
+                }
+            }
+            __syncthreads();
+            int k_run = 0, nv_run = 0;
+            for (int e0 = 0; e0 < n_u; e0 += 64) {
+                const int e = e0 + lane;
+                int cnt = 0;
+                if (e < n_u) {
+                    const uint64_t ui = u[e];
+                    int32_t j = (int32_t)ui;
+                    uint32_t step = bt_w[j] & 0xffffu;
+                    j = step ? j - (int32_t)step : -1;
+                    cnt = 1;
+                    for (int32_t it = 0; j >= 0 && it < n; ++it) {
+                        const uint32_t w = bt_w[j];
+                        if (w >> 16 != (uint32_t)e) break;
+                        ++cnt;
+                        step = w & 0xffffu;
+                        j = step ? j - (int32_t)step : -1;
+                    }
+                    const bool keep = cnt >= cp.min_cnt && (j < 0 || (int32_t)(ui >> 32) - f[j] >= cp.min_sc);
+                    if (!keep) cnt = 0;
+                    v[e] = cnt;
+                }
+                k_run += __builtin_amdgcn_readlane(wave_scan_add(cnt > 0 ? 1 : 0), 63);
+                nv_run += __builtin_amdgcn_readlane(wave_scan_add(cnt), 63);
+            }
             if (lane == 0) {
-                const u128 first = a[v[off + ni - 1]], last = a[v[off]];
-                rc[c] = ChainRec{first.x, first.y, last.x, last.y, ml, bl};
-            }
-            off += ni;
-        }
-        for (int c = lane; c < k; c += 64) uc[c] = u[c];
+                s_k = k_run;
+                n_chain[read] = k_run;
+                n_chained[read] = nv_run;
+                s_up = k_run ? atomicAdd(&used[0], (unsigned long long)k_run) : 0ULL;
+                s_bp = nv_run ? atomicAdd(&used[1], (unsigned long long)nv_run) : 0ULL;
+                u_pos[read] = (int64_t)s_up;
+                b_pos[read] = (int64_t)s_bp;
+            }
+            __builtin_amdgcn_fence(__ATOMIC_ACQ_REL, "workgroup");
+            __syncthreads();
+            u128 *b = B + s_bp;
+            uint64_t *uc = Uc + s_up;
+            ChainRec *rc = Rc + s_up;
+            k_run = 0; nv_run = 0;
+            for (int e0 = 0; e0 < n_u; e0 += 64) {
+                const int e = e0 + lane;
+                const int cnt = e < n_u ? v[e] : 0;
+                const int incl = wave_scan_add(cnt), kin = wave_scan_add(cnt > 0 ? 1 : 0);
+                if (cnt > 0) {
+                    const int kidx = k_run + kin - 1, off = nv_run + incl - cnt;
+                    const uint64_t ui = u[e];
+                    int32_t j = (int32_t)ui;
+                    u128 nxt = a[j];
+                    const u128 last = nxt;
+                    int ml = 0, bl = 0;
+                    b[off + cnt - 1] = nxt;
+                    for (int q = cnt - 2; q >= 0; q -= BT_PF) {
+                        int32_t jj[BT_PF];
+                        u128 c[BT_PF];
+#pragma unroll
+                        for (int s = 0; s < BT_PF; ++s) {
+                            if (s <= q) j -= (int32_t)(bt_w[j] & 0xffffu);
+                            jj[s] = j;
+                        }
+#pragma unroll
+                        for (int s = 0; s < BT_PF; ++s) c[s] = a[jj[s]];
+#pragma unroll
+                        for (int s = 0; s < BT_PF; ++s) {
+                            if (s <= q) {
+                                const u128 cur = c[s];
+                                b[off + q - s] = cur;
+                                const int span = (int)(nxt.y >> 32 & 0xff);
+                                const int tl = (int32_t)nxt.x - (int32_t)cur.x, ql = (int32_t)nxt.y - (int32_t)cur.y;
+                                bl += tl > ql ? tl : ql;
+                                ml += tl > span && ql > span ? span : tl < ql ? tl : ql;
+                                nxt = cur;
+                            }
+                        }
+                    }
+                    const int span0 = (int)(nxt.y >> 32 & 0xff);
+                    ml += span0; bl += span0;
+                    const uint32_t step = bt_w[j] & 0xffffu;
+                    j = step ? j - (int32_t)step : -1;
+                    const uint64_t sc = j < 0 ? ui >> 32 : (ui >> 32) - (uint64_t)f[j];
+                    uc[kidx] = sc << 32 | (uint32_t)cnt;
+                    rc[kidx] = ChainRec{nxt.x, nxt.y, last.x, last.y, ml, bl};
+                }
+                k_run += __builtin_amdgcn_readlane(kin, 63);
+                nv_run += __builtin_amdgcn_readlane(incl, 63);
+            }
+            __syncthreads();
+            continue;
+        }
+        if (lane == 0) {
+            int n_v = 0, k = 0;
+            for (int i = 0; i < n_u; ++i) {
+                const int n_v0 = n_v, k0 = k;
+                const uint64_t ui = u[i];
+                int32_t j = (int32_t)ui;
+                uint32_t w = bt_w[j];
+                for (int32_t it = 0; it < n; ++it) {
+                    if (n_v < n) v[n_v++] = j;
+                    bt_w[j] = w & 0xffffu;
+                    const uint32_t step = w & 0xffffu;
+                    j = step ? j - (int32_t)step : -1;
+                    if (j < 0) break;
+                    w = bt_w[j];
+                    if (w >> 16 != BT_NONE) break;
+                }
+                if (j < 0) {
+                    if (n_v - n_v0 >= cp.min_cnt) u[k++] = ui >> 32 << 32 | (uint32_t)(n_v - n_v0);
+                } else if ((int32_t)(ui >> 32) - f[j] >= cp.min_sc) {
+                    if (n_v - n_v0 >= cp.min_cnt) u[k++] = ((ui >> 32) - (uint64_t)f[j]) << 32 | (uint32_t)(n_v - n_v0);
+                }
+                if (k0 == k) n_v = n_v0;
+            }
+            s_k = k;
+            n_chain[read] = k;
+            n_chained[read] = n_v;
+            s_up = k ? atomicAdd(&used[0], (unsigned long long)k) : 0ULL;
+            s_bp = n_v ? atomicAdd(&used[1], (unsigned long long)n_v) : 0ULL;
+            u_pos[read] = (int64_t)s_up;
+            b_pos[read] = (int64_t)s_bp;
+        }
+        __builtin_amdgcn_fence(__ATOMIC_RELEASE, "workgroup");
+        __syncthreads();
+        bt_seq_place(lane, a, v, u, s_k, B + s_bp, Uc + s_up, Rc + s_up);
         __syncthreads();
     }
 }
diff --git a/megapath_nano_amd/csrc/mapper.hip b/megapath_nano_amd/csrc/mapper.hip
--- a/megapath_nano_amd/csrc/mapper.hip
+++ b/megapath_nano_amd/csrc/mapper.hip
@@ -233,11 +233,11 @@
 
 static int alloc_chain_tables(SeedChainOut &o, int n) {
     const size_t N = (size_t)n, o1 = (N + 1) * 8, o2 = o1 + N * 8, o3 = o2 + N * 8, o4 = o3 + N * 8, o5 = o4 + N * 4, o6 = (o5 + N * 4 + 7) & ~(size_t)7;
-    o.tables_bytes = o6 + (size_t)(2 + WORK_SLOTS) * 8;
+    o.tables_bytes = o6 + (size_t)(2 + WORK_SLOTS + BT_SLOTS) * 8;
     if (o.tables.alloc(o.tables_bytes)) return -1;
     auto view = [&](auto &buf, size_t off, size_t count) { buf.release(); buf.p = reinterpret_cast<decltype(buf.p)>(o.tables.p + off); buf.n = count; buf.owned = false; };
     view(o.n_anchor, 0, N + 1); view(o.n_chained, o1, N); view(o.u_pos, o2, N); view(o.b_pos, o3, N);
-    view(o.n_chain, o4, N); view(o.rep_len, o5, N); view(o.used, o6, 2 + WORK_SLOTS);
+    view(o.n_chain, o4, N); view(o.rep_len, o5, N); view(o.used, o6, 2 + WORK_SLOTS + BT_SLOTS);
     return 0;
 }
 
@@ -245,6 +245,7 @@
     int chain_item = 0;
     int bt_par_min = 0;
     int grid_cap = 0;
+    int bt_lds = 0;
 };
 struct ChainScratch {
     DevBuf<int64_t> kept, piece_kept, piece_off;
@@ -252,11 +253,12 @@
     DevBuf<int32_t> F, P, T, V;
     DevBuf<uint64_t> Utmp;
     DevBuf<ChainSeg> seg_big, seg_small;
+    DevBuf<int32_t> bt_list;
 };
 static int chain_enqueue(const mpn_map_opt *opt, int n, int64_t n_a, SeedChainOut &o, u128 *tmp, unsigned long long *read_kept,
                          const unsigned long long *span_sum, unsigned int *seg_counters, const ChainKnobs &kn, ChainScratch &cs, StreamLease &st,
                          EvTimer &ev) {
-    auto &[kept, piece_kept, piece_off, avg_qspan, F, P, T, V, Utmp, seg_big, seg_small] = cs;
+    auto &[kept, piece_kept, piece_off, avg_qspan, F, P, T, V, Utmp, seg_big, seg_small, bt_list] = cs;
     ChainParams cp;
     cp.max_dist_x = opt->max_gap; cp.max_dist_y = opt->max_gap; cp.bw = opt->bw; cp.max_skip = opt->max_chain_skip;
     cp.max_iter = opt->max_chain_iter; cp.min_cnt = opt->min_cnt; cp.min_sc = opt->min_chain_score;
@@ -308,8 +310,38 @@
     o.u_compact.p = Utmp.p; o.u_compact.n = Utmp.n; o.u_compact.owned = Utmp.owned; Utmp.p = nullptr; Utmp.n = 0;
     static const int bt_par_min_env = []() { const char *e = getenv("MPN_BT_PAR_MIN"); return e ? std::max(1, atoi(e)) : BT_PAR_MIN; }();
     const int bt_par_min = kn.bt_par_min > 0 ? kn.bt_par_min : bt_par_min_env;
-    hipLaunchKernelGGL(chain_backtrack_kernel, dim3(g), dim3(64), 0, st, (const u128 *)ca, (const int64_t *)o.c_off.p, n, cp, F.p, P.p, T.p, V.p,
-                       o.u.p, o.n_ends.p, o.chained.p, o.u_compact.p, o.used.p, o.u_pos.p, o.b_pos.p, o.n_chain.p, o.n_chained.p, o.recs.p, bt_par_min);
+    static const bool bt_lds_env = []() { const char *e = getenv("MPN_BT_LDS"); return !e || atoi(e) != 0; }();
+    constexpr int BT_LDS_MIN_AVG = 2048;
+    int cap_big = BT_LDS_BIG, cap_small = BT_LDS_SMALL;
+    if (kn.bt_lds > 1) { cap_big = kn.bt_lds & 0xffff; cap_small = kn.bt_lds >> 16 ? kn.bt_lds >> 16 : cap_big; }
+    bool bt_lds = (kn.bt_lds > 1 || (kn.bt_lds == 0 && bt_lds_env)) && cp.max_iter < 65536;
+    if (kn.bt_lds == 0) {
+        const int64_t avg = n_c / std::max(1, n);
+        if (avg > BT_LDS_BIG / 4 || avg < BT_LDS_MIN_AVG) bt_lds = false;
+    }
+    o.bt_global = !bt_lds;
+    if (!bt_lds) {
+        hipLaunchKernelGGL(chain_backtrack_kernel, dim3(g), dim3(64), 0, st, (const u128 *)ca, (const int64_t *)o.c_off.p, n, cp, F.p, P.p, T.p, V.p,
+                           o.u.p, o.n_ends.p, o.chained.p, o.u_compact.p, o.used.p, o.u_pos.p, o.b_pos.p, o.n_chain.p, o.n_chained.p, o.recs.p, bt_par_min);
+        MPN_HIP_CHECK(hipGetLastError());
+        return 0;
+    }
+    if (bt_list.alloc((size_t)2 * n)) return -1;
+    unsigned long long *bt = o.used.p + 2 + WORK_SLOTS;
+    const bool two_classes = cap_small < cap_big;
+    hipLaunchKernelGGL(chain_bt_classify_kernel, dim3(std::max(1, (n + 255) / 256)), dim3(256), 0, st, (const int64_t *)o.c_off.p, n,
+                       two_classes ? cap_small : INT32_MAX, bt_list.p, bt_list.p + n, bt);
+    MPN_HIP_CHECK(hipFuncSetAttribute((const void *)chain_backtrack_lds_kernel, hipFuncAttributeMaxDynamicSharedMemorySize, BT_LDS_BIG * 4));
+    for (int big = 1; big >= 0; --big) {
+        const int cap = big ? cap_big : cap_small;
+        if (big && !two_classes) continue;
+        const int per_cu = big ? 1 : std::min(16, (160 * 1024) / (cap * 4 + 64));
+        const int grid = capped(std::max(1, std::min(n, 256 * std::max(1, per_cu))));
+        hipLaunchKernelGGL(chain_backtrack_lds_kernel, dim3(grid), dim3(64), (size_t)cap * 4, st, (const u128 *)ca, (const int64_t *)o.c_off.p, cp, F.p, P.p,
+                           T.p, V.p, o.u.p, o.n_ends.p, o.chained.p, o.u_compact.p, o.used.p, o.u_pos.p, o.b_pos.p, o.n_chain.p, o.n_chained.p, o.recs.p,
+                           bt_par_min, (const int32_t *)(bt_list.p + (big ? n : 0)), (const unsigned long long *)(bt + (big ? BT_N_BIG : BT_N_SMALL)),
+                           bt + (big ? BT_PULL_BIG : BT_PULL_SMALL), bt + BT_N_GLOBAL, cap);
+    }
     MPN_HIP_CHECK(hipGetLastError());
     return 0;
 }
@@ -465,7 +497,7 @@
     const bool with_anchors = mode == 2;
     h.n_anchor.resize((size_t)n);
     h.n_chain.resize(n); h.n_chained.resize(n); h.rep_len.resize(n); h.u_pos.resize(n); h.b_pos.resize(n);
-    unsigned long long used[2 + WORK_SLOTS] = {0};
+    unsigned long long used[2 + WORK_SLOTS + BT_SLOTS] = {0};
     {
         const size_t N = (size_t)n;
         const size_t o1 = (N + 1) * 8, o2 = o1 + N * 8, o3 = o2 + N * 8, o4 = o3 + N * 8, o5 = o4 + N * 4, o6 = (o5 + N * 4 + 7) & ~(size_t)7;
@@ -480,6 +512,13 @@
     }
     for (int k = 0; k < WORK_SLOTS; ++k) g_stats[44] += (int64_t)used[2 + k];
     ++g_stats[32];
+    {
+        const unsigned long long *bt = used + 2 + WORK_SLOTS;
+        const int64_t n_global = o.bt_global ? n : (int64_t)bt[BT_N_GLOBAL];
+        g_stats[STAT_BT_GLOBAL] += n_global;
+        g_stats[STAT_BT_LDS] += n - n_global;
+        g_stats[STAT_BT_MAX] = std::max(g_stats[STAT_BT_MAX], (int64_t)bt[BT_MAX_ANCHORS]);
+    }
     h.n_pool_chains = (int64_t)used[0];
     if (mode == 0) { h.u_all = nullptr; h.rec_all = nullptr; h.b_all = nullptr; }
     else if (with_anchors) {
@@ -1032,6 +1071,12 @@
 int mpn_chain_batch(const mpn_map_opt *opt, int32_t n, const int64_t *anchor_off, const uint64_t *anchors, int32_t chain_item,
                     int32_t bt_par_min, int32_t grid_cap, int32_t *n_chain, int64_t *n_chained, uint64_t *u, int64_t *recs, int64_t u_cap,
                     uint64_t *b, int64_t b_cap) {
+    return mpn_chain_batch_ex(opt, n, anchor_off, anchors, chain_item, bt_par_min, grid_cap, n_chain, n_chained, u, recs, u_cap, b, b_cap, 0);
+}
+
+int mpn_chain_batch_ex(const mpn_map_opt *opt, int32_t n, const int64_t *anchor_off, const uint64_t *anchors, int32_t chain_item,
+                       int32_t bt_par_min, int32_t grid_cap, int32_t *n_chain, int64_t *n_chained, uint64_t *u, int64_t *recs, int64_t u_cap,
+                       uint64_t *b, int64_t b_cap, int32_t bt_lds) {
     if (!opt || n < 0) { set_error("mpn_chain_batch: options missing or a negative count"); return -1; }
     if (opt->max_gap < 0 || opt->bw < 0 || opt->max_chain_skip < 0 || opt->max_chain_iter < 0 || opt->min_cnt < 0 || opt->min_chain_score < 0) {
         set_error("mpn_chain_batch: a negative option"); return -1;
@@ -1039,6 +1084,10 @@
     if (opt->max_chain_iter < 1) { set_error("mpn_chain_batch: max_chain_iter below 1"); return -1; }
     if (chain_gap_check(opt, "mpn_chain_batch")) return -1;
     if (chain_item < 0 || bt_par_min < 0 || grid_cap < 0 || u_cap < 0 || b_cap < 0) { set_error("mpn_chain_batch: chain_item, bt_par_min, grid_cap or a capacity negative"); return -1; }
+    if (bt_lds < 0 || (bt_lds > 1 && ((bt_lds & 0xffff) < 2 || (bt_lds & 0xffff) > BT_LDS_BIG || (bt_lds >> 16) > (bt_lds & 0xffff)))) {
+        set_error("mpn_chain_batch: bt_lds %d: neither 0, 1 nor a capacity of 2 .. %d anchors with a small class (<< 16) within it", bt_lds, BT_LDS_BIG);
+        return -1;
+    }
     if (n == 0) return 0;
     if (!anchor_off || !n_chain || !n_chained) { set_error("mpn_chain_batch: an array missing"); return -1; }
     if (anchor_off[0] != 0) { set_error("mpn_chain_batch: offsets do not start at 0"); return -1; }
@@ -1081,7 +1130,7 @@
     }
     o.n_anchors = n_a;
     ChainKnobs kn;
-    kn.chain_item = chain_item; kn.bt_par_min = bt_par_min; kn.grid_cap = grid_cap;
+    kn.chain_item = chain_item; kn.bt_par_min = bt_par_min; kn.grid_cap = grid_cap; kn.bt_lds = bt_lds;
     ChainScratch cs;
     if (chain_enqueue(opt, n, n_a, o, tmp.p, read_kept.p, span_sum.p, seg_counters.p, kn, cs, sl, ev)) return -1;
     ev.mark(14);
diff --git a/megapath_nano_amd/csrc/mapper_internal.h b/megapath_nano_amd/csrc/mapper_internal.h
--- a/megapath_nano_amd/csrc/mapper_internal.h
+++ b/megapath_nano_amd/csrc/mapper_internal.h
@@ -52,6 +52,7 @@
     DevBuf<uint64_t> u, u_compact;
     DevBuf<ChainRec> recs;
     DevBuf<unsigned long long> used;
+    bool bt_global = false;
 };
 
 struct ReadSketch {
@@ -74,12 +75,13 @@
     void chain_order(int i, int32_t *order, int64_t *src) const;
 };
 
-constexpr int MPN_NSTATS = 77;
+constexpr int MPN_NSTATS = 80;
 constexpr int STAT_LEASE_WAIT = 65;
 constexpr int STAT_SIDE_LEASED = 66, STAT_SIDE_OWN = 67;
 constexpr int STAT_TILE_CLASS = 68, STAT_TILE_GIVEUPS = 72;
 constexpr int STAT_WALK_WAVE = 73, STAT_EV_WALK_LONG = 74, STAT_WALK_WAVE_FAILED = 75;
 constexpr int STAT_K_TAGS = 76;
+constexpr int STAT_BT_LDS = 77, STAT_BT_GLOBAL = 78, STAT_BT_MAX = 79;
 extern thread_local int64_t g_stats[MPN_NSTATS];
 
 void pack_2bit(const uint8_t *codes, int64_t n, std::vector<uint32_t> &words, std::vector<int64_t> &ns, std::vector<int64_t> &ne);
diff --git a/megapath_nano_amd/mapper.py b/megapath_nano_amd/mapper.py
--- a/megapath_nano_amd/mapper.py
+++ b/megapath_nano_amd/mapper.py
@@ -137,6 +137,8 @@
         lib.mpn_stitch_batch.restype = ct.c_int
         lib.mpn_chain_batch.argtypes = [ct.POINTER(MapOpt), ct.c_int32, P, P, ct.c_int32, ct.c_int32, ct.c_int32, P, P, P, P, ct.c_int64, P, ct.c_int64]
         lib.mpn_chain_batch.restype = ct.c_int
+        lib.mpn_chain_batch_ex.argtypes = lib.mpn_chain_batch.argtypes + [ct.c_int32]
+        lib.mpn_chain_batch_ex.restype = ct.c_int
         lib.mpn_map_last_stats.argtypes = [P]
         lib.mpn_map_last_stats.restype = None
         lib.mpn_reads_split_plan.argtypes = [ct.c_int32, P, ct.c_int64, P, P, ct.c_int32, ct.c_int64, P, P, P, P, P, P]
@@ -353,7 +355,7 @@
 CHAIN_REC_KEYS = ('fx', 'fy', 'lx', 'ly', 'mlen', 'blen')
 
 
-def chain_batch(opt, anchor_off, anchors, chain_item=0, bt_par_min=0, grid_cap=0):
+def chain_batch(opt, anchor_off, anchors, chain_item=0, bt_par_min=0, grid_cap=0, bt_lds=0):
     lib = _bind()
     anchor_off = np.ascontiguousarray(anchor_off, dtype=np.int64)
     anchors = np.ascontiguousarray(anchors, dtype=np.uint64).reshape(-1, 2)
@@ -366,8 +368,8 @@
         u = np.zeros(u_cap, dtype=np.uint64)
         recs = np.zeros((u_cap, 6), dtype=np.int64)
         b = np.zeros((b_cap, 2), dtype=np.uint64)
-        rc = lib.mpn_chain_batch(ct.byref(opt), n, anchor_off.ctypes.data, anchors.ctypes.data, int(chain_item), int(bt_par_min), int(grid_cap),
-                                 n_chain.ctypes.data, n_chained.ctypes.data, u.ctypes.data, recs.ctypes.data, u_cap, b.ctypes.data, b_cap)
+        rc = lib.mpn_chain_batch_ex(ct.byref(opt), n, anchor_off.ctypes.data, anchors.ctypes.data, int(chain_item), int(bt_par_min), int(grid_cap),
+                                    n_chain.ctypes.data, n_chained.ctypes.data, u.ctypes.data, recs.ctypes.data, u_cap, b.ctypes.data, b_cap, int(bt_lds))
         if rc == -3:
             u_cap, b_cap = max(u_cap, int(n_chain.sum()) + 1), max(b_cap, int(n_chained.sum()) + 1)
             continue
@@ -937,7 +939,8 @@
               72: 'tile_wait_giveups',
               73: 'walk_wave_windows', 74: 'ev_ext_walk_long_ns',
               75: 'walk_wave_failed',
-              76: 'k_tags_ns'}
+              76: 'k_tags_ns',
+              77: 'bt_reads_lds', 78: 'bt_reads_global', 79: 'bt_max_read_anchors'}
 
 
 def last_stats():
```
